# dune-community/pylrbms

Hardware: AMD Instinct MI355X
Metric: offline project+estimate throughput (higher is better)
Workload: dtype f64; 1 GPU; BASELINE.json config 3: 2D multiscale diffusion, 32x32 subdomains, k_c=4 (n=384 DG DoFs, n_rt=208 RT0 DoFs per subdomain), Q=2, local basis dim 40; subdomains=1024, N=40, Q=2, parallelism=subdomain tiles x1

## Files before the change

include/lrbms_hip.h:

```cpp
#ifndef LRBMS_HIP_H
#define LRBMS_HIP_H

#include <stdint.h>

#ifdef __cplusplus
extern "C" {
#endif

#define LRBMS_OK 0
#define LRBMS_E_INVALID (-1)
#define LRBMS_E_HIP (-2)
#define LRBMS_E_STATE (-3)
#define LRBMS_E_NOT_CONVERGED (-4)

#define LRBMS_NS 16

typedef struct lrbms_ctx lrbms_ctx;

typedef struct {
  int32_t kx, ky, n_T, n_rt, n_vertices, ncf;
  double hx, hy;
  double kappa[4];
  const int32_t* nb_elem;
  const int32_t* nb_face;
  const int32_t* nb_elem_out;
  const int32_t* nb_face_out;
  const int32_t* elem_side_pos;
  const int32_t* elem_rt;
  const int32_t* face_sign;
  const int32_t* dof_vertex;
  const int32_t* vdof_ptr;
  const int32_t* vdof_idx;
  const int32_t* rt_e0;
  const int32_t* rt_f0;
  const int32_t* rt_e1;
  const int32_t* rt_f1;
  const int32_t* rt_side;
  const int32_t* side_elem;
  const int32_t* side_elem_out;
  const int32_t* side_count;
  int32_t ntouch;
  const int32_t* touch_elem;
  const int32_t* touch_count;
  const double* grad;
  const double* area;
  const double* normal;
  const double* face_len;
  const double* points;
} lrbms_mesh_desc;

int lrbms_ctx_create(int device, lrbms_ctx** out);
int lrbms_ctx_destroy(lrbms_ctx* ctx);
const char* lrbms_last_error(lrbms_ctx* ctx);
const char* lrbms_version(void);

int lrbms_mesh_upload(lrbms_ctx* ctx, const lrbms_mesh_desc* desc, int32_t S, int32_t S_ext, const int32_t* nbr);

#define LRBMS_MAXQV 16
#define LRBMS_MAXQF 4
typedef struct {
  int32_t n, pad;
  double w[LRBMS_MAXQV];
  double b[LRBMS_MAXQV][3];
} lrbms_tri_rule;
typedef struct {
  int32_t n, pad;
  double w[LRBMS_MAXQF];
  double t[LRBMS_MAXQF];
} lrbms_edge_rule;
typedef struct {
  lrbms_tri_rule system_volume, energy_volume, elliptic_bar, rhs, f2, ceps, df_aa, df_ab, df_bb;
  lrbms_edge_rule system_inner_face, system_coupling_face, energy_face, flux_face;
  int32_t nfs, o_sysv, o_sysf, o_enf, o_flf, o_env, lam_stride;
  int32_t o_aa, o_ab, lamdf_stride;
  int32_t o_haa, o_hab, o_hbb, o_hceps, lhat_stride;
  int32_t o_frhs, o_ff2, f_stride, lbar_stride, pad_;
} lrbms_quadrature;
int lrbms_set_quadrature(lrbms_ctx* ctx, const lrbms_quadrature* quad);

int lrbms_assemble_swipdg(lrbms_ctx* ctx, int32_t Q, const double* lam, double* A_diag, double* A_cpl, void* stream);

int lrbms_assemble_rhs(lrbms_ctx* ctx, const double* f_smp, const double* lhat, double* b, double* f2, double* ceps,
                       void* stream);

int lrbms_assemble_products(lrbms_ctx* ctx, int32_t Q, const double* theta_bar, const double* lam, const double* lam_df,
                            const double* lbar, const double* lhat, double* P_diag, double* ebar, double* caa, double* Aab,
                            double* Bbb, void* stream);

int lrbms_assemble_flux(lrbms_ctx* ctx, int32_t Q, const double* lam, double* F, void* stream);

int lrbms_oswald_apply(lrbms_ctx* ctx, int32_t N, const double* V, double* Wt, void* stream);

int lrbms_flux_reconstruct(lrbms_ctx* ctx, int32_t Q, int32_t N, const double* F, const double* V, double* Rt,
                           void* stream);

int lrbms_project_system(lrbms_ctx* ctx, int32_t Q, int32_t N, const double* V, const double* A_diag,
                         const double* A_cpl, const double* P_diag, const double* b, double* work, double* B_sys,
                         double* rhs_red, double* E_red, double* M_red, void* stream);

int64_t lrbms_estimator_work_size(lrbms_ctx* ctx, int32_t Q, int32_t N);
int lrbms_estimator_grams(lrbms_ctx* ctx, int32_t Q, int32_t N, const double* V, const double* Wt, const double* Rt,
                          const double* ebar, const double* caa, const double* Aab, const double* Bbb,
                          const double* b, double* work, double* G_nc, double* r_fd, double* G_rdd, double* G_bb,
                          double* G_ab, double* G_aa, void* stream);

int lrbms_fused_supported(lrbms_ctx* ctx, int32_t Q, int32_t N);
int32_t lrbms_fused_fnc_ld(lrbms_ctx* ctx, int32_t N);
int64_t lrbms_fused_mfma_per_subdomain(lrbms_ctx* ctx, int32_t Q, int32_t N);
int lrbms_fused_factored_supported(lrbms_ctx* ctx, int32_t Q, int32_t N);
int64_t lrbms_fused_work_size(lrbms_ctx* ctx, int32_t Q, int32_t N);
int lrbms_project_estimate_fused(lrbms_ctx* ctx, int32_t Q, int32_t N, const double* V, const double* F,
                                 const double* A_diag, const double* A_cpl, const double* P_diag, const double* b,
                                 const double* ebar, const double* caa, const double* Aab, const double* Bbb,
                                 double* work, double* B_sys, double* rhs_red, double* E_red, double* M_red,
                                 double* G_nc, double* r_fd, double* G_rdd, double* G_bb, double* G_ab, double* G_aa,
                                 void* stream);

void* lrbms_ctx_aux_stream(lrbms_ctx* ctx, int32_t i);

#define LRBMS_OPT_OSWALD_VERTEX_PATCH 9
#define LRBMS_OPT_OSWALD_ZERO_ON_SUBDOMAIN_BOUNDARY 1
#define LRBMS_OPT_ACCUMULATE_COUPLING_ACROSS_Q 2
#define LRBMS_OPT_STREAMS 3
#define LRBMS_OPT_F1_KSPLIT 4
#define LRBMS_OPT_F1_FORM 5
#define LRBMS_OPT_COARSE 6
#define LRBMS_OPT_SOLVE_VALU 7
#define LRBMS_OPT_ESTIMATE_VALU 8
#define LRBMS_OPT_PREP_LDS 10
#define LRBMS_OPT_F2_FORM 11
int lrbms_ctx_set_option(lrbms_ctx* ctx, int32_t option, int32_t value);

int lrbms_set_diagonal_neighbours(lrbms_ctx* ctx, const int32_t* nbr_diag);

int lrbms_fused_set_subset(lrbms_ctx* ctx, const int32_t* subset, int32_t count);

int lrbms_kernel_timing(lrbms_ctx* ctx, int32_t enable);
int lrbms_kernel_timing_read(lrbms_ctx* ctx, char* names, int64_t names_cap, double* ms, int32_t cap, int32_t* count);

int lrbms_project_estimate_fused_phase(lrbms_ctx* ctx, int32_t phase, int32_t Q, int32_t N, const double* V, const double* F,
                                       const double* A_diag, const double* A_cpl, const double* P_diag, const double* b,
                                       const double* ebar, const double* caa, const double* Aab, const double* Bbb, double* work,
                                       double* B_sys, double* rhs_red, double* E_red, double* M_red, double* G_nc, double* r_fd,
                                       double* G_rdd, double* G_bb, double* G_ab, double* G_aa, void* stream);

int64_t lrbms_fside_size(lrbms_ctx* ctx, int32_t Q, int32_t N);
int64_t lrbms_fnc_size(lrbms_ctx* ctx, int32_t N);
int lrbms_project_estimate_fused_factored(lrbms_ctx* ctx, int32_t phase, int32_t Q, int32_t N, const double* V, const double* F,
                                          const double* A_diag, const double* A_cpl, const double* P_diag, const double* b,
                                          const double* ebar, const double* caa, const double* Aab, const double* Bbb, double* work,
                                          double* B_sys, double* rhs_red, double* E_red, double* M_red, double* G_nc_self,
                                          double* r_fd, double* G_rdd_self, double* G_bb_self, double* G_ab_self, double* G_aa,
                                          double* F_side, double* F_nc, void* stream);
int lrbms_reduced_estimate_factored(lrbms_ctx* ctx, int32_t Q, int32_t N, const double* theta, const double* u,
                                    const double* G_nc_self, const double* r_fd, const double* G_rdd_self, const double* G_bb_self,
                                    const double* G_ab_self, const double* G_aa, const double* F_side, const double* F_nc,
                                    const double* f2, const double* ceps, double hdiam, double* eta_loc, void* stream);
int lrbms_reduced_estimate_batch_factored(lrbms_ctx* ctx, int32_t Q, int32_t N, int32_t nmu, const double* theta, const double* u,
                                          const double* G_nc_self, const double* r_fd, const double* G_rdd_self,
                                          const double* G_bb_self, const double* G_ab_self, const double* G_aa, const double* F_side,
                                          const double* F_nc, const double* f2, const double* ceps, double hdiam, double* eta_loc,
                                          void* stream);

int lrbms_reduced_estimate(lrbms_ctx* ctx, int32_t Q, int32_t N, const double* theta, const double* u,
                           const double* G_nc, const double* r_fd, const double* G_rdd, const double* G_bb,
                           const double* G_ab, const double* G_aa, const double* f2, const double* ceps, double hdiam,
                           double* eta_loc, void* stream);

int lrbms_reduced_estimate_batch(lrbms_ctx* ctx, int32_t Q, int32_t N, int32_t nmu, const double* theta, const double* u,
                                 const double* G_nc, const double* r_fd, const double* G_rdd, const double* G_bb,
                                 const double* G_ab, const double* G_aa, const double* f2, const double* ceps, double hdiam,
                                 double* eta_loc, void* stream);

int64_t lrbms_reduced_solve_work_size(lrbms_ctx* ctx, int32_t N);
int lrbms_reduced_solve(lrbms_ctx* ctx, int32_t Q, int32_t N, const double* theta, const double* B_sys,
                        const double* rhs_red, double* work, double* u, double rtol, int32_t max_iter, double* info,
                        void* stream);

int64_t lrbms_reduced_solve_batch_work_size(lrbms_ctx* ctx, int32_t N, int32_t nmu);
int lrbms_reduced_solve_batch(lrbms_ctx* ctx, int32_t Q, int32_t N, int32_t nmu, const double* theta, const double* B_sys,
                              const double* rhs_red, double* work, double* u, double rtol, int32_t max_iter, double* info,
                              void* stream);

int64_t lrbms_reduced_precond_size(lrbms_ctx* ctx, int32_t N);
int lrbms_reduced_precond_build(lrbms_ctx* ctx, int32_t Q, int32_t N, const double* theta, const double* B_sys, double* work,
                                double* pc, void* stream);
int lrbms_reduced_precond_use(lrbms_ctx* ctx, int32_t N, const double* pc);

int64_t lrbms_fom_solve_work_size(lrbms_ctx* ctx);
int lrbms_fom_solve(lrbms_ctx* ctx, int32_t Q, const double* theta, const double* A_diag, const double* A_cpl, const double* b,
                    double* work, double* x, double rtol, int32_t max_iter, double* info, void* stream);

int lrbms_fom_implicit_euler(lrbms_ctx* ctx, int32_t Q, const double* theta, double dt, int32_t nt, const double* A_diag,
                             const double* A_cpl, const double* b, double* work, double* U, double rtol, int32_t max_iter,
                             double* info, void* stream);

int lrbms_mass_inverse_norm2(lrbms_ctx* ctx, int32_t L, const double* Y, double* out, void* stream);

int lrbms_div_apply(lrbms_ctx* ctx, int32_t C, int32_t mode, const double* Rt, double* out, void* stream);
int lrbms_div_pairing(lrbms_ctx* ctx, int32_t Q, int32_t L, const double* theta, const double* D, const double* G, double* out,
                      void* stream);
int lrbms_reduced_reconstruction_terms(lrbms_ctx* ctx, int32_t Q, int32_t N, int32_t L, const double* theta, const double* B_sys,
                                       const double* M_red, const double* rhs_red, const double* G_ud, const double* U,
                                       double* work, double* out, void* stream);

int lrbms_reduced_implicit_euler(lrbms_ctx* ctx, int32_t Q, int32_t N, const double* theta, double dt, int32_t nt,
                                 const double* B_sys, const double* M_red, const double* rhs_red, double* work, double* U,
                                 double rtol, int32_t max_iter, double* info, void* stream);

int64_t lrbms_reduced_time_residual_work_size(lrbms_ctx* ctx, int32_t N);
int lrbms_reduced_time_residual(lrbms_ctx* ctx, int32_t Q, int32_t N, int32_t L, const double* theta, const double* B_sys,
                                const double* M_red, const double* dU, double* work, double* out, void* stream);

// ... 46 lines not shown
```

pylrbms_amd/_native.py:

```python
import ctypes
import os

import numpy as np

_HERE = os.path.dirname(os.path.abspath(__file__))
LIB_PATH = os.path.join(_HERE, 'liblrbms_hip.so')

c_i32, c_i64, c_dbl, c_vp = ctypes.c_int32, ctypes.c_int64, ctypes.c_double, ctypes.c_void_p
_P_I32 = ctypes.POINTER(c_i32)
_P_DBL = ctypes.POINTER(c_dbl)


class MeshDesc(ctypes.Structure):
    _fields_ = ([(k, c_i32) for k in ('kx', 'ky', 'n_T', 'n_rt', 'n_vertices', 'ncf')] +
                [('hx', c_dbl), ('hy', c_dbl), ('kappa', c_dbl * 4)] +
                [(k, _P_I32) for k in ('nb_elem', 'nb_face', 'nb_elem_out', 'nb_face_out', 'elem_side_pos', 'elem_rt',
                                       'face_sign', 'dof_vertex', 'vdof_ptr', 'vdof_idx', 'rt_e0', 'rt_f0', 'rt_e1',
                                       'rt_f1', 'rt_side', 'side_elem', 'side_elem_out', 'side_count')] +
                [('ntouch', c_i32), ('touch_elem', _P_I32), ('touch_count', _P_I32)] +
                [(k, _P_DBL) for k in ('grad', 'area', 'normal', 'face_len', 'points')])


SIGNATURES = {
    'lrbms_version': (ctypes.c_char_p, []),
    'lrbms_ctx_create': (ctypes.c_int, [ctypes.c_int, ctypes.POINTER(c_vp)]),
    'lrbms_ctx_destroy': (ctypes.c_int, [c_vp]),
    'lrbms_last_error': (ctypes.c_char_p, [c_vp]),
    'lrbms_ctx_aux_stream': (c_vp, [c_vp, c_i32]),
    'lrbms_ctx_set_option': (ctypes.c_int, [c_vp, c_i32, c_i32]),
    'lrbms_set_quadrature': (ctypes.c_int, [c_vp, c_vp]),
    'lrbms_fused_set_subset': (ctypes.c_int, [c_vp, _P_I32, c_i32]),
    'lrbms_set_diagonal_neighbours': (ctypes.c_int, [c_vp, _P_I32]),
    'lrbms_kernel_timing': (ctypes.c_int, [c_vp, c_i32]),
    'lrbms_kernel_timing_read': (ctypes.c_int, [c_vp, ctypes.c_char_p, ctypes.c_int64, ctypes.POINTER(ctypes.c_double), c_i32,
                                                ctypes.POINTER(c_i32)]),
    'lrbms_mesh_upload': (ctypes.c_int, [c_vp, ctypes.POINTER(MeshDesc), c_i32, c_i32, _P_I32]),
    'lrbms_assemble_swipdg': (ctypes.c_int, [c_vp, c_i32, c_vp, c_vp, c_vp, c_vp]),
    'lrbms_assemble_rhs': (ctypes.c_int, [c_vp, c_vp, c_vp, c_vp, c_vp, c_vp, c_vp]),
    'lrbms_assemble_products': (ctypes.c_int, [c_vp, c_i32, _P_DBL, c_vp, c_vp, c_vp, c_vp, c_vp, c_vp, c_vp, c_vp, c_vp, c_vp]),
    'lrbms_assemble_flux': (ctypes.c_int, [c_vp, c_i32, c_vp, c_vp, c_vp]),
    'lrbms_oswald_apply': (ctypes.c_int, [c_vp, c_i32, c_vp, c_vp, c_vp]),
    'lrbms_flux_reconstruct': (ctypes.c_int, [c_vp, c_i32, c_i32, c_vp, c_vp, c_vp, c_vp]),
    'lrbms_project_system': (ctypes.c_int, [c_vp, c_i32, c_i32] + [c_vp] * 11),
    'lrbms_estimator_work_size': (c_i64, [c_vp, c_i32, c_i32]),
    'lrbms_estimator_grams': (ctypes.c_int, [c_vp, c_i32, c_i32] + [c_vp] * 16),
    'lrbms_fused_supported': (ctypes.c_int, [c_vp, c_i32, c_i32]),
    'lrbms_fused_mfma_per_subdomain': (c_i64, [c_vp, c_i32, c_i32]),
    'lrbms_fused_fnc_ld': (c_i32, [c_vp, c_i32]),
    'lrbms_fused_factored_supported': (ctypes.c_int, [c_vp, c_i32, c_i32]),
    'lrbms_fused_work_size': (c_i64, [c_vp, c_i32, c_i32]),
    'lrbms_project_estimate_fused': (ctypes.c_int, [c_vp, c_i32, c_i32] + [c_vp] * 22),
    'lrbms_project_estimate_fused_phase': (ctypes.c_int, [c_vp, c_i32, c_i32, c_i32] + [c_vp] * 22),
    'lrbms_fside_size': (c_i64, [c_vp, c_i32, c_i32]),
    'lrbms_fnc_size': (c_i64, [c_vp, c_i32]),
    'lrbms_project_estimate_fused_factored': (ctypes.c_int, [c_vp, c_i32, c_i32, c_i32] + [c_vp] * 24),
    'lrbms_reduced_estimate_factored': (ctypes.c_int, [c_vp, c_i32, c_i32, _P_DBL] + [c_vp] * 11 + [c_dbl, c_vp, c_vp]),
    'lrbms_reduced_estimate_batch_factored': (ctypes.c_int, [c_vp, c_i32, c_i32, c_i32, _P_DBL] + [c_vp] * 11 + [c_dbl, c_vp, c_vp]),
    'lrbms_reduced_estimate': (ctypes.c_int, [c_vp, c_i32, c_i32, _P_DBL] + [c_vp] * 9 + [c_dbl, c_vp, c_vp]),
    'lrbms_reduced_estimate_batch': (ctypes.c_int, [c_vp, c_i32, c_i32, c_i32, _P_DBL] + [c_vp] * 9 + [c_dbl, c_vp, c_vp]),
    'lrbms_reduced_solve_work_size': (c_i64, [c_vp, c_i32]),
    'lrbms_reduced_solve': (ctypes.c_int, [c_vp, c_i32, c_i32, _P_DBL, c_vp, c_vp, c_vp, c_vp, c_dbl, c_i32, _P_DBL, c_vp]),
    'lrbms_reduced_solve_batch_work_size': (c_i64, [c_vp, c_i32, c_i32]),
    'lrbms_reduced_solve_batch': (ctypes.c_int, [c_vp, c_i32, c_i32, c_i32, _P_DBL, c_vp, c_vp, c_vp, c_vp, c_dbl, c_i32, _P_DBL,
                                                 c_vp]),
    'lrbms_reduced_precond_size': (c_i64, [c_vp, c_i32]),
    'lrbms_reduced_precond_build': (ctypes.c_int, [c_vp, c_i32, c_i32, _P_DBL, c_vp, c_vp, c_vp, c_vp]),
    'lrbms_reduced_precond_use': (ctypes.c_int, [c_vp, c_i32, c_vp]),
    'lrbms_fom_solve_work_size': (c_i64, [c_vp]),
    'lrbms_fom_solve': (ctypes.c_int, [c_vp, c_i32, _P_DBL, c_vp, c_vp, c_vp, c_vp, c_vp, c_dbl, c_i32, _P_DBL, c_vp]),
    'lrbms_fom_implicit_euler': (ctypes.c_int, [c_vp, c_i32, _P_DBL, c_dbl, c_i32, c_vp, c_vp, c_vp, c_vp, c_vp, c_dbl, c_i32, _P_DBL,
                                                c_vp]),
    'lrbms_mass_inverse_norm2': (ctypes.c_int, [c_vp, c_i32, c_vp, c_vp, c_vp]),
    'lrbms_div_apply': (ctypes.c_int, [c_vp, c_i32, c_i32, c_vp, c_vp, c_vp]),
    'lrbms_div_pairing': (ctypes.c_int, [c_vp, c_i32, c_i32, _P_DBL, c_vp, c_vp, c_vp, c_vp]),
    'lrbms_reduced_reconstruction_terms': (ctypes.c_int, [c_vp, c_i32, c_i32, c_i32, _P_DBL] + [c_vp] * 8),
    'lrbms_reduced_implicit_euler': (ctypes.c_int, [c_vp, c_i32, c_i32, _P_DBL, c_dbl, c_i32, c_vp, c_vp, c_vp, c_vp, c_vp, c_dbl,
                                                    c_i32, _P_DBL, c_vp]),
    'lrbms_reduced_time_residual_work_size': (c_i64, [c_vp, c_i32]),
    'lrbms_reduced_time_residual': (ctypes.c_int, [c_vp, c_i32, c_i32, c_i32, _P_DBL, c_vp, c_vp, c_vp, c_vp, c_vp, c_vp]),
    'lrbms_assemble_source_gram': (ctypes.c_int, [c_vp, c_i32, c_vp, c_vp, c_vp]),
    'lrbms_fom_implicit_euler_src': (ctypes.c_int, [c_vp, c_i32, c_i32, _P_DBL, c_dbl, c_i32, c_vp, c_vp, c_vp, c_vp, c_vp, c_vp,
                                                    c_dbl, c_i32, _P_DBL, c_vp]),
    'lrbms_reduced_implicit_euler_src': (ctypes.c_int, [c_vp, c_i32, c_i32, c_i32, _P_DBL, c_dbl, c_i32, c_vp, c_vp, c_vp, c_vp, c_vp,
                                                        c_vp, c_dbl, c_i32, _P_DBL, c_vp]),
    'lrbms_project_sources': (ctypes.c_int, [c_vp, c_i32, c_i32, c_i32, c_vp, c_vp, c_vp, c_vp, c_vp, c_vp]),
    'lrbms_reduced_source_terms': (ctypes.c_int, [c_vp, c_i32, c_i32, c_i32, c_i32, _P_DBL, c_vp, c_vp, c_vp, c_vp, c_vp, c_dbl,
                                                  c_vp, c_vp]),
    'lrbms_reduced_solve_batch_src': (ctypes.c_int, [c_vp, c_i32, c_i32, c_i32, c_i32, _P_DBL, _P_DBL, c_vp, c_vp, c_vp, c_vp, c_dbl,
                                                     c_i32, _P_DBL, c_vp]),
    'lrbms_reduced_implicit_euler_batch_work_size': (c_i64, [c_vp, c_i32, c_i32]),
    'lrbms_reduced_implicit_euler_batch': (ctypes.c_int, [c_vp, c_i32, c_i32, c_i32, _P_DBL, c_dbl, c_i32, c_vp, c_vp, c_vp, c_vp, c_vp,
                                                          c_dbl, c_i32, _P_DBL, c_vp]),
    'lrbms_reduced_implicit_euler_batch_src': (ctypes.c_int, [c_vp, c_i32, c_i32, c_i32, c_i32, _P_DBL, c_dbl, c_i32, c_vp, c_vp, c_vp,
                                                              c_vp, c_vp, c_vp, c_dbl, c_i32, _P_DBL, c_vp]),
    'lrbms_combine_sources': (ctypes.c_int, [c_vp, c_i32, c_i64, _P_DBL, c_vp, c_vp, c_vp]),
    'lrbms_assemble_dirichlet_correction': (ctypes.c_int, [c_vp, c_i32, c_vp, c_vp, c_vp]),
    'lrbms_local_correction_work_size': (c_i64, [c_vp, c_i32]),
    'lrbms_local_correction_solve': (ctypes.c_int, [c_vp, c_i32, _P_DBL, c_i32, _P_I32, c_vp, c_vp, c_vp, c_vp, c_vp, c_vp, c_dbl,
                                                    c_i32, _P_DBL, c_vp]),
    'lrbms_blockell_apply': (ctypes.c_int, [c_vp, c_i32, c_vp, c_vp, c_vp, c_vp]),
    'lrbms_fom_apply': (ctypes.c_int, [c_vp, c_i32, c_i32, _P_DBL, c_vp, c_vp, c_vp, c_vp, c_vp]),
    'lrbms_gemm_tn': (ctypes.c_int, [c_vp, c_i32, c_i32, c_i32, c_i32, c_vp, c_i64, c_i32, c_vp, c_i64, c_i32, c_vp,
                                     c_i64, c_i32, c_vp, c_dbl, c_vp]),
}

_lib = None


class NativeError(RuntimeError):
    pass


def load_library(path=None):
    global _lib
    if _lib is not None and path is None:
        return _lib
    path = path or os.environ.get('LRBMS_HIP_LIB') or LIB_PATH
    import torch
    if not os.path.exists(path):
        raise NativeError('{} is missing: run `python __graft_entry__.py` (or pylrbms_amd/_build.py) to build the HIP '
                          'extension; there is no CPU fallback'.format(path))
    lib = ctypes.CDLL(path)
    for name, (restype, argtypes) in SIGNATURES.items():
        fn = getattr(lib, name)
        fn.restype, fn.argtypes = restype, argtypes
    _lib = lib
    return lib


def _i32p(a):
    return a.ctypes.data_as(_P_I32)


def _dblp(a):
    return a.ctypes.data_as(_P_DBL)


class ContextBase:

    PREFIX = None
    OPTIONS = {}
    TIMING_CAP = None
    _load = None

    def __init__(self, device_index=0):
        import torch
        self.torch = torch
        if not torch.cuda.is_available():
            raise NativeError('no HIP device visible: the LRBMS hot path has no CPU fallback')
        self.lib = self._load()
        self.device = torch.device('cuda', device_index)
        handle = c_vp()
        rc = self._fn('ctx_create')(device_index, ctypes.byref(handle))
        if rc != 0:
            raise NativeError('{}ctx_create failed with code {}'.format(self.PREFIX, rc))
        self.handle = handle
        self._pid = os.getpid()

    def _fn(self, name):
        return getattr(self.lib, self.PREFIX + name)

    def close(self):
        if getattr(self, 'handle', None):
            if getattr(self, '_pid', None) == os.getpid():
                self._fn('ctx_destroy')(self.handle)
            self.handle = None

    def __del__(self):
        try:
            self.close()
        except Exception:
            pass

    def _check(self, rc, what):
        if rc != 0:
            msg = self._fn('last_error')(self.handle)
            raise NativeError('{} failed ({}): {}'.format(what, rc, msg.decode() if msg else ''))

    def _stream(self):
        return c_vp(self.torch.cuda.current_stream(self.device).cuda_stream)

    def _ptr(self, t, shape, name):
        torch = self.torch
        if not isinstance(t, torch.Tensor) or t.dtype != torch.float64 or t.device != self.device:
            raise NativeError('{}: expected a float64 tensor on {}'.format(name, self.device))
        if tuple(t.shape) != tuple(shape):
            raise NativeError('{}: expected shape {}, got {}'.format(name, tuple(shape), tuple(t.shape)))
        if not t.is_contiguous():
            raise NativeError('{}: tensor must be contiguous'.format(name))
        return c_vp(t.data_ptr())

    def empty(self, *shape):
        return self.torch.empty(*shape, dtype=self.torch.float64, device=self.device)

    def zeros(self, *shape):
        return self.torch.zeros(*shape, dtype=self.torch.float64, device=self.device)

    def from_numpy(self, a):
        return self.torch.from_numpy(np.array(a, dtype=np.float64, order='C', copy=True)).to(self.device)

    def set_option(self, name, value):
        if name not in self.OPTIONS:
            raise NativeError('unknown option {!r}; known: {}'.format(name, sorted(self.OPTIONS)))
        self._check(self._fn('ctx_set_option')(self.handle, self.OPTIONS[name], int(value)), self.PREFIX + 'ctx_set_option')

    def kernel_timing(self, enable):
        self._check(self._fn('kernel_timing')(self.handle, 1 if enable else 0), self.PREFIX + 'kernel_timing')

    def kernel_timing_read(self, cap=None):
        cap = self.TIMING_CAP if cap is None else int(cap)
        names = ctypes.create_string_buffer(64 * cap)
        ms = (c_dbl * cap)()
        count = c_i32(0)
        self._check(self._fn('kernel_timing_read')(self.handle, names, 64 * cap, ms, cap, ctypes.byref(count)),
                    self.PREFIX + 'kernel_timing_read')
        nm = names.value.decode().split('\n') if count.value else []
        return [(nm[i], ms[i]) for i in range(count.value)]


class NativeContext(ContextBase):

    PREFIX = 'lrbms_'
    TIMING_CAP = 256
    _load = staticmethod(load_library)
    OPTIONS = {'oswald_zero_on_subdomain_boundary': 1, 'accumulate_coupling_across_q': 2, 'oswald_vertex_patch': 9, 'prep_lds': 10,
               'streams': 3, 'f1_ksplit': 4, 'f1_form': 5, 'coarse': 6, 'solve_valu': 7, 'estimate_valu': 8,
               'f2_form': 11}
    S = S_ext = None
    _keep = None

    def mesh_upload(self, template, kappa, nbr, S, S_ext):
        t = template
        self.t, self.S, self.S_ext = t, int(S), int(S_ext)
        self.n_T, self.n, self.n_rt, self.ncf = t.n_T, t.n, t.n_rt, t.ncf
        self.nvs = max(t.nvx, t.nvy)
        arrs = {}
        d = MeshDesc()
        d.kx, d.ky, d.n_T, d.n_rt, d.n_vertices, d.ncf = t.kx, t.ky, t.n_T, t.n_rt, t.n_vertices, t.ncf
        d.hx, d.hy = t.hx, t.hy
        d.ntouch = t.ntouch
        kap = np.asarray(kappa, dtype=np.float64).reshape(4)
        for i in range(4):
            d.kappa[i] = kap[i]
        for k in ('nb_elem', 'nb_face', 'nb_elem_out', 'nb_face_out', 'elem_side_pos', 'elem_rt', 'face_sign',
                  'dof_vertex', 'vdof_ptr', 'vdof_idx', 'rt_e0', 'rt_f0', 'rt_e1', 'rt_f1', 'rt_side', 'side_elem',
                  'side_elem_out', 'side_count', 'touch_elem', 'touch_count'):
            arrs[k] = np.ascontiguousarray(getattr(t, k), dtype=np.int32)
            setattr(d, k, _i32p(arrs[k]))
        for k in ('grad', 'area', 'normal', 'face_len', 'points'):
            arrs[k] = np.ascontiguousarray(getattr(t, k), dtype=np.float64)
            setattr(d, k, _dblp(arrs[k]))
        nb = np.ascontiguousarray(nbr, dtype=np.int32)
        assert nb.shape == (S, 5)
        rc = self.lib.lrbms_mesh_upload(self.handle, ctypes.byref(d), S, S_ext, _i32p(nb))
        self._keep = (arrs, nb)
        self._check(rc, 'lrbms_mesh_upload')

    def set_quadrature(self, spec):
        from pylrbms_amd.quadrature import native_quadrature
        self.quad = native_quadrature(spec)
        self.quad_spec = spec
        self._check(self.lib.lrbms_set_quadrature(self.handle, ctypes.byref(self.quad)), 'lrbms_set_quadrature')

    def _quad(self):
        if getattr(self, 'quad', None) is None:
            raise NativeError('set_quadrature() must run before the assembly calls')
        return self.quad

    def assemble_swipdg(self, lam):
        Q, qd = lam.shape[0], self._quad()
        A_diag = self.empty(Q, self.S, self.n_T, 4, 9)
        A_cpl = self.empty(Q, self.S, 4, self.ncf, 9)
        rc = self.lib.lrbms_assemble_swipdg(self.handle, Q, self._ptr(lam, (Q, self.S_ext, self.n_T, qd.lam_stride), 'lam'),
                                            c_vp(A_diag.data_ptr()), c_vp(A_cpl.data_ptr()), self._stream())
        self._check(rc, 'lrbms_assemble_swipdg')
        return A_diag, A_cpl

    def assemble_rhs(self, f_smp, lhat):
        qd = self._quad()
        b, f2, ceps = self.empty(self.S, self.n), self.empty(self.S), self.empty(self.S)
        rc = self.lib.lrbms_assemble_rhs(self.handle, self._ptr(f_smp, (self.S, self.n_T, qd.f_stride), 'f_smp'),
                                         self._ptr(lhat, (self.S, self.n_T, qd.lhat_stride), 'lhat'), c_vp(b.data_ptr()),
                                         c_vp(f2.data_ptr()), c_vp(ceps.data_ptr()), self._stream())
        self._check(rc, 'lrbms_assemble_rhs')
        return b, f2, ceps

    def assemble_products(self, theta_bar, lam, lam_df, lbar, lhat):
        Q, qd = lam.shape[0], self._quad()
        th = np.ascontiguousarray(theta_bar, dtype=np.float64)
        assert th.shape == (Q,)
        P_diag = self.empty(self.S, self.n_T, 4, 9)
        ebar = self.empty(self.S, self.n_T)
        caa = self.empty(Q, Q, self.S, self.n_T)
        Aab = self.empty(Q, self.S, self.n_T, 3, 3)
        Bbb = self.empty(self.S, self.n_T, 3, 3)
        rc = self.lib.lrbms_assemble_products(
            self.handle, Q, _dblp(th), self._ptr(lam, (Q, self.S_ext, self.n_T, qd.lam_stride), 'lam'),
            self._ptr(lam_df, (Q, self.S, self.n_T, qd.lamdf_stride), 'lam_df'),
            self._ptr(lbar, (self.S, self.n_T, qd.lbar_stride), 'lbar'), self._ptr(lhat, (self.S, self.n_T, qd.lhat_stride), 'lhat'),
            c_vp(P_diag.data_ptr()), c_vp(ebar.data_ptr()), c_vp(caa.data_ptr()), c_vp(Aab.data_ptr()),
            c_vp(Bbb.data_ptr()), self._stream())
        self._check(rc, 'lrbms_assemble_products')
        return P_diag, ebar, caa, Aab, Bbb

    def assemble_flux(self, lam):
        Q, qd = lam.shape[0], self._quad()
        F = self.empty(Q, self.S, self.n_rt, 6)
        rc = self.lib.lrbms_assemble_flux(self.handle, Q, self._ptr(lam, (Q, self.S_ext, self.n_T, qd.lam_stride), 'lam'),
                                          c_vp(F.data_ptr()), self._stream())
        self._check(rc, 'lrbms_assemble_flux')
        return F

    def oswald_apply(self, V, out=None):
        N = V.shape[2]
        Wt = out if out is not None else self.empty(self.S, self.n, 5 * N)
        rc = self.lib.lrbms_oswald_apply(self.handle, N, self._ptr(V, (self.S_ext, self.n, N), 'V'),
                                         self._ptr(Wt, (self.S, self.n, 5 * N), 'Wt'), self._stream())
        self._check(rc, 'lrbms_oswald_apply')
        return Wt

    def flux_reconstruct(self, F, V, out=None):
        Q, N = F.shape[0], V.shape[2]
        Rt = out if out is not None else self.empty(self.S, self.n_rt, 5 * Q * N)
        rc = self.lib.lrbms_flux_reconstruct(self.handle, Q, N, self._ptr(F, (Q, self.S, self.n_rt, 6), 'F'),
                                             self._ptr(V, (self.S_ext, self.n, N), 'V'),
                                             self._ptr(Rt, (self.S, self.n_rt, 5 * Q * N), 'Rt'), self._stream())
        self._check(rc, 'lrbms_flux_reconstruct')
        return Rt

    def project_system(self, V, A_diag, A_cpl, P_diag, b, work=None, out=None):
        Q, N, S = A_diag.shape[0], V.shape[2], self.S
        if work is None:
            work = self.empty(Q * S * self.n * N)
        if work.numel() < Q * S * self.n * N:
            raise NativeError('project_system: work too small')
        if out is None:
            out = (self.empty(Q, S, 5, N, N), self.empty(S, N), self.empty(S, N, N), self.empty(S, N, N))
        B_sys, rhs_red, E_red, M_red = out
        rc = self.lib.lrbms_project_system(
            self.handle, Q, N, self._ptr(V, (self.S_ext, self.n, N), 'V'),
            self._ptr(A_diag, (Q, S, self.n_T, 4, 9), 'A_diag'), self._ptr(A_cpl, (Q, S, 4, self.ncf, 9), 'A_cpl'),
            self._ptr(P_diag, (S, self.n_T, 4, 9), 'P_diag'), self._ptr(b, (S, self.n), 'b'), c_vp(work.data_ptr()),
            self._ptr(B_sys, (Q, S, 5, N, N), 'B_sys'), self._ptr(rhs_red, (S, N), 'rhs_red'),
            self._ptr(E_red, (S, N, N), 'E_red'), self._ptr(M_red, (S, N, N), 'M_red'), self._stream())
        self._check(rc, 'lrbms_project_system')
        return B_sys, rhs_red, E_red, M_red

    def estimator_work_size(self, Q, N):
        sz = self.lib.lrbms_estimator_work_size(self.handle, Q, N)
        if sz < 0:
            raise NativeError('lrbms_estimator_work_size failed')
        return int(sz)

    def estimator_grams(self, V, Wt, Rt, ebar, caa, Aab, Bbb, b, work=None, out=None):
        Q, N, S = caa.shape[0], V.shape[2], self.S
        W, C = 5 * N, 5 * Q * N
        need = self.estimator_work_size(Q, N)
        if work is None:
            work = self.empty(need)
        if work.numel() < need:
            raise NativeError('estimator_grams: work too small')
        if out is None:
            out = (self.empty(S, W, W), self.empty(S, C), self.empty(S, 9, Q * N, Q * N), self.empty(S, 9, Q * N, Q * N),
                   self.empty(Q, S, N, C), self.empty(Q, Q, S, N, N))
        G_nc, r_fd, G_rdd, G_bb, G_ab, G_aa = out
        rc = self.lib.lrbms_estimator_grams(
            self.handle, Q, N, self._ptr(V, (self.S_ext, self.n, N), 'V'), self._ptr(Wt, (S, self.n, W), 'Wt'),
            self._ptr(Rt, (S, self.n_rt, C), 'Rt'), self._ptr(ebar, (S, self.n_T), 'ebar'),
            self._ptr(caa, (Q, Q, S, self.n_T), 'caa'), self._ptr(Aab, (Q, S, self.n_T, 3, 3), 'Aab'),
            self._ptr(Bbb, (S, self.n_T, 3, 3), 'Bbb'), self._ptr(b, (S, self.n), 'b'), c_vp(work.data_ptr()),
            self._ptr(G_nc, (S, W, W), 'G_nc'), self._ptr(r_fd, (S, C), 'r_fd'), self._ptr(G_rdd, (S, 9, Q * N, Q * N), 'G_rdd'),
            self._ptr(G_bb, (S, 9, Q * N, Q * N), 'G_bb'), self._ptr(G_ab, (Q, S, N, C), 'G_ab'),
            self._ptr(G_aa, (Q, Q, S, N, N), 'G_aa'), self._stream())
        self._check(rc, 'lrbms_estimator_grams')
        return G_nc, r_fd, G_rdd, G_bb, G_ab, G_aa

    def fused_supported(self, Q, N, factored=False):
        fn = self.lib.lrbms_fused_factored_supported if factored else self.lib.lrbms_fused_supported
        return bool(fn(self.handle, Q, N))

    def fused_work_size(self, Q, N):
        sz = self.lib.lrbms_fused_work_size(self.handle, Q, N)
        if sz < 0:
            raise NativeError('lrbms_fused_work_size failed')
        return int(sz)
# ... 500 lines not shown
```

pylrbms_amd/csrc/assemble.hip:

```cpp
#include "lrbms_dev.h"

struct QVec { double v[8]; };

namespace {

typedef lrbms_quadrature Quad;

struct FaceSide {
  double lam[LRBMS_MAXQF];
  double kgn[3];
  double phi[3][LRBMS_MAXQF];
};

__device__ inline void kgrad_dot_n(const Tmpl& t, int e, double nx, double ny, double out[3]) {
  for (int i = 0; i < 3; ++i) {
    double gx = t.grad[(e * 3 + i) * 2 + 0], gy = t.grad[(e * 3 + i) * 2 + 1];
    double kx = t.kappa[0] * gx + t.kappa[1] * gy, ky = t.kappa[2] * gx + t.kappa[3] * gy;
    out[i] = kx * nx + ky * ny;
  }
}

__device__ inline void load_self_side(const Tmpl& t, const lrbms_edge_rule& r, const double* smp, int e, int f, double nx,
                                      double ny, FaceSide& s) {
  for (int k = 0; k < r.n; ++k) s.lam[k] = smp[k];
// ... 354 lines not shown
      double sigma = 0.5 * (m.lam[k] + p.lam[k]) * SIGMA_INNER * (0.5 * delta) / len;
      for (int j = 0; j < 3; ++j) {
        c0[j] += rf.w[k] * (-0.5 * m.lam[k] * m.kgn[j] + rho * sigma * m.phi[j][k]);
        c1[j] += rf.w[k] * (-0.5 * p.lam[k] * p.kgn[j] - rho * sigma * p.phi[j][k]);
      }
    }
  }
  double* out = F + (((long)q * S + s) * t.nrt + r) * 6;
  for (int j = 0; j < 3; ++j) {
    out[j] = c0[j];
    out[3 + j] = c1[j];
  }
}

__global__ __launch_bounds__(256) void k_assemble_dcorr(Tmpl t, const Quad* __restrict__ qd, int S, int S_ext,
                                                        const int* __restrict__ nbr, const double* __restrict__ lam,
                                                        double* __restrict__ D_corr) {
  long idx = (long)blockIdx.x * blockDim.x + threadIdx.x;
  if (idx >= (long)S * t.nT) return;
  const Quad& Q_ = *qd;
  const lrbms_edge_rule& r = Q_.system_coupling_face;
  const int LS = Q_.lam_stride, oF = Q_.o_sysf, nfs = Q_.nfs;
  const int q = blockIdx.y;
  const int s = (int)(idx / t.nT), e = (int)(idx % t.nT);
  const double* lam_q = lam + (long)q * S_ext * t.nT * LS;
  const double* lam_e = lam_q + ((long)s * t.nT + e) * LS;
  for (int f = 0; f < 3; ++f) {
    const int nb = t.nb_elem[e * 3 + f];
    if (nb >= 0) continue;
    const int side = -1 - nb;
    const int s2 = nbr[s * 5 + side_to_slot(side)];
    if (s2 < 0) continue;
    const double nx = t.normal[(e * 3 + f) * 2], ny = t.normal[(e * 3 + f) * 2 + 1];
    const double len = t.face_len[e * 3 + f];
    const double delta = n_kappa_n(t, nx, ny);
    FaceSide m, p;
    load_self_side(t, r, lam_e + oF + f * nfs, e, f, nx, ny, m);
    const int e2 = t.nb_elem_out[e * 3 + f], f2 = t.nb_face_out[e * 3 + f];
    load_other_side(t, r, lam_q + ((long)s2 * t.nT + e2) * LS + oF + f2 * nfs, e2, f2, nx, ny, p);
    double ss[9] = {0, 0, 0, 0, 0, 0, 0, 0, 0}, so[9] = {0, 0, 0, 0, 0, 0, 0, 0, 0}, bd[9] = {0, 0, 0, 0, 0, 0, 0, 0, 0};
    swipdg_inner(r, m, p, len, delta, ss, so);
    swipdg_boundary(r, m, len, delta, bd);
    double* out = D_corr + ((((long)q * S + s) * 4 + side) * t.ncf + t.elem_side_pos[e * 3 + f]) * 9;
    for (int i = 0; i < 9; ++i) out[i] = bd[i] - ss[i];
  }
}

}

int launch_assemble_dcorr(lrbms_ctx* ctx, int Q, const double* lam, double* D_corr, hipStream_t st) {
  const Tmpl& t = ctx->t;
  LRBMS_HIP_CHECK(ctx, hipMemsetAsync(D_corr, 0, sizeof(double) * (size_t)Q * ctx->S * 4 * t.ncf * 9, st));
  long total = (long)ctx->S * t.nT;
  dim3 grid((unsigned)((total + 255) / 256), Q);
  if (!ctx->qdev) return lrbms_fail(ctx, LRBMS_E_STATE, "quadrature not set (lrbms_set_quadrature)");
  hipLaunchKernelGGL(k_assemble_dcorr, grid, dim3(256), 0, st, t, ctx->qdev, ctx->S, ctx->S_ext, ctx->nbr, lam, D_corr);
  LRBMS_LAUNCH_CHECK(ctx);
  return LRBMS_OK;
}

int launch_assemble_swipdg(lrbms_ctx* ctx, int Q, const double* lam, double* A_diag, double* A_cpl, hipStream_t st) {
  const Tmpl& t = ctx->t;
  LRBMS_HIP_CHECK(ctx, hipMemsetAsync(A_cpl, 0, sizeof(double) * (size_t)Q * ctx->S * 4 * t.ncf * 9, st));
  long total = (long)ctx->S * t.nT;
  dim3 grid((unsigned)((total + 255) / 256), Q);
  if (!ctx->qdev) return lrbms_fail(ctx, LRBMS_E_STATE, "quadrature not set (lrbms_set_quadrature)");
  hipLaunchKernelGGL(k_assemble_swipdg, grid, dim3(256), 0, st, t, ctx->qdev, ctx->S, ctx->S_ext, ctx->nbr, lam, A_diag, A_cpl);
  LRBMS_LAUNCH_CHECK(ctx);
  return LRBMS_OK;
}

int launch_assemble_source_gram(lrbms_ctx* ctx, int K, const double* f_smp_K, double* F2, hipStream_t st) {
  if (K < 1 || K > 64) return lrbms_fail(ctx, LRBMS_E_INVALID, "assemble_source_gram: K must be in [1, 64]");
  hipLaunchKernelGGL(k_assemble_source_gram, dim3(ctx->S, K * (K + 1) / 2), dim3(256), 0, st, ctx->t, ctx->qdev, ctx->S, K, f_smp_K, F2);
  LRBMS_LAUNCH_CHECK(ctx);
  return LRBMS_OK;
}

int launch_assemble_rhs(lrbms_ctx* ctx, const double* f_smp, const double* lhat, double* b, double* f2, double* ceps,
                        hipStream_t st) {
  if (!ctx->qdev) return lrbms_fail(ctx, LRBMS_E_STATE, "quadrature not set (lrbms_set_quadrature)");
  hipLaunchKernelGGL(k_assemble_rhs, dim3(ctx->S), dim3(256), 0, st, ctx->t, ctx->qdev, f_smp, lhat, b, f2, ceps);
  LRBMS_LAUNCH_CHECK(ctx);
  return LRBMS_OK;
}

int launch_assemble_products(lrbms_ctx* ctx, int Q, const double* theta_bar, const double* lam, const double* lam_df,
                             const double* lbar, const double* lhat, double* P_diag, double* ebar, double* caa, double* Aab,
                             double* Bbb, hipStream_t st) {
  if (!ctx->qdev) return lrbms_fail(ctx, LRBMS_E_STATE, "quadrature not set (lrbms_set_quadrature)");
  QVec tb;
  for (int q = 0; q < 8; ++q) tb.v[q] = q < Q ? theta_bar[q] : 0.0;
  long total = (long)ctx->S * ctx->t.nT;
  hipLaunchKernelGGL(k_assemble_products, dim3((unsigned)((total + 255) / 256)), dim3(256), 0, st, ctx->t, ctx->qdev, ctx->S,
                     ctx->S_ext, ctx->nbr, Q, tb, lam, lam_df, lbar, lhat, P_diag, ebar, caa, Aab, Bbb);
  LRBMS_LAUNCH_CHECK(ctx);
  const long need = (long)Q * ctx->S * ctx->t.nT * 6;
  if (ctx->wab_cap < need) {
    if (ctx->wab) LRBMS_HIP_CHECK(ctx, hipFree(ctx->wab));
    ctx->wab = nullptr;
    ctx->wab_cap = 0;
    LRBMS_HIP_CHECK(ctx, hipMalloc(&ctx->wab, sizeof(double) * (size_t)need));
    ctx->wab_cap = need;
  }
  ctx->wab_src = nullptr;
  if (int rc = launch_wab(ctx, Q, Aab, ctx->wab, st)) return rc;
  ctx->wab_src = Aab;
  ctx->wab_Q = Q;
  return LRBMS_OK;
}

int launch_assemble_flux(lrbms_ctx* ctx, int Q, const double* lam, double* F, hipStream_t st) {
  long total = (long)ctx->S * ctx->t.nrt;
  dim3 grid((unsigned)((total + 255) / 256), Q);
  if (!ctx->qdev) return lrbms_fail(ctx, LRBMS_E_STATE, "quadrature not set (lrbms_set_quadrature)");
  hipLaunchKernelGGL(k_assemble_flux, grid, dim3(256), 0, st, ctx->t, ctx->qdev, ctx->S, ctx->S_ext, ctx->nbr, lam, F);
  LRBMS_LAUNCH_CHECK(ctx);
  return LRBMS_OK;
}
```

pylrbms_amd/csrc/capi.hip:

```cpp
#include <cmath>
#include <cstring>
#include <map>
#include <mutex>

#include "lrbms_dev.h"

int64_t estimator_work_size(lrbms_ctx* ctx, int Q, int N);
int64_t reduced_solve_work_size(lrbms_ctx* ctx, int N);
int launch_reduced_estimate_batch(lrbms_ctx* ctx, int Q, int N, int nmu, const double* theta, const double* u, const double* G_nc,
                                  const double* r_fd, const double* G_rdd, const double* G_bb, const double* G_ab,
                                  const double* G_aa, const double* Fside, const double* Fnc, const double* f2, const double* ceps,
                                  double hdiam, double* eta_loc, hipStream_t st);
int64_t reduced_solve_batch_work_size(lrbms_ctx* ctx, int N, int nmu);
int launch_reduced_solve_batch(lrbms_ctx* ctx, int Q, int N, int nmu, const double* theta, const double* B_sys,
                               const double* rhs_red, double* work, double* u, double rtol, int max_iter, double* info,
                               hipStream_t st);
int launch_assemble_dcorr(lrbms_ctx* ctx, int Q, const double* lam, double* D_corr, hipStream_t st);
int64_t local_correction_work_size(lrbms_ctx* ctx, int nmark);
int launch_local_correction(lrbms_ctx* ctx, int Q, const double* theta, int nmark, const int32_t* marked, const double* A_diag,
                            const double* A_cpl, const double* D_corr, const double* b, double* work, double* corr, double rtol,
                            int max_iter, double* info, hipStream_t st);
int64_t fom_solve_work_size(lrbms_ctx* ctx);
int launch_fom_solve(lrbms_ctx* ctx, int Q, const double* theta, const double* A_diag, const double* A_cpl, const double* b,
                     double* work, double* x, double rtol, int max_iter, double* info, hipStream_t st);
// ... 91 lines not shown
    (void)hipStreamDestroy(it->second.s);
    side_streams.erase(it);
  }
}

int lrbms_ctx_base_init(lrbms_ctx_base* ctx, int device) {
  ctx->device = device;
  bool ok = hipEventCreateWithFlags(&ctx->ev_fork, hipEventDisableTiming) == hipSuccess;
  for (int i = 0; i < 3 && ok; ++i)
    ok = (ctx->aux[i] = lrbms_side_stream_acquire(device, i)) != nullptr &&
         hipEventCreateWithFlags(&ctx->ev_join[i], hipEventDisableTiming) == hipSuccess;
  return ok ? LRBMS_OK : LRBMS_E_HIP;
}

void lrbms_ctx_base_release(lrbms_ctx_base* ctx) {
  for (int i = 0; i < 3; ++i) {
    if (ctx->aux[i]) lrbms_side_stream_release(ctx->device, i);
    if (ctx->ev_join[i]) (void)hipEventDestroy(ctx->ev_join[i]);
  }
  if (ctx->ev_fork) (void)hipEventDestroy(ctx->ev_fork);
  for (auto& k : ctx->ktimers) {
    if (k.e0) (void)hipEventDestroy(k.e0);
    if (k.e1) (void)hipEventDestroy(k.e1);
  }
}

int lrbms_ctx_kernel_timing(lrbms_ctx_base* ctx, int32_t enable) {
  if (!ctx) return LRBMS_E_INVALID;
  ctx->ktime = enable != 0;
  ctx->ktime_n = 0;
  for (auto& k : ctx->ktimers) k.used = false;
  return LRBMS_OK;
}

int lrbms_ctx_kernel_timing_read(lrbms_ctx_base* ctx, char* names, int64_t names_cap, double* ms, int32_t cap, int32_t* count) {
  if (!ctx || !names || !ms || !count || names_cap <= 0) return LRBMS_E_INVALID;
  LRBMS_HIP_CHECK(ctx, hipDeviceSynchronize());
  int n = 0;
  std::string joined;
  for (int i = 0; i < ctx->ktime_n && n < cap; ++i) {
    const auto& k = ctx->ktimers[i];
    if (!k.used) continue;
    float t = 0.f;
    LRBMS_HIP_CHECK(ctx, hipEventElapsedTime(&t, k.e0, k.e1));
    ms[n++] = (double)t;
    if (!joined.empty()) joined += '\n';
    joined += k.name;
  }
  if ((int64_t)joined.size() + 1 > names_cap) return lrbms_fail(ctx, LRBMS_E_INVALID, "kernel_timing_read: names buffer too small");
  memcpy(names, joined.c_str(), joined.size() + 1);
  *count = n;
  ctx->ktime_n = 0;
  for (auto& k : ctx->ktimers) k.used = false;
  return LRBMS_OK;
}

extern "C" {

const char* lrbms_version(void) { return "lrbms_hip 0.1.0 (gfx950)"; }

int lrbms_ctx_create(int device, lrbms_ctx** out) {
  if (!out) return LRBMS_E_INVALID;
  *out = nullptr;
  int count = 0;
  if (hipGetDeviceCount(&count) != hipSuccess || device < 0 || device >= count) return LRBMS_E_HIP;
  if (hipSetDevice(device) != hipSuccess) return LRBMS_E_HIP;
  lrbms_ctx* ctx = new (std::nothrow) lrbms_ctx();
  if (!ctx) return LRBMS_E_INVALID;
  if (lrbms_ctx_base_init(ctx, device) != LRBMS_OK || hipEventCreateWithFlags(&ctx->ev_prep, hipEventDisableTiming) != hipSuccess)
    return lrbms_ctx_destroy(ctx), LRBMS_E_HIP;
  *out = ctx;
  return LRBMS_OK;
}

int lrbms_ctx_destroy(lrbms_ctx* ctx) {
  if (!ctx) return LRBMS_E_INVALID;
  (void)hipSetDevice(ctx->device);
  coarse_release(ctx);
  free_owned(ctx);
  if (ctx->ksp_part) (void)hipFree(ctx->ksp_part);
  if (ctx->ksp_ticket) (void)hipFree(ctx->ksp_ticket);
  if (ctx->subset) (void)hipFree(ctx->subset);
  if (ctx->wab) (void)hipFree(ctx->wab);
  if (ctx->src_phi) (void)hipFree(ctx->src_phi);
  lrbms_ctx_base_release(ctx);
  if (ctx->ev_prep) (void)hipEventDestroy(ctx->ev_prep);
  delete ctx;
  return LRBMS_OK;
}

void* lrbms_ctx_aux_stream(lrbms_ctx* ctx, int32_t i) { return (ctx && i >= 0 && i < 3) ? (void*)ctx->aux[i] : nullptr; }

const char* lrbms_last_error(lrbms_ctx* ctx) { return ctx ? ctx->err.c_str() : "null context"; }

int lrbms_ctx_set_option(lrbms_ctx* ctx, int32_t option, int32_t value) {
  if (!ctx) return LRBMS_E_INVALID;
  int lo = 0, hi = 1;
  if (option == LRBMS_OPT_STREAMS) lo = -1;
  if (option == LRBMS_OPT_F1_KSPLIT) hi = 4;
  if (option == LRBMS_OPT_COARSE) hi = 2;
  if (option == LRBMS_OPT_PREP_LDS) hi = 3;
  if (option == LRBMS_OPT_F1_FORM) hi = 3;
  if (option == LRBMS_OPT_F2_FORM) hi = 2;
  if (value < lo || value > hi || (option == LRBMS_OPT_F1_KSPLIT && value == 3))
    return lrbms_fail(ctx, LRBMS_E_INVALID, "set_option: value out of range for this option");
  switch (option) {
    case LRBMS_OPT_OSWALD_ZERO_ON_SUBDOMAIN_BOUNDARY: ctx->t.opt_oswald_subdomain = value; break;
    case LRBMS_OPT_ACCUMULATE_COUPLING_ACROSS_Q: ctx->t.opt_accumulate_coupling = value; break;
    case LRBMS_OPT_OSWALD_VERTEX_PATCH:
      if (ctx->pass_ran && ctx->t.opt_oswald_vertex != value)
        return lrbms_fail(ctx, LRBMS_E_STATE, "set_option: LRBMS_OPT_OSWALD_VERTEX_PATCH cannot change after a fused pass has run on this context");
      ctx->t.opt_oswald_vertex = value;
      break;
    case LRBMS_OPT_STREAMS: ctx->opt_streams = value; break;
    case LRBMS_OPT_F1_KSPLIT: ctx->opt_f1_ksplit = value; break;
    case LRBMS_OPT_F1_FORM: ctx->opt_f1_legacy = value; break;
    case LRBMS_OPT_F2_FORM: ctx->opt_f2_form = value; break;
    case LRBMS_OPT_COARSE: ctx->opt_coarse = value; break;
    case LRBMS_OPT_SOLVE_VALU: ctx->opt_solve_valu = value; break;
    case LRBMS_OPT_ESTIMATE_VALU: ctx->opt_estimate_valu = value; break;
    case LRBMS_OPT_PREP_LDS: ctx->opt_prep_lds = value; break;
    default: return lrbms_fail(ctx, LRBMS_E_INVALID, "set_option: unknown option");
  }
  return LRBMS_OK;
}

int lrbms_set_diagonal_neighbours(lrbms_ctx* ctx, const int32_t* nbr_diag) {
  LRBMS_REQUIRE_MESH(ctx);
  if (!nbr_diag) return lrbms_fail(ctx, LRBMS_E_INVALID, "set_diagonal_neighbours: null table");
  for (long i = 0; i < (long)ctx->S * 4; ++i)
    if (nbr_diag[i] < -1 || nbr_diag[i] >= ctx->S_ext)
      return lrbms_fail(ctx, LRBMS_E_INVALID, "set_diagonal_neighbours: index out of range [-1, S_ext)");
  LRBMS_HIP_CHECK(ctx, hipDeviceSynchronize());
  LRBMS_HIP_CHECK(ctx, hipMemcpy(const_cast<int*>(ctx->t.nbr_diag), nbr_diag, sizeof(int) * (size_t)ctx->S * 4, hipMemcpyHostToDevice));
  ctx->diag_explicit = true;
  return LRBMS_OK;
}

int lrbms_fused_set_subset(lrbms_ctx* ctx, const int32_t* subset, int32_t count) {
  LRBMS_REQUIRE_MESH(ctx);
  if (count < 0 || count > ctx->S || (count > 0 && subset == nullptr))
    return lrbms_fail(ctx, LRBMS_E_INVALID, "fused_set_subset: count must be in [0, S] and the list non-null");
  for (int i = 0; i < count; ++i)
    if (subset[i] < 0 || subset[i] >= ctx->S || (i > 0 && subset[i] <= subset[i - 1]))
      return lrbms_fail(ctx, LRBMS_E_INVALID, "fused_set_subset: the list must be strictly ascending local subdomain indices in [0, S)");
  if (count > ctx->subset_cap) {
    if (ctx->subset) LRBMS_HIP_CHECK(ctx, hipFree(ctx->subset));
    ctx->subset = nullptr;
    ctx->subset_cap = 0;
    LRBMS_HIP_CHECK(ctx, hipMalloc(&ctx->subset, sizeof(int) * (size_t)ctx->S));
    ctx->subset_cap = ctx->S;
  }
  if (count > 0) {
    LRBMS_HIP_CHECK(ctx, hipDeviceSynchronize());
    LRBMS_HIP_CHECK(ctx, hipMemcpy(ctx->subset, subset, sizeof(int) * (size_t)count, hipMemcpyHostToDevice));
  }
  ctx->subset_n = count;
  return LRBMS_OK;
}

int lrbms_kernel_timing(lrbms_ctx* ctx, int32_t enable) { return lrbms_ctx_kernel_timing(ctx, enable); }

int lrbms_kernel_timing_read(lrbms_ctx* ctx, char* names, int64_t names_cap, double* ms, int32_t cap, int32_t* count) {
  return lrbms_ctx_kernel_timing_read(ctx, names, names_cap, ms, cap, count);
}

int lrbms_mesh_upload(lrbms_ctx* ctx, const lrbms_mesh_desc* d, int32_t S, int32_t S_ext, const int32_t* nbr) {
  if (!ctx || !d || !nbr) return LRBMS_E_INVALID;
  if (S <= 0 || S_ext < S) return lrbms_fail(ctx, LRBMS_E_INVALID, "mesh_upload: need 0 < S <= S_ext");
  if (d->kx <= 0 || d->ky <= 0 || d->n_T != 8 * d->kx * d->ky || d->n_rt <= 0 ||
      d->n_vertices != (2 * d->kx + 1) * (2 * d->ky + 1) || d->ncf != 2 * (d->kx > d->ky ? d->kx : d->ky))
    return lrbms_fail(ctx, LRBMS_E_INVALID, "mesh_upload: inconsistent template sizes");
  for (int i = 0; i < S; ++i) {
    for (int k = 0; k < 5; ++k) {
      const int v = nbr[i * 5 + k];
      if (v < -1 || v >= S_ext) return lrbms_fail(ctx, LRBMS_E_INVALID, "mesh_upload: neighbour index out of range");
    }
    if (nbr[i * 5 + 2] != i) return lrbms_fail(ctx, LRBMS_E_INVALID, "mesh_upload: nbr[s][2] must be s");
  }
  const int nT = d->n_T, n = 3 * nT;
  for (int i = 0; i < 3 * nT; ++i) {
    if (d->nb_elem[i] >= nT || d->nb_elem[i] < -4) return lrbms_fail(ctx, LRBMS_E_INVALID, "mesh_upload: nb_elem out of range");
    if (d->nb_elem[i] < 0 && (d->nb_elem_out[i] < 0 || d->nb_elem_out[i] >= nT || d->elem_side_pos[i] < 0 ||
                              d->elem_side_pos[i] >= d->ncf || d->nb_face_out[i] < 0 || d->nb_face_out[i] > 2))
      return lrbms_fail(ctx, LRBMS_E_INVALID, "mesh_upload: side face pairing out of range");
    if (d->nb_face[i] < 0 || d->nb_face[i] > 2) return lrbms_fail(ctx, LRBMS_E_INVALID, "mesh_upload: nb_face out of range");
    if (d->elem_rt[i] < 0 || d->elem_rt[i] >= d->n_rt) return lrbms_fail(ctx, LRBMS_E_INVALID, "mesh_upload: elem_rt out of range");
    if (d->dof_vertex[i] < 0 || d->dof_vertex[i] >= d->n_vertices || d->vdof_idx[i] < 0 || d->vdof_idx[i] >= n)
      return lrbms_fail(ctx, LRBMS_E_INVALID, "mesh_upload: vertex star out of range");
  }
  if (d->vdof_ptr[0] != 0 || d->vdof_ptr[d->n_vertices] != n) return lrbms_fail(ctx, LRBMS_E_INVALID, "mesh_upload: bad vdof_ptr");
  for (int v = 0; v < d->n_vertices; ++v)
    if (d->vdof_ptr[v + 1] < d->vdof_ptr[v]) return lrbms_fail(ctx, LRBMS_E_INVALID, "mesh_upload: vdof_ptr not monotone");
  for (int r = 0; r < d->n_rt; ++r) {
    if (d->rt_e0[r] < 0 || d->rt_e0[r] >= nT || d->rt_f0[r] < 0 || d->rt_f0[r] > 2 || d->rt_side[r] < -1 || d->rt_side[r] > 3 ||
        d->rt_e1[r] < 0 || d->rt_e1[r] >= nT || d->rt_f1[r] < 0 || d->rt_f1[r] > 2)
      return lrbms_fail(ctx, LRBMS_E_INVALID, "mesh_upload: rt face table out of range");
  }
  for (int sd = 0; sd < 4; ++sd) {
    if (d->side_count[sd] < 0 || d->side_count[sd] > d->ncf) return lrbms_fail(ctx, LRBMS_E_INVALID, "mesh_upload: side_count");
    for (int p = 0; p < d->side_count[sd]; ++p)
      if (d->side_elem[sd * d->ncf + p] < 0 || d->side_elem[sd * d->ncf + p] >= nT || d->side_elem_out[sd * d->ncf + p] < 0 ||
          d->side_elem_out[sd * d->ncf + p] >= nT)
        return lrbms_fail(ctx, LRBMS_E_INVALID, "mesh_upload: side element out of range");
  }

  LRBMS_HIP_CHECK(ctx, hipSetDevice(ctx->device));
  free_owned(ctx);
  Tmpl& t = ctx->t;
  t.kx = d->kx; t.ky = d->ky; t.nT = nT; t.n = n; t.nrt = d->n_rt; t.nv = d->n_vertices;
  t.nvx = 2 * d->kx + 1; t.nvy = 2 * d->ky + 1; t.ncf = d->ncf; t.hx = d->hx; t.hy = d->hy;
  std::memcpy(t.kappa, d->kappa, sizeof(double) * 4);
  const double det = t.kappa[0] * t.kappa[3] - t.kappa[1] * t.kappa[2];
  if (!(det > 0.0)) return lrbms_fail(ctx, LRBMS_E_INVALID, "mesh_upload: kappa must be positive definite");
  t.kinv[0] = t.kappa[3] / det; t.kinv[1] = -t.kappa[1] / det; t.kinv[2] = -t.kappa[2] / det; t.kinv[3] = t.kappa[0] / det;
  const double a = t.kappa[0], b = 0.5 * (t.kappa[1] + t.kappa[2]), c = t.kappa[3];
  t.kmin = 0.5 * (a + c) - std::sqrt(0.25 * (a - c) * (a - c) + b * b);
  int rc;
#define UP(field, count)                                                                            \
  do {                                                                                              \
    if (!d->field) return lrbms_fail(ctx, LRBMS_E_INVALID, "mesh_upload: null template array");     \
    if ((rc = upload(ctx, d->field, (long)(count), &t.field))) return rc;                           \
  } while (0)
  UP(nb_elem, 3 * nT); UP(nb_face, 3 * nT); UP(nb_elem_out, 3 * nT); UP(nb_face_out, 3 * nT); UP(elem_side_pos, 3 * nT);
  UP(elem_rt, 3 * nT); UP(face_sign, 3 * nT); UP(dof_vertex, n); UP(vdof_ptr, d->n_vertices + 1); UP(vdof_idx, n);
  UP(rt_e0, d->n_rt); UP(rt_f0, d->n_rt); UP(rt_e1, d->n_rt); UP(rt_f1, d->n_rt); UP(rt_side, d->n_rt);
  UP(side_elem, 4 * d->ncf); UP(side_elem_out, 4 * d->ncf); UP(side_count, 4);
  if (d->ntouch <= 0 || !d->touch_elem || !d->touch_count) return lrbms_fail(ctx, LRBMS_E_INVALID, "mesh_upload: touch table missing");
  for (int sd = 0; sd < 4; ++sd) {
    if (d->touch_count[sd] < 0 || d->touch_count[sd] > d->ntouch) return lrbms_fail(ctx, LRBMS_E_INVALID, "mesh_upload: touch_count");
    for (int p = 0; p < d->touch_count[sd]; ++p)
      if (d->touch_elem[sd * d->ntouch + p] < 0 || d->touch_elem[sd * d->ntouch + p] >= nT)
        return lrbms_fail(ctx, LRBMS_E_INVALID, "mesh_upload: touch_elem out of range");
  }
  t.ntouch = d->ntouch;
  UP(touch_elem, 4 * d->ntouch); UP(touch_count, 4);
  UP(grad, 6 * nT); UP(area, nT); UP(normal, 6 * nT); UP(face_len, 3 * nT); UP(points, 6 * nT);
#undef UP
  const int* nbr_dev = nullptr;
  if ((rc = upload(ctx, nbr, (long)S * 5, &nbr_dev))) return rc;
  ctx->nbr = const_cast<int*>(nbr_dev);
  ctx->nbr_host.assign(nbr, nbr + (size_t)S * 5);
  {
    std::vector<int32_t> dg((size_t)S * 4, -1);
    for (int i = 0; i < S; ++i)
      for (int c = 0; c < 4; ++c) {
        const int sa = nbr[i * 5 + (c < 2 ? 0 : 4)];
        if (sa >= 0 && sa < S) dg[(size_t)i * 4 + c] = nbr[sa * 5 + ((c & 1) ? 3 : 1)];
      }
    const int* dg_dev = nullptr;
    if ((rc = upload(ctx, dg.data(), (long)dg.size(), &dg_dev))) return rc;
    t.nbr_diag = dg_dev;
    ctx->diag_explicit = false;
  }
  ctx->subset_n = 0;
  ctx->wab_src = nullptr;
  ctx->pass_ran = false;
  ctx->S = S;
  ctx->S_ext = S_ext;
  if ((rc = build_template_tables(ctx))) return rc;
  ctx->has_mesh = true;
  return LRBMS_OK;
}

#define CHECK_Q_N(ctx, Q, N)                                                                        \
  do {                                                                                              \
    if ((Q) < 1 || (Q) > 8) return lrbms_fail(ctx, LRBMS_E_INVALID, "Q must be in 1..8");            \
    if ((N) < 1) return lrbms_fail(ctx, LRBMS_E_INVALID, "N must be >= 1");                          \
  } while (0)
#define CHECK_PTR(ctx, p) \
  do { if (!(p)) return lrbms_fail(ctx, LRBMS_E_INVALID, "null pointer: " #p); } while (0)

int lrbms_set_quadrature(lrbms_ctx* ctx, const lrbms_quadrature* quad) {
  if (!ctx || !quad) return LRBMS_E_INVALID;
  const lrbms_tri_rule* tri[9] = {&quad->system_volume, &quad->energy_volume, &quad->elliptic_bar, &quad->rhs, &quad->f2,
                                  &quad->ceps, &quad->df_aa, &quad->df_ab, &quad->df_bb};
  const lrbms_edge_rule* edge[4] = {&quad->system_inner_face, &quad->system_coupling_face, &quad->energy_face, &quad->flux_face};
  for (auto r : tri)
    if (r->n < 1 || r->n > LRBMS_MAXQV) return lrbms_fail(ctx, LRBMS_E_INVALID, "set_quadrature: triangle rule size out of range");
  for (auto r : edge) {
    if (r->n < 1 || r->n > LRBMS_MAXQF) return lrbms_fail(ctx, LRBMS_E_INVALID, "set_quadrature: edge rule size out of range");
    for (int k = 0; k < r->n; ++k)
      if (fabs(r->t[k] + r->t[r->n - 1 - k] - 1.0) > 1e-14 || fabs(r->w[k] - r->w[r->n - 1 - k]) > 1e-14)
        return lrbms_fail(ctx, LRBMS_E_INVALID, "set_quadrature: edge rules must be symmetric about 1/2");
  }
  const int nfs = quad->system_inner_face.n > quad->system_coupling_face.n ? quad->system_inner_face.n : quad->system_coupling_face.n;
  if (quad->nfs != nfs || quad->o_sysf < quad->o_sysv + quad->system_volume.n || quad->o_enf < quad->o_sysf + 3 * nfs ||
      quad->o_flf < quad->o_enf + 3 * quad->energy_face.n || quad->o_env < quad->o_flf + 3 * quad->flux_face.n ||
      quad->lam_stride < quad->o_env + quad->energy_volume.n || quad->lamdf_stride < quad->o_ab + quad->df_ab.n ||
      quad->o_ab < quad->o_aa + quad->df_aa.n || quad->o_hab < quad->o_haa + quad->df_aa.n ||
      quad->o_hbb < quad->o_hab + quad->df_ab.n || quad->o_hceps < quad->o_hbb + quad->df_bb.n ||
      quad->lhat_stride < quad->o_hceps + quad->ceps.n || quad->o_ff2 < quad->o_frhs + quad->rhs.n ||
      quad->f_stride < quad->o_ff2 + quad->f2.n || quad->lbar_stride < quad->elliptic_bar.n)
    return lrbms_fail(ctx, LRBMS_E_INVALID, "set_quadrature: inconsistent sample record layout");
  LRBMS_HIP_CHECK(ctx, hipSetDevice(ctx->device));
  if (!ctx->qdev) {
    LRBMS_HIP_CHECK(ctx, hipMalloc(&ctx->qdev, sizeof(lrbms_quadrature)));
    ctx->owned.push_back(ctx->qdev);
  }
  LRBMS_HIP_CHECK(ctx, hipMemcpy(ctx->qdev, quad, sizeof(lrbms_quadrature), hipMemcpyHostToDevice));
  return LRBMS_OK;
}

int lrbms_assemble_swipdg(lrbms_ctx* ctx, int32_t Q, const double* lam, double* A_diag, double* A_cpl, void* stream) {
  LRBMS_REQUIRE_MESH(ctx); CHECK_Q_N(ctx, Q, 1); CHECK_PTR(ctx, lam); CHECK_PTR(ctx, A_diag); CHECK_PTR(ctx, A_cpl);
  return launch_assemble_swipdg(ctx, Q, lam, A_diag, A_cpl, (hipStream_t)stream);
}

int lrbms_assemble_rhs(lrbms_ctx* ctx, const double* f_smp, const double* lhat, double* b, double* f2, double* ceps,
                       void* stream) {
  LRBMS_REQUIRE_MESH(ctx); CHECK_PTR(ctx, f_smp); CHECK_PTR(ctx, lhat); CHECK_PTR(ctx, b); CHECK_PTR(ctx, f2); CHECK_PTR(ctx, ceps);
  return launch_assemble_rhs(ctx, f_smp, lhat, b, f2, ceps, (hipStream_t)stream);
}

int lrbms_assemble_products(lrbms_ctx* ctx, int32_t Q, const double* theta_bar, const double* lam, const double* lam_df,
                            const double* lbar, const double* lhat, double* P_diag, double* ebar, double* caa, double* Aab,
                            double* Bbb, void* stream) {
  LRBMS_REQUIRE_MESH(ctx); CHECK_Q_N(ctx, Q, 1); CHECK_PTR(ctx, theta_bar); CHECK_PTR(ctx, lam); CHECK_PTR(ctx, lam_df); CHECK_PTR(ctx, lbar);
  CHECK_PTR(ctx, lhat); CHECK_PTR(ctx, P_diag); CHECK_PTR(ctx, ebar); CHECK_PTR(ctx, caa); CHECK_PTR(ctx, Aab); CHECK_PTR(ctx, Bbb);
  return launch_assemble_products(ctx, Q, theta_bar, lam, lam_df, lbar, lhat, P_diag, ebar, caa, Aab, Bbb, (hipStream_t)stream);
}

int lrbms_assemble_flux(lrbms_ctx* ctx, int32_t Q, const double* lam, double* F, void* stream) {
  LRBMS_REQUIRE_MESH(ctx); CHECK_Q_N(ctx, Q, 1); CHECK_PTR(ctx, lam); CHECK_PTR(ctx, F);
  return launch_assemble_flux(ctx, Q, lam, F, (hipStream_t)stream);
}

int lrbms_oswald_apply(lrbms_ctx* ctx, int32_t N, const double* V, double* Wt, void* stream) {
  LRBMS_REQUIRE_MESH(ctx); CHECK_Q_N(ctx, 1, N); CHECK_PTR(ctx, V); CHECK_PTR(ctx, Wt);
  return launch_oswald(ctx, N, V, Wt, (hipStream_t)stream);
}

int lrbms_flux_reconstruct(lrbms_ctx* ctx, int32_t Q, int32_t N, const double* F, const double* V, double* Rt, void* stream) {
  LRBMS_REQUIRE_MESH(ctx); CHECK_Q_N(ctx, Q, N); CHECK_PTR(ctx, F); CHECK_PTR(ctx, V); CHECK_PTR(ctx, Rt);
  return launch_flux(ctx, Q, N, F, V, Rt, (hipStream_t)stream);
}

int lrbms_project_system(lrbms_ctx* ctx, int32_t Q, int32_t N, const double* V, const double* A_diag, const double* A_cpl,
                         const double* P_diag, const double* b, double* work, double* B_sys, double* rhs_red, double* E_red,
                         double* M_red, void* stream) {
  LRBMS_REQUIRE_MESH(ctx); CHECK_Q_N(ctx, Q, N); CHECK_PTR(ctx, V); CHECK_PTR(ctx, A_diag); CHECK_PTR(ctx, A_cpl);
  CHECK_PTR(ctx, P_diag); CHECK_PTR(ctx, b); CHECK_PTR(ctx, work); CHECK_PTR(ctx, B_sys); CHECK_PTR(ctx, rhs_red);
  CHECK_PTR(ctx, E_red); CHECK_PTR(ctx, M_red);
  if ((size_t)2 * 3 * ctx->t.ncf * N * sizeof(double) > 64 * 1024)
    return lrbms_fail(ctx, LRBMS_E_INVALID, "project_system: coupling tile exceeds 64 KB of LDS");
  return launch_project_system(ctx, Q, N, V, A_diag, A_cpl, P_diag, b, work, B_sys, rhs_red, E_red, M_red, (hipStream_t)stream);
}

int64_t lrbms_estimator_work_size(lrbms_ctx* ctx, int32_t Q, int32_t N) {
  if (!ctx || !ctx->has_mesh || Q < 1 || N < 1) return -1;
  return estimator_work_size(ctx, Q, N);
}

int lrbms_estimator_grams(lrbms_ctx* ctx, int32_t Q, int32_t N, const double* V, const double* Wt, const double* Rt,
                          const double* ebar, const double* caa, const double* Aab, const double* Bbb, const double* b,
                          double* work, double* G_nc, double* r_fd, double* G_rdd, double* G_bb, double* G_ab, double* G_aa,
                          void* stream) {
  LRBMS_REQUIRE_MESH(ctx); CHECK_Q_N(ctx, Q, N); CHECK_PTR(ctx, V); CHECK_PTR(ctx, Wt); CHECK_PTR(ctx, Rt); CHECK_PTR(ctx, ebar);
  CHECK_PTR(ctx, caa); CHECK_PTR(ctx, Aab); CHECK_PTR(ctx, Bbb); CHECK_PTR(ctx, b); CHECK_PTR(ctx, work); CHECK_PTR(ctx, G_nc);
  CHECK_PTR(ctx, r_fd); CHECK_PTR(ctx, G_rdd); CHECK_PTR(ctx, G_bb); CHECK_PTR(ctx, G_ab); CHECK_PTR(ctx, G_aa);
  return launch_estimator_grams(ctx, Q, N, V, Wt, Rt, ebar, caa, Aab, Bbb, b, work, G_nc, r_fd, G_rdd, G_bb, G_ab, G_aa,
                                (hipStream_t)stream);
}

int32_t lrbms_fused_fnc_ld(lrbms_ctx* ctx, int32_t N) {
  if (!ctx || !ctx->has_mesh || N < 1) return -1;
  const int nvs = ctx->t.nvx > ctx->t.nvy ? ctx->t.nvx : ctx->t.nvy;
  return 2 * N + 4 * nvs + (ctx->t.opt_oswald_vertex ? N : 0);
}

int64_t lrbms_fused_mfma_per_subdomain(lrbms_ctx* ctx, int32_t Q, int32_t N) {
  if (!ctx || !ctx->has_mesh) return -1;
  return f1_mfma_per_subdomain(ctx, Q, N);
}

int lrbms_fused_supported(lrbms_ctx* ctx, int32_t Q, int32_t N) {
  if (!ctx || !ctx->has_mesh || Q < 1 || Q > 8 || N < 1) return 0;
  return fused_supported(ctx, Q, N, false) ? 1 : 0;
}

int lrbms_fused_factored_supported(lrbms_ctx* ctx, int32_t Q, int32_t N) {
  if (!ctx || !ctx->has_mesh || Q < 1 || N < 1) return 0;
  return fused_supported(ctx, Q, N, true) ? 1 : 0;
}

int64_t lrbms_fused_work_size(lrbms_ctx* ctx, int32_t Q, int32_t N) {
  if (!ctx || !ctx->has_mesh || Q < 1 || N < 1) return -1;
  return fused_work_size(ctx, Q, N);
}

int lrbms_project_estimate_fused(lrbms_ctx* ctx, int32_t Q, int32_t N, const double* V, const double* F, const double* A_diag,
                                 const double* A_cpl, const double* P_diag, const double* b, const double* ebar,
                                 const double* caa, const double* Aab, const double* Bbb, double* work, double* B_sys,
                                 double* rhs_red, double* E_red, double* M_red, double* G_nc, double* r_fd, double* G_rdd,
                                 double* G_bb, double* G_ab, double* G_aa, void* stream) {
  LRBMS_REQUIRE_MESH(ctx); CHECK_Q_N(ctx, Q, N); CHECK_PTR(ctx, V); CHECK_PTR(ctx, F); CHECK_PTR(ctx, A_diag); CHECK_PTR(ctx, A_cpl);
  CHECK_PTR(ctx, P_diag); CHECK_PTR(ctx, b); CHECK_PTR(ctx, ebar); CHECK_PTR(ctx, caa); CHECK_PTR(ctx, Aab); CHECK_PTR(ctx, Bbb);
  CHECK_PTR(ctx, work); CHECK_PTR(ctx, B_sys); CHECK_PTR(ctx, rhs_red); CHECK_PTR(ctx, E_red); CHECK_PTR(ctx, M_red);
  CHECK_PTR(ctx, G_nc); CHECK_PTR(ctx, r_fd); CHECK_PTR(ctx, G_rdd); CHECK_PTR(ctx, G_bb); CHECK_PTR(ctx, G_ab); CHECK_PTR(ctx, G_aa);
  return launch_project_estimate_fused(ctx, Q, N, V, F, A_diag, A_cpl, P_diag, b, ebar, caa, Aab, Bbb, work, B_sys, rhs_red, E_red,
                                       M_red, G_nc, r_fd, G_rdd, G_bb, G_ab, G_aa, nullptr, nullptr, 0, (hipStream_t)stream);
}

// ... 316 lines not shown
```

pylrbms_amd/csrc/fused.hip:

```cpp
#include <cstdlib>
#include <map>
#include <mutex>
#include <type_traits>
#include <utility>

#include "lrbms_dev.h"

namespace {

typedef double d4 __attribute__((ext_vector_type(4)));
typedef double d2 __attribute__((ext_vector_type(2)));
template <int W> struct VecT { using T = double; };
template <> struct VecT<2> { using T = d2; };
template <int W> __device__ inline typename VecT<W>::T ldv(const double* p) { return *reinterpret_cast<const typename VecT<W>::T*>(p); }
template <int W> __device__ inline void stv(double* p, typename VecT<W>::T v) { *reinterpret_cast<typename VecT<W>::T*>(p) = v; }
template <int W> __device__ inline typename VecT<W>::T zerov() { return typename VecT<W>::T(0.0); }
using W1 = std::integral_constant<int, 1>;
using W2 = std::integral_constant<int, 2>;

#if !defined(LRBMS_EXPERIMENT_BUILD) &&                                                                               \
    (defined(F1_NO_STAGE) || defined(F1_NO_APPLY) || defined(F1_NO_VALU_STAGE) || defined(F1_NO_MFMA) ||             \
     defined(F1_LDS_FILL) || defined(F1_PRODUCER_PRIO) || defined(F1_SPLIT_SIMD) || defined(F1_PF) ||                \
     defined(F2_NO_STAGE) || defined(F2_NO_MFMA) || defined(F2G_WG) || defined(F1_TRACE) || defined(F1V_NO_STORE) || defined(F1V_NO_MIRROR) || defined(F3_EW_X) || defined(PREP_TRACE) || defined(THIN_TRACE))
#error "experiment switch defined in a product build of fused.hip (use tools/build_variant.sh, which sets LRBMS_EXPERIMENT_BUILD)"
// ... 3276 lines not shown
    d4 acc[NACC];
#pragma unroll
    for (int k = 0; k < NACC; ++k) acc[k] = (d4){0.0, 0.0, 0.0, 0.0};
    for (int kk = 0; kk < KP; kk += 4) {
#pragma unroll
      for (int k = 0; k < NACC; ++k) {
        const int tile = wave + NW * k;
        if (tile < NTX * NTX) {
          const int ti = tile / NTX, tj = tile - ti * NTX;
          acc[k] = __builtin_amdgcn_mfma_f64_16x16x4f64(Wa[(kk + lk) * LDA + ti * 16 + li], Yc[(kk + lk) * LDB + tj * 16 + li], acc[k], 0, 0, 0);
        }
      }
    }
    const int cslot = pass == 0 ? 2 : slot;
#pragma unroll
    for (int k = 0; k < NACC; ++k) {
      const int tile = wave + NW * k;
      const int ti = tile / NTX, tj = tile - ti * NTX;
      const int jj = tj * 16 + li;
#pragma unroll
      for (int r = 0; r < 4; ++r) {
        const int row = ti * 16 + lk + 4 * r;
        const double val = acc[k][r];
        if (tile < NTX * NTX && jj < N && row < N) {
          G[(long)(slot * N + row) * W + cslot * N + jj] = val;
          if (pass == 0) G[(long)(2 * N + jj) * W + slot * N + row] = val;
        }
      }
    }
  }
  constexpr int RPC = NMAX / 4;
  for (int it = tid; it < 3 * N * 4; it += 512) {
    const int which = it / (4 * N), rem = it - which * 4 * N, rc = rem / N, j = rem - rc * N;
    int slot2 = -1, seen = 0;
#pragma unroll
    for (int sl = 0; sl < 5; ++sl) {
      if (sl == 2 || sl == slot) continue;
      if (seen == which) slot2 = sl;
      ++seen;
    }
    double accv[RPC];
#pragma unroll
    for (int i = 0; i < RPC; ++i) accv[i] = 0.0;
    const int sx = nbr[s * 5 + slot2];
    if (sx >= 0) {
      const int sd2 = slot_to_side(slot2), bit2 = 1 << sd2;
      const double* Ab = AvgSide + ((long)s * 4 + sd2) * nvs * N;
      for (int p = 0; p < ne; ++p) {
        if (!(side_mask[p] & bit2)) continue;
        double w[3];
#pragma unroll
        for (int i = 0; i < 3; ++i) {
          const int pos = ptab[(3 * p + i) * 4 + sd2];
          w[i] = pos >= 0 ? -Ab[(long)pos * N + j] : 0.0;
        }
        const double* K = Ksc + 9 * p;
#pragma unroll
        for (int k = 0; k < 3; ++k) {
          const double y = K[k * 3] * w[0] + K[k * 3 + 1] * w[1] + K[k * 3 + 2] * w[2];
          const double* wa = Wa + (3 * p + k) * LDA + rc * RPC;
#pragma unroll
          for (int i = 0; i < RPC; ++i) accv[i] += wa[i] * y;
        }
      }
    }
#pragma unroll
    for (int i = 0; i < RPC; ++i)
      if (rc * RPC + i < N) G[(long)(slot * N + rc * RPC + i) * W + slot2 * N + j] = accv[i];
  }
}

template <int NTX>
__global__ __launch_bounds__(512) __attribute__((amdgpu_waves_per_eu(NTX <= 3 ? 8 : 6, 8))) void k_thin_nc(Tmpl t, int S, const int* __restrict__ nbr, int N,
                                                 const double* __restrict__ V, const double* __restrict__ ebar,
                                                 const double* __restrict__ AvgSelf, const double* __restrict__ AvgSide,
                                                 double* __restrict__ G_nc) {
  thin_nc_body<NTX>(t, S, nbr, N, V, ebar, AvgSelf, AvgSide, G_nc, blockIdx.x, subdomain_of(t, blockIdx.y));
}

__host__ __device__ inline int fnc_ld(int nvs, int N, int vertex_patch = 0) { return 2 * N + 4 * nvs + (vertex_patch ? N : 0); }
constexpr int NCF_ROWS = 8;

struct ThinNcfArgs {
  const double *V, *ebar, *AvgSelf, *AvgSide;
  const int* nbr;
  double* Fnc;
  int N, S;
};

__device__ __forceinline__ void thin_ncf_body(const Tmpl& t, const ThinNcfArgs& a, int side, int s) {
  extern __shared__ double lds[];
  const int slot = side_to_slot(side), tid = threadIdx.x, N = a.N;
  const int nvs = nvs_of(t), LD = fnc_ld(nvs, N, t.opt_oswald_vertex);
  double* Fs = a.Fnc + ((long)s * 4 + side) * nvs * LD;
  const int s2 = a.nbr[s * 5 + slot];
  if (s2 < 0) {
    for (int i = tid; i < nvs * LD; i += 256) Fs[i] = 0.0;
    return;
  }
  THIN_STAMP(2, 0);
  const int ne = t.touch_count[side];
  double* Y = lds;
  double* Ksc = Y + 3 * t.ntouch * N;
  int* ttab = reinterpret_cast<int*>(Ksc + 9 * t.ntouch);
  int* vtab = ttab + t.ntouch;
  int* ptab = vtab + 3 * t.ntouch;
  int* side_mask = ptab + 12 * t.ntouch;
  int* rlist = side_mask + t.ntouch;
  const double* ebs = a.ebar + (long)s * t.nT;
  for (int i = tid; i < ne; i += 256) {
    ttab[i] = t.touch_elem[side * t.ntouch + i];
    side_mask[i] = t.touch_mask[side * t.ntouch + i];
  }
  static_assert(NCF_ROWS == 8, "layout of t.touch_rlist");
  for (int i = tid; i < nvs * (NCF_ROWS + 1); i += 256) rlist[i] = t.touch_rlist[side * nvs * (NCF_ROWS + 1) + i];
  for (int i = tid; i < 3 * ne; i += 256) vtab[i] = t.touch_vtx[side * t.ntouch * 3 + i];
  for (int i = tid; i < 12 * ne; i += 256) ptab[i] = t.touch_pos[side * t.ntouch * 12 + i];
  for (int i = tid; i < 9 * ne; i += 256) {
    const int T = t.touch_elem[side * t.ntouch + i / 9];
    Ksc[i] = ebs[T] * t.stiff[9 * T + i % 9];
  }
  THIN_STAMP(2, 1);
  __syncthreads();
  THIN_STAMP(2, 2);
  const double* Vs = a.V + (long)s * t.n * N;
  const double* As = a.AvgSelf + (long)s * t.nv * N;
  const int nside = (side == 0 || side == 3) ? t.nvx : t.nvy;
  const double* Aa = a.AvgSide + ((long)s * 4 + side) * nvs * N;
  constexpr int OT = 2;
  double aav[OT];
#pragma unroll
  for (int u = 0; u < OT; ++u) {
    const int it = u * 256 + tid, pos = it / N, j = it - pos * N;
    aav[u] = it < nvs * N && pos < nside ? Aa[(long)pos * N + j] : 0.0;
  }
  auto stage_y = [&](auto wtag) {
    constexpr int W = decltype(wtag)::value;
    using VT = typename VecT<W>::T;
    constexpr int IT = W == 2 ? 3 : 5;
    const int NW = N / W;
    for (int base = 0; base < ne * NW; base += IT * 256) {
      VT vv[IT][3], av[IT][3];
#pragma unroll
      for (int u = 0; u < IT; ++u) {
        const int it = base + u * 256 + tid, itc = it < ne * NW ? it : ne * NW - 1;
        const int p = itc / NW, j = (itc - p * NW) * W, T = ttab[p];
#pragma unroll
        for (int i = 0; i < 3; ++i) {
          vv[u][i] = ldv<W>(Vs + (long)(3 * T + i) * N + j);
          av[u][i] = ldv<W>(As + (long)vtab[3 * p + i] * N + j);
        }
      }
#pragma unroll
      for (int u = 0; u < IT; ++u) {
        const int it = base + u * 256 + tid;
        if (it >= ne * NW) continue;
        const int p = it / NW, j = (it - p * NW) * W;
        VT ws[3];
#pragma unroll
        for (int i = 0; i < 3; ++i) ws[i] = vv[u][i] - av[u][i];
        const double* K = Ksc + 9 * p;
#pragma unroll
        for (int k = 0; k < 3; ++k) stv<W>(Y + (3 * p + k) * N + j, K[k * 3] * ws[0] + K[k * 3 + 1] * ws[1] + K[k * 3 + 2] * ws[2]);
      }
    }
  };
  if (N & 1) stage_y(W1{});
  else stage_y(W2{});
  THIN_STAMP(2, 3);
  __syncthreads();
  THIN_STAMP(2, 4);
  for (int it = tid, u = 0; it < nvs * N; it += 256, ++u) {
    const int pos = it / N, j = it - pos * N;
    double c = 0.0;
    if (pos < nside) {
      const int* rl = rlist + pos * (NCF_ROWS + 1);
      if (rl[0] >= 0) {
        for (int k = 0; k < rl[0]; ++k) c -= Y[rl[1 + k] * N + j];
      } else {
        for (int r = 0; r < 3 * ne; ++r)
          if (ptab[r * 4 + side] == pos) c -= Y[r * N + j];
      }
    }
    Fs[(long)pos * LD + j] = u < OT ? (u == 0 ? aav[0] : aav[1]) : (pos < nside ? Aa[(long)pos * N + j] : 0.0);
    Fs[(long)pos * LD + N + j] = c;
    if (t.opt_oswald_vertex) {
      const bool carries = (side == 0 || side == 3) && (pos == 0 || pos == t.nvx - 1);
      const int corner = (side == 0 ? 0 : 2) + (pos == 0 ? 0 : 1);
      const double* Ac = a.AvgSide + (long)a.S * 4 * nvs * N;
      Fs[(long)pos * LD + 2 * N + 4 * nvs + j] = carries ? Ac[((long)s * 4 + corner) * N + j] : 0.0;
    }
  }
  for (int it = tid; it < nvs * 4 * nvs; it += 256) {
    const int pos = it / (4 * nvs), rem = it - pos * 4 * nvs, sb = rem / nvs, pos2 = rem - sb * nvs;
    double m = 0.0;
    const int ax = side == 0 || side == 3 ? pos : (side == 1 ? 0 : t.nvx - 1), ay = side == 1 || side == 2 ? pos : (side == 0 ? 0 : t.nvy - 1);
    const int bx = sb == 0 || sb == 3 ? pos2 : (sb == 1 ? 0 : t.nvx - 1), by = sb == 1 || sb == 2 ? pos2 : (sb == 0 ? 0 : t.nvy - 1);
    const bool near = ax - bx <= 1 && bx - ax <= 1 && ay - by <= 1 && by - ay <= 1;
    if (pos < nside && near) {
      const int bit = 1 << sb;
      const int* rl = rlist + pos * (NCF_ROWS + 1);
      const int nr = rl[0] >= 0 ? rl[0] : 3 * ne;
      for (int i = 0; i < nr; ++i) {
        const int r = rl[0] >= 0 ? rl[1 + i] : i, p = r / 3, k = r - 3 * p;
        if (!(side_mask[p] & bit) || ptab[r * 4 + side] != pos) continue;
#pragma unroll
        for (int k2 = 0; k2 < 3; ++k2)
          if (ptab[(3 * p + k2) * 4 + sb] == pos2) m += Ksc[9 * p + 3 * k + k2];
      }
    }
    Fs[(long)pos * LD + 2 * N + rem] = m;
  }
  THIN_STAMP(2, 5);
}

__global__ __launch_bounds__(256) void k_thin_ncf(Tmpl t, ThinNcfArgs a) { thin_ncf_body(t, a, blockIdx.x, subdomain_of(t, blockIdx.y)); }

static size_t thin_ncf_lds_bytes(const Tmpl& t, int N) {
  const size_t nvs = (size_t)(t.nvx > t.nvy ? t.nvx : t.nvy);
  return sizeof(double) * (3 * (size_t)t.ntouch * N + 9 * (size_t)t.ntouch) +
         sizeof(int) * (17 * (size_t)t.ntouch + nvs * (NCF_ROWS + 1));
}

struct ThinRtArgs {
  const double *V, *Rself, *Rside, *Bbb, *Aab, *b;
  const int* nbr;
  double *Fside, *r_fd;
  int Q, N, S;
};

__host__ __device__ inline int fside_ld(int Q, int N) { return 4 * Q * N + 4; }

static size_t thin_rt_lds_bytes(const Tmpl& t, int Q, int N) {
  return sizeof(double) * ((size_t)(8 + 3 * Q) * t.ncf + 1 + (size_t)t.ncf * Q * N + 3 * (size_t)t.ncf);
}

__device__ __forceinline__ void thin_rt_body(const Tmpl& t, const ThinRtArgs& a, int side, int s) {
  extern __shared__ double lds[];
  const int slot = side_to_slot(side), tid = threadIdx.x;
  const int Q = a.Q, N = a.N, QN = Q * N, C = 5 * QN, S = a.S, LD = fside_ld(Q, N);
  double* Fs = a.Fside + ((long)s * 4 + side) * t.ncf * LD;
  const int s2 = a.nbr[s * 5 + slot];
  const int np = s2 < 0 ? 0 : t.side_count[side];
  for (int i = tid; i < (t.ncf - np) * LD; i += 256) Fs[(long)np * LD + i] = 0.0;
  if (np == 0) {
    for (int i = tid; i < QN; i += 256) a.r_fd[(long)s * C + slot * QN + i] = 0.0;
    return;
  }
  THIN_STAMP(1, 0);
  double* fco = lds;
  double* sc2 = fco + 4 * np;
  double* Bl = sc2 + np;
  double* Aq = Bl + 3 * np;
  double* Rl = Aq + 3 * Q * np + ((np * (8 + 3 * Q)) & 1);
  int* fidx = reinterpret_cast<int*>(Rl + np * QN);
  const int* nbr_s = a.nbr + s * 5;
  const double* Rs = a.Rself + (long)s * t.nrt * QN;
  const double* Rsd = a.Rside + ((long)s * 4 + side) * t.ncf * QN;
  constexpr int RT_IT = 3;
  double rr[RT_IT];
#pragma unroll
  for (int u = 0; u < RT_IT; ++u) rr[u] = Rsd[u * 256 + tid < np * QN ? u * 256 + tid : 0];
  if (tid < np) {
    const int p = tid;
    const int4* ti4 = reinterpret_cast<const int4*>(t.sface_i + (side * t.ncf + p) * 12);
    const int4 i0 = ti4[0], i1 = ti4[1], i2 = ti4[2];
    const double* td = t.sface_d + (side * t.ncf + p) * 4;
    const double len[3] = {td[0], td[1], td[2]}, area = td[3];
    const int T = i0.x, fp = i0.y;
    const int rt[3] = {i0.z, i0.w, i1.x}, sg[3] = {i1.y, i1.z, i1.w}, bs[3] = {i2.x, i2.y, i2.z};
    const double* be = a.b + (long)s * t.n + 3 * T;
    const double* B = a.Bbb + ((long)s * t.nT + T) * 9 + fp * 3;
    const double b0 = be[0], b1 = be[1], b2 = be[2], B0 = B[0], B1 = B[1], B2 = B[2];
    double Aqv[4][3];
#pragma unroll
    for (int q = 0; q < 4; ++q)
      if (q < Q) {
        const double* A = a.Aab + (((long)q * S + s) * t.nT + T) * 9;
#pragma unroll
        for (int k = 0; k < 3; ++k) Aqv[q][k] = A[k * 3 + fp];
      }
    fidx[p * 5] = T;
    fidx[p * 5 + 1] = fp;
#pragma unroll
    for (int g = 0; g < 3; ++g) {
      fidx[p * 5 + 2 + g] = rt[g];
      const int sign = (bs[g] >= 0 && nbr_s[side_to_slot(bs[g] >= 0 ? bs[g] : 0)] < 0) ? 1 : sg[g];
      fco[p * 4 + g] = sign * len[g] / area;
    }
    fco[p * 4 + 3] = area;
    const double cp = fco[p * 4 + fp];
    sc2[p] = (b0 + b1 + b2) * cp;
    double* row = Fs + (long)p * LD + 4 * QN;
    row[0] = fp == 0 ? B0 : fp == 1 ? B1 : B2;
    row[1] = area * cp * cp;
    row[2] = sc2[p];
    row[3] = 0.0;
    Bl[p * 3] = B0;
    Bl[p * 3 + 1] = B1;
    Bl[p * 3 + 2] = B2;
#pragma unroll
    for (int q = 0; q < 4; ++q)
      if (q < Q)
#pragma unroll
        for (int k = 0; k < 3; ++k) Aq[(p * Q + q) * 3 + k] = Aqv[q][k];
  }
#pragma unroll
  for (int u = 0; u < RT_IT; ++u)
    if (u * 256 + tid < np * QN) Rl[u * 256 + tid] = rr[u];
  for (int i = RT_IT * 256 + tid; i < np * QN; i += 256) Rl[i] = Rsd[i];
  THIN_STAMP(1, 1);
  __syncthreads();
  THIN_STAMP(1, 2);
  auto factor_rows = [&](auto wtag) {
    constexpr int W = decltype(wtag)::value;
    using VT = typename VecT<W>::T;
    constexpr int IT = W == 2 ? 2 : 3;
    const int QW = QN / W;
    for (int base = 0; base < np * QW; base += IT * 256) {
      VT ra[IT], rv[IT][3], xv[IT][3];
#pragma unroll
      for (int u = 0; u < IT; ++u) {
        const int it = base + u * 256 + tid, itc = it < np * QW ? it : np * QW - 1;
        const int p = itc / QW, c = (itc - p * QW) * W, q = c / N, i = c - q * N;
        const int T = fidx[p * 5];
        ra[u] = ldv<W>(Rl + p * QN + c);
#pragma unroll
        for (int g = 0; g < 3; ++g) {
          rv[u][g] = ldv<W>(Rs + (long)fidx[p * 5 + 2 + g] * QN + c);
          xv[u][g] = ldv<W>(a.V + ((long)s * t.n + 3 * T + g) * N + i);
        }
      }
#pragma unroll
      for (int u = 0; u < IT; ++u) {
        const int it = base + u * 256 + tid;
        if (it >= np * QW) continue;
        const int p = it / QW, c = (it - p * QW) * W, q = c / N;
        const int fp = fidx[p * 5 + 1];
        const double area = fco[p * 4 + 3];
        VT yb = zerov<W>(), d = zerov<W>();
#pragma unroll
        for (int g = 0; g < 3; ++g) {
          yb += Bl[p * 3 + g] * rv[u][g];
          d += fco[p * 4 + g] * rv[u][g];
        }
        VT x = zerov<W>();
#pragma unroll
        for (int k = 0; k < 3; ++k) x += xv[u][k] * Aq[(p * Q + q) * 3 + k];
        double* row = Fs + (long)p * LD;
        stv<W>(row + c, ra[u]);
        stv<W>(row + QN + c, yb);
        stv<W>(row + 2 * QN + c, area * fco[p * 4 + fp] * d);
        stv<W>(row + 3 * QN + c, x);
      }
    }
  };
  if (N & 1) factor_rows(W1{});
  else factor_rows(W2{});
  THIN_STAMP(1, 3);
  for (int c = tid; c < QN; c += 256) {
    double v = 0.0;
    for (int p = 0; p < np; ++p) v += sc2[p] * Rl[p * QN + c];
    a.r_fd[(long)s * C + slot * QN + c] = v;
  }
  THIN_STAMP(1, 4);
}

__global__ __launch_bounds__(256) void k_thin_rt(Tmpl t, ThinRtArgs a) { thin_rt_body(t, a, blockIdx.x, subdomain_of(t, blockIdx.y)); }

struct ThinExpandArgs {
  const double* Fside;
  const int* nbr;
  double *G_bb, *G_rdd, *G_ab;
  int Q, N, S;
};

__global__ __launch_bounds__(256) __attribute__((amdgpu_waves_per_eu(6, 8))) void k_thin_expand(Tmpl t, ThinExpandArgs a) {
  extern __shared__ double lds[];
  const int side = blockIdx.x, s = subdomain_of(t, blockIdx.y), slot = side_to_slot(side), tid = threadIdx.x;
  const int Q = a.Q, N = a.N, QN = Q * N, C = 5 * QN, S = a.S, LD = fside_ld(Q, N);
  double* Gb_as = a.G_bb + ((long)s * 9 + 1 + side) * QN * QN;
  double* Gb_aa = a.G_bb + ((long)s * 9 + 5 + side) * QN * QN;
  double* Gd_as = a.G_rdd + ((long)s * 9 + 1 + side) * QN * QN;
  double* Gd_aa = a.G_rdd + ((long)s * 9 + 5 + side) * QN * QN;
  const int s2 = a.nbr[s * 5 + slot];
  const int np = t.side_count[side];
  if (s2 < 0 || np == 0) {
    for (int i = tid; i < QN * QN; i += 256) Gb_as[i] = Gb_aa[i] = Gd_as[i] = Gd_aa[i] = 0.0;
// ... 174 lines not shown
        const int i = base + u * 256 + tid;
        if (i >= KP * NW) continue;
        const int row = i / NW, col = (i - row * NW) * W;
        stv<W>(Xin + row * LD + col, i < K * NW ? xv[u] : zerov<W>());
        stv<W>(Tm + row * LD + col, i < K * NW ? vv[u] : zerov<W>());
        for (int q = 1; q < Q; ++q)
          if (i >= K * NW) stv<W>(Tm + (q * KP + row) * LD + col, zerov<W>());
      }
    }
    THIN_STAMP(0, 1);
    __syncthreads();
    for (int i = tid; i < cnt * NW; i += 256) {
      const int pos = i / NW, col = (i - pos * NW) * W;
      VT v2[3];
#pragma unroll
      for (int k = 0; k < 3; ++k) v2[k] = ldv<W>(Tm + (3 * pos + k) * LD + col);
      for (int q = 0; q < Q; ++q) {
        const double* C = Cl + (q * cnt + pos) * 9;
#pragma unroll
        for (int ii = 0; ii < 3; ++ii)
          stv<W>(Tm + (q * KP + 3 * pos + ii) * LD + col, C[ii * 3] * v2[0] + C[ii * 3 + 1] * v2[1] + C[ii * 3 + 2] * v2[2]);
      }
    }
  };
  if (N & 1) stage(W1{});
  else stage(W2{});
  __syncthreads();
  THIN_STAMP(0, 2);
  for (int q = 0; q < Q; ++q) {
    double* out = B_sys + ((((long)q * S + s) * 5 + slot) * N) * N;
    const double* Tq = Tm + q * KP * LD;
#pragma unroll
    for (int k = 0; k < NT; ++k) {
      const int tile = wave + 4 * k;
      if (tile >= NTX * NTX) continue;
      const int ti = tile / NTX, tj = tile - ti * NTX;
      d4 acc = (d4){0.0, 0.0, 0.0, 0.0};
      for (int k0 = 0; k0 < KP; k0 += 32) {
        double xa[8], yb[8];
#pragma unroll
        for (int u = 0; u < 8; ++u) {
          const int kr = k0 + 4 * u + lk < KP ? k0 + 4 * u + lk : KP - 1;
          xa[u] = Xin[kr * LD + ti * 16 + li];
          yb[u] = Tq[kr * LD + tj * 16 + li];
        }
#pragma unroll
        for (int u = 0; u < 8; ++u)
          if (k0 + 4 * u < KP) acc = __builtin_amdgcn_mfma_f64_16x16x4f64(xa[u], yb[u], acc, 0, 0, 0);
      }
      const int col = tj * 16 + li;
#pragma unroll
      for (int r = 0; r < 4; ++r) {
        const int row = ti * 16 + lk + 4 * r;
        if (row < N && col < N) out[(long)row * N + col] = acc[r];
      }
    }
  }
  THIN_STAMP(0, 3);
}

template <int NTX>
__global__ __launch_bounds__(256) void k_coupling(Tmpl t, int S, const int* __restrict__ nbr, int Q, int N,
                                                  const double* __restrict__ V, const double* __restrict__ A_cpl,
                                                  double* __restrict__ B_sys) {
  coupling_body<NTX>(t, S, nbr, Q, N, V, A_cpl, B_sys, blockIdx.x, subdomain_of(t, blockIdx.y));
}

template <int NTX>
__global__ __launch_bounds__(256) void k_thin3(Tmpl t, ThinRtArgs a, ThinNcfArgs f, const double* __restrict__ A_cpl,
                                               double* __restrict__ B_sys) {
  const int side = blockIdx.x, s = subdomain_of(t, blockIdx.y), z = blockIdx.z;
  if (z == 0)
    coupling_body<NTX>(t, a.S, a.nbr, a.Q, a.N, a.V, A_cpl, B_sys, side, s);
  else if (z == 1)
    thin_rt_body(t, a, side, s);
  else
    thin_ncf_body(t, f, side, s);
}

struct ThinNcArgs {
  const double *ebar, *AvgSelf, *AvgSide, *A_cpl;
  double *G_nc, *B_sys;
  double* Fnc;
};
template <int NTX>
__global__ __launch_bounds__(512) __attribute__((amdgpu_waves_per_eu(NTX <= 3 ? 5 : 4, 8))) void k_thin(Tmpl t, ThinRtArgs a, ThinNcArgs c) {
  const int side = blockIdx.x, s = subdomain_of(t, blockIdx.y);
  if (blockIdx.z == 0 && c.Fnc == nullptr) {
    thin_nc_body<NTX>(t, a.S, a.nbr, a.N, a.V, c.ebar, c.AvgSelf, c.AvgSide, c.G_nc, side, s);
    return;
  }
  if (threadIdx.x >= 256) return;
  if (blockIdx.z == 0) {
    const ThinNcfArgs f{a.V, c.ebar, c.AvgSelf, c.AvgSide, a.nbr, c.Fnc, a.N, a.S};
    thin_ncf_body(t, f, side, s);
    return;
  }
  if (blockIdx.z == 1)
    coupling_body<NTX>(t, a.S, a.nbr, a.Q, a.N, a.V, c.A_cpl, c.B_sys, side, s);
  else
    thin_rt_body(t, a, side, s);
}

inline unsigned grid_for(long total) {
  long g = (total + 255) / 256;
  return (unsigned)(g < 1 ? 1 : (g > 16384 ? 16384 : g));
}

}


int64_t fused_work_size(lrbms_ctx* ctx, int Q, int N) {
  const Tmpl& t = ctx->t;
  const long nvs = t.nvx > t.nvy ? t.nvx : t.nvy;
  return (long)ctx->S * t.nrt * Q * N + (long)ctx->S * 4 * t.ncf * Q * N + (long)ctx->S * t.nv * N + (long)ctx->S * 4 * nvs * N +
         (long)ctx->S * 4 * t.ncf * fside_ld(Q, N) +
         (long)Q * ctx->S * t.nT * 6;
}

int64_t fused_fside_size(lrbms_ctx* ctx, int Q, int N) { return (long)ctx->S * 4 * ctx->t.ncf * fside_ld(Q, N); }

int64_t fused_fnc_size(lrbms_ctx* ctx, int N) {
  const int nvs = ctx->t.nvx > ctx->t.nvy ? ctx->t.nvx : ctx->t.nvy;
  return (long)ctx->S * 4 * nvs * fnc_ld(nvs, N, ctx->t.opt_oswald_vertex);
}

namespace {
__global__ __launch_bounds__(256) void k_build_tables(Tmpl t, double* __restrict__ stiff, int* __restrict__ tvtx,
                                                      int* __restrict__ tpos, int* __restrict__ tmask, int* __restrict__ sfi,
                                                      double* __restrict__ sfd, int* __restrict__ trl) {
  const int i = blockIdx.x * blockDim.x + threadIdx.x;
  const int nvs_b = t.nvx > t.nvy ? t.nvx : t.nvy;
  if (i < 4 * nvs_b) {
    const int sd = i / nvs_b, pos = i - sd * nvs_b;
    int cnt = 0;
    for (int r = 0; r < 3 * t.touch_count[sd]; ++r) {
      const int T = t.touch_elem[sd * t.ntouch + r / 3];
      const int v = t.dof_vertex[3 * T + r % 3], lx = v % t.nvx, ly = v / t.nvx;
      const int ps = sd == 0 ? (ly == 0 ? lx : -1) : sd == 1 ? (lx == 0 ? ly : -1) : sd == 2 ? (lx == t.nvx - 1 ? ly : -1) : (ly == t.nvy - 1 ? lx : -1);
      if (ps == pos) {
        if (cnt < 8) trl[i * 9 + 1 + cnt] = r;
        ++cnt;
      }
    }
    for (int k = cnt; k < 8; ++k) trl[i * 9 + 1 + k] = 0;
    trl[i * 9] = cnt <= 8 ? cnt : -1;
  }
  if (i < 4 * t.ncf) {
    const int sd = i / t.ncf, p = i - sd * t.ncf;
    int* o = sfi + i * 12;
    double* d = sfd + i * 4;
    for (int k = 0; k < 12; ++k) o[k] = 0;
    for (int k = 0; k < 4; ++k) d[k] = 0.0;
    if (p < t.side_count[sd]) {
      const int T = t.side_elem[i];
      int fp = 0;
      for (int f = 0; f < 3; ++f)
        if (t.nb_elem[T * 3 + f] == -(1 + sd)) fp = f;
      o[0] = T;
      o[1] = fp;
      for (int g = 0; g < 3; ++g) {
        const int nb = t.nb_elem[T * 3 + g];
        o[2 + g] = t.elem_rt[T * 3 + g];
        o[5 + g] = t.face_sign[T * 3 + g];
        o[8 + g] = nb < 0 ? -1 - nb : -1;
        d[g] = t.face_len[T * 3 + g];
      }
      d[3] = t.area[T];
    }
  }
  if (i < t.nT) {
    double K[9];
    stiffness3(t, i, K);
    for (int k = 0; k < 9; ++k) stiff[i * 9 + k] = K[k];
    double* mass9 = stiff + 9 * t.nT;
    const double m = t.area[i] * (1.0 / 12.0);
    for (int k = 0; k < 9; ++k) mass9[i * 9 + k] = (k % 4 == 0) ? m + m : m;
// ... 57 lines not shown
  LRBMS_HIP_CHECK(ctx, hipMalloc(&tmask, sizeof(int) * 4 * (size_t)t.ntouch));
  ctx->owned.push_back(tmask);
  int* sfi = nullptr;
  double* sfd = nullptr;
  LRBMS_HIP_CHECK(ctx, hipMalloc(&sfi, sizeof(int) * 48 * (size_t)t.ncf));
  ctx->owned.push_back(sfi);
  LRBMS_HIP_CHECK(ctx, hipMalloc(&sfd, sizeof(double) * 16 * (size_t)t.ncf));
  ctx->owned.push_back(sfd);
  const int nvs_b = t.nvx > t.nvy ? t.nvx : t.nvy;
  int* trl = nullptr;
  LRBMS_HIP_CHECK(ctx, hipMalloc(&trl, sizeof(int) * 36 * (size_t)nvs_b));
  ctx->owned.push_back(trl);
  const int total = std::max(std::max(64, std::max(4 * t.ncf, 4 * nvs_b)), t.nT > 4 * t.ntouch ? t.nT : 4 * t.ntouch);
  hipLaunchKernelGGL(k_build_tables, dim3((total + 255) / 256), dim3(256), 0, nullptr, t, stiff, tvtx, tpos, tmask, sfi, sfd, trl);
  LRBMS_LAUNCH_CHECK(ctx);
  LRBMS_HIP_CHECK(ctx, hipDeviceSynchronize());
  t.stiff = stiff;
  t.mass9 = stiff + 9 * (size_t)t.nT;
  t.zero64 = stiff + 18 * (size_t)t.nT;
  t.lgz = stiff + 27 * (size_t)t.nT + 64;
  t.hab = t.lgz + 6 * (size_t)t.nT;
  t.touch_vtx = tvtx;
  t.touch_pos = tpos;
  t.touch_mask = tmask;
  t.sface_i = sfi;
  t.sface_d = sfd;
  t.touch_rlist = trl;
  return LRBMS_OK;
}

#define LRBMS_F1V_LIST(X) X(2, 2, 1, 3, 0)
static bool f1v_instantiated(int ntx, int Q, const int lv[3]) {
#define LRBMS_F1V_HAS(A, B, C, D, E) if (ntx == A && Q == B && lv[0] == C && lv[1] == D && lv[2] == E) return true;
  LRBMS_F1V_LIST(LRBMS_F1V_HAS)
#undef LRBMS_F1V_HAS
  return false;
}

static bool f1v_layout(std::vector<Grp>& groups, int N, int ntx, int lv[3]) {
  int ns = 0, nu = 0;
  for (Grp& g : groups) {
    g.sym = (g.kind == G_SYS || g.kind == G_ENERGY || g.kind == G_MASS || (g.kind == G_AA && g.q == g.q2)) ? 1 : 0;
    (g.sym ? ns : nu) += 1;
  }
  const int tail = N - 16 * (ntx - 1);
  const int ntail = (ns * tail + 15) / 16, nuns = (nu * N + 15) / 16;
  const int nblock = ns * (ntx - 1), T = nblock + ntail + nuns;
  if (T > 4 * F1_NTY || ntx > 3) return false;
  int si = 0, ui = 0;
  for (Grp& g : groups) {
    if (g.sym) {
      for (int j = 0; j < 4; ++j) g.cb[j] = j < ntx - 1 ? 16 * (j * ns + si) : 16 * nblock + si * tail;
      ++si;
    } else {
      for (int j = 0; j < 4; ++j) g.cb[j] = 16 * (nblock + ntail) + ui * N + 16 * j;
      ++ui;
    }
  }
  lv[0] = lv[1] = lv[2] = 0;
  for (int l = 0; 4 * l < T; ++l) {
    const int k = std::min(4 * l + 3, T - 1);
    lv[(k < nblock ? k / ns + 1 : ntx) - 1] += 1;
  }
  return true;
}

namespace {
__global__ __launch_bounds__(256) void k_wab(Tmpl t, long total, const double* __restrict__ Aab, double* __restrict__ Wab) {
  for (long it = (long)blockIdx.x * 256 + threadIdx.x; it < total; it += (long)gridDim.x * 256) {
    const long blk = it / 6;
    const int k = (int)(it - blk * 6), d = k / 3, f = k - d * 3, T = (int)(blk % t.nT);
    const double* ab = Aab + blk * 9;
    const double* h = t.hab + T * 6 + d * 3;
    Wab[it] = (h[0] * ab[f] + h[1] * ab[3 + f]) + h[2] * ab[6 + f];
  }
}
}
int launch_wab(lrbms_ctx* ctx, int Q, const double* Aab, double* Wab, hipStream_t st) {
  const long total = (long)Q * ctx->S * ctx->t.nT * 6;
  KScope ks(ctx, "k_wab", st);
  hipLaunchKernelGGL(k_wab, dim3(grid_for(total)), dim3(256), 0, st, ctx->t, total, Aab, Wab);
  LRBMS_LAUNCH_CHECK(ctx);
  return LRBMS_OK;
}

static bool f1w_usable(lrbms_ctx* ctx, int Q, int N) { return Q == 2 && N % 2 == 0; }

static bool f1w_layout(std::vector<Grp>& groups, int N, int Q) {
  const int ntx = (N + 15) / 16, tail = N - 32;
  if (Q != 2 || ntx != 3 || N % 2 != 0 || tail < 2 || tail > 8 || groups.size() != 11) return false;
  int s3 = 0, s2 = 0, ui = 0;
  for (Grp& g : groups) {
    g.sym = (g.kind == G_SYS || g.kind == G_ENERGY || g.kind == G_MASS || (g.kind == G_AA && g.q == g.q2)) ? 1 : 0;
    for (int j = 0; j < 4; ++j) g.cb[j] = 0;
    if (g.sym && g.kind != G_AA) {
      g.cb[0] = 16 * s3;
      g.cb[1] = 16 * (4 + s3);
      g.cb[2] = 16 * 8 + s3 * tail;
      ++s3;
    } else if (g.sym) {
      g.cb[0] = 16 * (12 + s2);
      g.cb[1] = 16 * (10 + s2);
      g.cb[2] = 16 * 14 + s2 * tail;
      ++s2;
    } else {
      for (int j = 0; j < 4; ++j) g.cb[j] = g.kind == G_AA ? 16 * (15 + j) : 16 * 18 + (ui - 1) * N + 16 * j;
      if (g.kind == G_AA && ui != 0) return false;
      ++ui;
    }
  }
  return s3 == 4 && s2 == 2 && ui == 5 && 16 * 18 + 4 * N <= 16 * 28;
}

long f1_mfma_per_subdomain(lrbms_ctx* ctx, int Q, int N) {
  const Tmpl& t = ctx->t;
  if (N < 1 || N > 64 || Q < 1 || Q > 4) return 0;
  const int ntx = (N + 15) / 16, ng = Q + 2 + Q * (Q + 1) / 2 + Q * Q, nch = t.nT / EC;
  std::vector<Grp> groups;
  for (int q = 0; q < Q; ++q) groups.push_back({G_SYS, q, 0});
  groups.push_back({G_ENERGY, 0, 0});
  groups.push_back({G_MASS, 0, 0});
  for (int q = 0; q < Q; ++q)
    for (int q2 = q; q2 < Q; ++q2) groups.push_back({G_AA, q, q2});
  for (int q = 0; q < Q; ++q)
    for (int q2 = 0; q2 < Q; ++q2) groups.push_back({G_AB, q, q2});
  const bool one_slice = ng <= std::min(F1_MAXG, (4 * F1_NTY * 16) / N);
  const bool unified = (Q == 1 || Q == 2) && one_slice && ntx <= 3 && ctx->opt_f1_legacy != 1;
  int lv[3] = {0, 0, 0};
  if (unified && ctx->opt_f1_legacy == 0 && f1w_usable(ctx, Q, N) && f1w_layout(groups, N, Q))
    return (long)nch * (150 - 34 + 34 * 2 / 4) + (long)t.nT * 3 * ntx + (long)t.nT * 5 / 4;
  if (unified && ctx->opt_f1_legacy != 2 && N % 2 == 0 && N >= 2 && f1v_layout(groups, N, ntx, lv) && f1v_instantiated(ntx, Q, lv))
    return (long)nch * 3 * 4 * (lv[0] + 2 * lv[1] + 3 * lv[2]) + (long)t.nT * (3 * ntx + Q * ntx);
  const int tiles = (ng * N + 15) / 16;
  return (long)nch * 3 * ntx * tiles + (long)t.nT * 3 * ntx;
}

static size_t thin_nc_lds_bytes(const Tmpl& t, int ntx) {
  const size_t kp = (size_t)((3 * t.ntouch + 3) & ~3);
  return sizeof(double) * (kp * 2 * padded_ld(ntx) + 9 * (size_t)t.ntouch) + sizeof(int) * 17 * (size_t)t.ntouch;
}

bool fused_supported(lrbms_ctx* ctx, int Q, int N, bool factored) {
  const Tmpl& t = ctx->t;
  constexpr size_t LDS_MAX = 160 * 1024;
  if (N > 64 || Q > 4 || Q * N > 128 || t.nT % 8 != 0 || t.ntouch > 256) return false;
  const int ntx = (N + 15) / 16, nr = (Q * N + 15) / 16, nch = t.nT / EC;
  const int ngroups = Q + 2 + Q * (Q + 1) / 2 + Q * Q;
  const bool unified = (Q == 1 || Q == 2) && ntx <= 3 && ngroups <= std::min(F1_MAXG, (4 * F1_NTY * 16) / N);
  if (unified) {
    int ks = 1;
    while (72 * (size_t)(t.nT / ks) > 56 * 1024 && nch % (4 * ks) == 0) ks *= 2;
    if (72 * (size_t)(t.nT / ks) > 56 * 1024) return false;
  } else if (96 * (size_t)t.nT > 48 * 1024) {
    return false;
  }
  static const size_t f2_static[8] = {12288, 28672, 28672, 45056, 45056, 61440, 61440, 77824};
  if (44 * (size_t)t.nT + f2_static[nr - 1] > LDS_MAX) return false;
  if (coupling_lds_bytes(t, ntx, Q) > LDS_MAX) return false;
  if (factored) return thin_ncf_lds_bytes(t, N) <= LDS_MAX;
  if (thin_nc_lds_bytes(t, ntx) > LDS_MAX || t.ntouch * N > 3 * 512) return false;
  if ((size_t)t.ncf * fside_ld(Q, N) * sizeof(double) > LDS_MAX) return false;
  return true;
}

static hipError_t raise_max_lds(int device, const void* fn, int bytes) {
  static std::mutex mu;
  static std::map<std::pair<int, const void*>, int> raised;
  std::lock_guard<std::mutex> lock(mu);
  int& cur = raised[{device, fn}];
  if (cur >= bytes) return hipSuccess;
  const hipError_t e = hipFuncSetAttribute(fn, hipFuncAttributeMaxDynamicSharedMemorySize, bytes);
  if (e == hipSuccess) cur = bytes;
  return e;
}

int launch_project_estimate_fused(lrbms_ctx* ctx, int Q, int N, const double* V, const double* F, const double* A_diag,
                                  const double* A_cpl, const double* P_diag, const double* b, const double* ebar,
                                  const double* caa, const double* Aab, const double* Bbb, double* work, double* B_sys,
                                  double* rhs_red, double* E_red, double* M_red, double* G_nc, double* r_fd, double* G_rdd,
                                  double* G_bb, double* G_ab, double* G_aa, double* Fside, double* Fnc, int phase,
                                  hipStream_t st) {
  if (!fused_supported(ctx, Q, N, Fside != nullptr))
    return lrbms_fail(ctx, LRBMS_E_INVALID, "fused pass: unsupported N / Q / template size for this output layout");
  if (phase < 0 || phase > 5) return lrbms_fail(ctx, LRBMS_E_INVALID, "fused pass: phase must be 0 .. 5");
  if (phase == 5 && st == ctx->aux[0])
    return lrbms_fail(ctx, LRBMS_E_INVALID, "fused pass: phase 5 runs its halo-dependent half on library stream 0; the caller's stream must be another one");
  ctx->pass_ran = true;
  const bool both = phase == 5;
  const bool do_prep = phase == 0 || phase == 1 || phase == 3 || both;
  const bool do_a = phase == 0 || phase == 1 || phase == 4 || both;
  const bool do_b = phase == 0 || phase == 2 || both;
  Tmpl t = ctx->t;
  t.sub_list = ctx->subset_n > 0 ? ctx->subset : nullptr;
  t.sub_count = ctx->subset_n;
  const int S = ctx->S, QN = Q * N, C = 5 * QN;
  const int Sg = t.sub_list ? t.sub_count : S;
  const long nvs = t.nvx > t.nvy ? t.nvx : t.nvy;
  double* Rself = work;
  double* Rside = Rself + (long)S * t.nrt * QN;
  double* AvgSelf = Rside + (long)S * 4 * t.ncf * QN;
  double* AvgSide = AvgSelf + (long)S * t.nv * N;
  const bool factored = Fside != nullptr;
  if (factored != (Fnc != nullptr)) return lrbms_fail(ctx, LRBMS_E_INVALID, "fused pass: F_side and F_nc go together");
  if (t.opt_oswald_vertex && !factored)
    return lrbms_fail(ctx, LRBMS_E_INVALID, "LRBMS_OPT_OSWALD_VERTEX_PATCH: the diagonal subdomains enter through the factored layout "
                                            "only (F_nc)");
  if (t.opt_oswald_vertex && ctx->S_ext != ctx->S && !ctx->diag_explicit)
    return lrbms_fail(ctx, LRBMS_E_INVALID, "LRBMS_OPT_OSWALD_VERTEX_PATCH on a sharded grid: the diagonal subdomains must be halo "
                                            "slabs named by lrbms_set_diagonal_neighbours");
  if (!factored) Fside = AvgSide + (long)S * 4 * nvs * N;
  const long gstride = factored ? (long)QN * QN : (long)9 * QN * QN;
  const int abld = factored ? QN : C;
  const int aboff = factored ? 0 : 2 * QN;
  const bool forked = ctx->opt_streams >= 0 ? ctx->opt_streams != 0 : Sg < 192;
  const int gy_flux = (t.nrt * N + 255) / 256, gy_vtx = (t.nv * N + 255) / 256;
  const bool merge_thin = forked || factored;
  const int ntx_p = (N + 15) / 16;
  const bool prep_ok = ctx->opt_prep_lds != 0 && N % 2 == 0;
  const bool gnc_fold = prep_ok && ctx->opt_prep_lds != 2 && ntx_p <= 3 && prep_lds_bytes(t, Q, N, true) <= 160 * 1024;
  const size_t prep_lds = prep_lds_bytes(t, Q, N, gnc_fold);
  const bool prep_from_lds = prep_ok && prep_lds <= 160 * 1024;
  bool side_from_lds = false;
  const double* Wab = nullptr;
  bool f1w_ok = false;
  if (ctx->opt_f1_legacy == 0 && do_a) {
    std::vector<Grp> probe;
    for (int i = 0; i < 11; ++i) probe.push_back({i < 2 ? G_SYS : i == 2 ? G_ENERGY : i == 3 ? G_MASS : i < 7 ? G_AA : G_AB, i == 6 ? 1 : 0, i == 5 || i == 6 ? 1 : 0});
    f1w_ok = Q == 2 && f1w_layout(probe, N, Q);
    if (f1w_ok) {
      if (ctx->wab != nullptr && ctx->wab_src == Aab && ctx->wab_Q == Q) {
        Wab = ctx->wab;
      } else {
        double* wloc = AvgSide + (long)S * 4 * nvs * N + (long)S * 4 * t.ncf * fside_ld(Q, N);
        if (int rc = launch_wab(ctx, Q, Aab, wloc, st)) return rc;
        Wab = wloc;
      }
    }
  }
  if (do_prep) {
    if (prep_from_lds) {
      KScope ks(ctx, "k_prep_lds", st);
      if (ctx->num_cus == 0) {
        int ncu = 0;
        LRBMS_HIP_CHECK(ctx, hipDeviceGetAttribute(&ncu, hipDeviceAttributeMultiprocessorCount, ctx->device));
        ctx->num_cus = ncu > 0 ? ncu : 256;
      }
      const int prep_parts = 2 * Sg <= ctx->num_cus ? 2 : 1;
      const GncArgs ga{ebar, gnc_fold ? G_nc : nullptr, factored ? (long)N * N : (long)25 * N * N, factored ? N : 5 * N,
                       factored ? 0 : 10 * N * N + 2 * N};
      const size_t prep_lds_p = prep_lds_bytes_persistent(t, Q, N, gnc_fold);
      const bool persist = prep_parts == 1 && Sg > ctx->num_cus && ctx->opt_prep_lds != 3 && prep_lds_p <= 160 * 1024 && gnc_fold &&
                           7 * ((t.nT / 2 + 7) / 8) < t.nT / 2 &&
                           (size_t)t.n * (N / 2) <= 8 * (size_t)PREP_LDS_THREADS && (size_t)Q * t.nrt * 3 <= 2 * (size_t)PREP_LDS_THREADS &&
                           (size_t)Q * S * t.nrt * 48 < ((size_t)1 << 31);
      const size_t lds_used = persist ? prep_lds_p : prep_lds;
      const int gx = persist ? ctx->num_cus : Sg;
#define LRBMS_PREP(NTXV)                                                                                                              \
  do {                                                                                                                                \
    LRBMS_HIP_CHECK(ctx, raise_max_lds(ctx->device, (const void*)k_prep_lds<NTXV>, (int)lds_used));                                   \
    hipLaunchKernelGGL(k_prep_lds<NTXV>, dim3(gx, prep_parts), dim3(PREP_LDS_THREADS), lds_used, st, t, S, ctx->nbr, Q, N, F, V, Rself, Rside, AvgSelf, \
                       AvgSide, phase == 0 ? 1 : 0, ga, persist ? 1 : 0);                                                             \
  } while (0)
      if (ntx_p == 1) LRBMS_PREP(1);
      else if (ntx_p == 2) LRBMS_PREP(2);
      else LRBMS_PREP(3);
#undef LRBMS_PREP
    } else {
      {
        KScope ks(ctx, "k_flux_compact", st);
        hipLaunchKernelGGL(k_flux_compact, dim3(Sg, gy_flux), dim3(256), 0, st, t, S, ctx->nbr, Q, N, F, V, Rself, Rside,
                           phase == 0 ? 1 : 0);
      }
      KScope ks(ctx, "k_vertex_avg", st);
      hipLaunchKernelGGL(k_vertex_avg, dim3(Sg, gy_vtx), dim3(256), 0, st, t, S, ctx->nbr, N, V, AvgSelf, AvgSide,
                         phase == 0 ? 1 : 0);
    }
  }
  auto side_prep = [&](hipStream_t ss) -> int {
    if (prep_from_lds && prep_lds_bytes(t, Q, N, false) - prep_lds_slab_bytes(t, N, false) <= 64 * 1024) {
      side_from_lds = true;
      KScope ks(ctx, "k_prep_lds<side>", ss);
      const GncArgs ga{ebar, nullptr, 0, 0, 0};
      const size_t side_lds = prep_lds_bytes(t, Q, N, false) - prep_lds_slab_bytes(t, N, false);
      hipLaunchKernelGGL((k_prep_lds<1, 256>), dim3(Sg, 1), dim3(256), side_lds, ss, t, S, ctx->nbr, Q, N, F, V, Rself, Rside, AvgSelf,
                         AvgSide, 2, ga, 0);
    } else {
      {
        KScope ks(ctx, "k_flux_side", ss);
        hipLaunchKernelGGL(k_flux_side, dim3(grid_for((long)Sg * 4 * t.ncf * N)), dim3(256), 0, ss, t, S, ctx->nbr, Q, N, F, V, Rside);
      }
      if (merge_thin) {
        KScope ks(ctx, "k_vertex_side", ss);
        hipLaunchKernelGGL(k_vertex_side, dim3(grid_for((long)Sg * 4 * nvs * N)), dim3(256), 0, ss, t, S, ctx->nbr, N, V, AvgSide);
      }
    }
    return LRBMS_OK;
  };
  if (phase == 2) {
    LRBMS_HIP_CHECK(ctx, hipStreamWaitEvent(st, ctx->prep_done ? ctx->prep_done : ctx->ev_prep, 0));
    if (int rc = side_prep(st)) return rc;
  }
  LRBMS_LAUNCH_CHECK(ctx);
  const bool multi = (do_a || do_b) && forked;
  hipStream_t s_rt = multi || both ? ctx->aux[0] : st, s_f23 = multi ? ctx->aux[1] : st, s_nc = multi || both ? ctx->aux[0] : st;
  hipStream_t s_f3 = multi ? ctx->aux[0] : st;
  const bool f3_runs = do_a && !(prep_from_lds && gnc_fold);
  const bool use_aux[3] = {(both || (multi && (do_b || f3_runs))) && ctx->aux[0] != st, multi && do_a && ctx->aux[1] != st, false};
  const bool forks = use_aux[0] || use_aux[1] || use_aux[2];
  if (forks) {
    LRBMS_HIP_CHECK(ctx, hipEventRecord(ctx->ev_fork, st));
    for (int i = 0; i < 3; ++i)
      if (use_aux[i]) LRBMS_HIP_CHECK(ctx, hipStreamWaitEvent(ctx->aux[i], ctx->ev_fork, 0));
  }
  if (phase == 1 || phase == 3) {
    if (!forks) LRBMS_HIP_CHECK(ctx, hipEventRecord(ctx->ev_prep, st));
    ctx->prep_done = forks ? ctx->ev_fork : ctx->ev_prep;
  }

  std::vector<Grp> groups;
  if (do_a) {
  for (int q = 0; q < Q; ++q) groups.push_back({G_SYS, q, 0, N, B_sys + ((long)q * S * 5 + 2) * N * N, nullptr, (long)5 * N * N});
// ... 35 lines not shown
      const int nch = t.nT / EC;
      int ksplit = 1;
      if (lean) {
        const int want = ctx->opt_f1_ksplit > 0 ? ctx->opt_f1_ksplit : (S <= 64 ? 2 : 1);
        while (ksplit < want && nch % (4 * ksplit) == 0) ksplit *= 2;
      } else if (unified) {
        const int want = ctx->opt_f1_ksplit > 0 ? ctx->opt_f1_ksplit : (S <= 64 ? 2 : 1);
        while (ksplit < want && nch % (4 * ksplit) == 0) ksplit *= 2;
        while (72 * (size_t)(t.nT / ksplit) > 56 * 1024 && nch % (4 * ksplit) == 0) ksplit *= 2;
        if (72 * (size_t)(t.nT / ksplit) > 56 * 1024)
          return lrbms_fail(ctx, LRBMS_E_INVALID, "fused pass: template too large for k_f1u");
      } else {
        const bool split_ok = nch % 4 == 0;
        ksplit = split_ok && (ctx->opt_f1_ksplit > 0 ? ctx->opt_f1_ksplit == 2 : 4 * S * nsl <= 256) ? 2 : 1;
      }
      if (ksplit > 1 && unified) {
        const long need = (long)S * ksplit * (lean ? f1v_part_size(ntx) : f1u_part_size(ntx));
        if (ctx->ksp_part_cap < need) {
          if (ctx->ksp_part) LRBMS_HIP_CHECK(ctx, hipFree(ctx->ksp_part));
          ctx->ksp_part = nullptr;
          ctx->ksp_part_cap = 0;
          LRBMS_HIP_CHECK(ctx, hipMalloc(&ctx->ksp_part, sizeof(double) * (size_t)need));
          ctx->ksp_part_cap = need;
        }
        if (ctx->ksp_ticket_cap < S) {
          if (ctx->ksp_ticket) LRBMS_HIP_CHECK(ctx, hipFree(ctx->ksp_ticket));
          ctx->ksp_ticket = nullptr;
          ctx->ksp_ticket_cap = 0;
          LRBMS_HIP_CHECK(ctx, hipMalloc(&ctx->ksp_ticket, sizeof(int) * (size_t)S));
          LRBMS_HIP_CHECK(ctx, hipMemset(ctx->ksp_ticket, 0, sizeof(int) * (size_t)S));
          ctx->ksp_ticket_cap = S;
        }
        a.part = ctx->ksp_part;
        a.ticket = ctx->ksp_ticket;
      }
      if (ksplit > 1 && !unified) {
        for (int sl = 0; sl < nsl; ++sl)
          hipLaunchKernelGGL(k_f1_zero, dim3(Sg), dim3(256), 0, st, gt[sl], S, N, sl == 0 ? a.rhs_red : nullptr, t.sub_list);
      }
      const dim3 grid(Sg, nsl, ksplit);
      KScope ks(ctx, lean2 ? "k_f1w" : lean ? "k_f1v" : unified ? "k_f1u" : "k_f1", st);
      if (lean2) {
        hipLaunchKernelGGL(k_f1w, grid, dim3(512), 0, st, t, a, gt[0], Wab);
        LRBMS_LAUNCH_CHECK(ctx);
        continue;
      }
      if (lean) {
#define LRBMS_F1V(A, B, C, D, E)                                               \
  if (ntx == A && Q == B && lv[0] == C && lv[1] == D && lv[2] == E)            \
    hipLaunchKernelGGL((k_f1v<A, B, C, D, E>), grid, dim3(512), 0, st, t, a, gt[0]);
        LRBMS_F1V_LIST(LRBMS_F1V)
#undef LRBMS_F1V
        LRBMS_LAUNCH_CHECK(ctx);
        continue;
      }
      const size_t ldsf1u = sizeof(double) * 9 * (t.nT / ksplit);
#define LRBMS_F1(NTXV)                                                                                              \
  do {                                                                                                              \
    if (Q == 1 && unified) hipLaunchKernelGGL((k_f1u<NTXV, 1>), grid, dim3(512), ldsf1u, st, t, a, gt[0]);            \
    else if (Q == 2 && unified) hipLaunchKernelGGL((k_f1u<NTXV, 2>), grid, dim3(512), ldsf1u, st, t, a, gt[0]);       \
    else if (Q == 1 && one_slice) hipLaunchKernelGGL((k_f1<NTXV, NTY, 1>), grid, dim3(512), ldsf1, st, t, a, gt[0], gt[1], gt[2]); \
    else if (Q == 2 && one_slice) hipLaunchKernelGGL((k_f1<NTXV, NTY, 2>), grid, dim3(512), ldsf1, st, t, a, gt[0], gt[1], gt[2]); \
    else hipLaunchKernelGGL((k_f1<NTXV, NTY, 0>), grid, dim3(512), ldsf1, st, t, a, gt[0], gt[1], gt[2]);             \
  } while (0)
      switch (ntx) {
        case 1: LRBMS_F1(1); break;
        case 2: LRBMS_F1(2); break;
        case 3: LRBMS_F1(3); break;
        default:
          if (Q == 1 && one_slice) hipLaunchKernelGGL((k_f1<4, NTY, 1>), grid, dim3(512), ldsf1, st, t, a, gt[0], gt[1], gt[2]);
          else if (Q == 2 && one_slice) hipLaunchKernelGGL((k_f1<4, NTY, 2>), grid, dim3(512), ldsf1, st, t, a, gt[0], gt[1], gt[2]);
          else hipLaunchKernelGGL((k_f1<4, NTY, 0>), grid, dim3(512), ldsf1, st, t, a, gt[0], gt[1], gt[2]);
          break;
      }
#undef LRBMS_F1
      LRBMS_LAUNCH_CHECK(ctx);
    }
  }
  }
  if (both)
    if (int rc = side_prep(ctx->aux[0])) return rc;
  if (do_b && merge_thin) {
    const int ntx = (N + 15) / 16;
    ThinRtArgs a{V, Rself, Rside, Bbb, Aab, b, ctx->nbr, Fside, r_fd, Q, N, S};
    ThinNcArgs c{ebar, AvgSelf, AvgSide, A_cpl, G_nc, B_sys, Fnc};
    size_t lds = factored ? thin_ncf_lds_bytes(t, N) : thin_nc_lds_bytes(t, ntx);
    lds = std::max(lds, thin_rt_lds_bytes(t, Q, N));
    lds = std::max(lds, coupling_lds_bytes(t, ntx, Q));
#define LRBMS_THIN(NTX)                                                                                                      \
  do {                                                                                                                       \
    if (lds > 64 * 1024)                                                                                                     \
      LRBMS_HIP_CHECK(ctx, hipFuncSetAttribute((const void*)k_thin<NTX>, hipFuncAttributeMaxDynamicSharedMemorySize, (int)lds)); \
    hipLaunchKernelGGL(k_thin<NTX>, dim3(4, Sg, 3), dim3(512), lds, s_rt, t, a, c);                                           \
  } while (0)
#define LRBMS_THIN3(NTX)                                                                                                     \
  do {                                                                                                                       \
    if (lds > 64 * 1024)                                                                                                     \
      LRBMS_HIP_CHECK(ctx, hipFuncSetAttribute((const void*)k_thin3<NTX>, hipFuncAttributeMaxDynamicSharedMemorySize, (int)lds)); \
    hipLaunchKernelGGL(k_thin3<NTX>, dim3(4, Sg, 3), dim3(256), lds, s_rt, t, a, f, A_cpl, B_sys);                            \
  } while (0)
    if (factored) {
      const ThinNcfArgs f{V, ebar, AvgSelf, AvgSide, ctx->nbr, Fnc, N, S};
      KScope ks(ctx, "k_thin3", s_rt);
      switch (ntx) {
        case 1: LRBMS_THIN3(1); break;
        case 2: LRBMS_THIN3(2); break;
        case 3: LRBMS_THIN3(3); break;
        default: LRBMS_THIN3(4); break;
      }
    } else {
      KScope ks(ctx, "k_thin", s_rt);
      switch (ntx) {
        case 1: LRBMS_THIN(1); break;
        case 2: LRBMS_THIN(2); break;
        case 3: LRBMS_THIN(3); break;
        default: LRBMS_THIN(4); break;
      }
    }
#undef LRBMS_THIN3
#undef LRBMS_THIN
    LRBMS_LAUNCH_CHECK(ctx);
    if (!factored) {
      ThinExpandArgs e{Fside, ctx->nbr, G_bb, G_rdd, G_ab, Q, N, S};
      const size_t lds3 = sizeof(double) * (size_t)t.ncf * fside_ld(Q, N);
      KScope ks(ctx, "k_thin_expand", s_rt);
      hipLaunchKernelGGL(k_thin_expand, dim3(4, Sg), dim3(256), lds3, s_rt, t, e);
      LRBMS_LAUNCH_CHECK(ctx);
    }
  }
  if (do_b && !merge_thin) {
    hipStream_t side = s_nc;
    if (phase != 0 && !side_from_lds) {
      KScope ks(ctx, "k_vertex_side", side);
      hipLaunchKernelGGL(k_vertex_side, dim3(grid_for((long)Sg * 4 * nvs * N)), dim3(256), 0, side, t, S, ctx->nbr, N, V, AvgSide);
    }
    const int ntx = (N + 15) / 16;
    if (factored) {
      const ThinNcfArgs f{V, ebar, AvgSelf, AvgSide, ctx->nbr, Fnc, N, S};
      const size_t ldsf = thin_ncf_lds_bytes(t, N);
      if (ldsf > 64 * 1024)
        LRBMS_HIP_CHECK(ctx, hipFuncSetAttribute((const void*)k_thin_ncf, hipFuncAttributeMaxDynamicSharedMemorySize, (int)ldsf));
      KScope ks(ctx, "k_thin_ncf", side);
      hipLaunchKernelGGL(k_thin_ncf, dim3(4, Sg), dim3(256), ldsf, side, t, f);
    } else {
    const size_t lds = thin_nc_lds_bytes(t, ntx);
#define LRBMS_THIN_NC(NTX)                                                                                                       \
  do {                                                                                                                           \
    if (lds > 64 * 1024)                                                                                                         \
      LRBMS_HIP_CHECK(ctx, hipFuncSetAttribute((const void*)k_thin_nc<NTX>, hipFuncAttributeMaxDynamicSharedMemorySize, (int)lds)); \
    hipLaunchKernelGGL(k_thin_nc<NTX>, dim3(4, Sg), dim3(512), lds, side, t, S, ctx->nbr, N, V, ebar, AvgSelf, AvgSide, G_nc);    \
  } while (0)
    {
    KScope ks(ctx, "k_thin_nc", side);
    switch (ntx) {
      case 1: LRBMS_THIN_NC(1); break;
      case 2: LRBMS_THIN_NC(2); break;
      case 3: LRBMS_THIN_NC(3); break;
      default: LRBMS_THIN_NC(4); break;
    }
    }
#undef LRBMS_THIN_NC
    }
    LRBMS_LAUNCH_CHECK(ctx);
    ThinRtArgs a{V, Rself, Rside, Bbb, Aab, b, ctx->nbr, Fside, r_fd, Q, N, S};
    const size_t lds2 = thin_rt_lds_bytes(t, Q, N);
    {
      KScope ks(ctx, "k_thin_rt", s_rt);
      hipLaunchKernelGGL(k_thin_rt, dim3(4, Sg), dim3(256), lds2, s_rt, t, a);
    }
    LRBMS_LAUNCH_CHECK(ctx);
    if (!factored) {
      ThinExpandArgs e{Fside, ctx->nbr, G_bb, G_rdd, G_ab, Q, N, S};
      const size_t lds3 = sizeof(double) * (size_t)t.ncf * fside_ld(Q, N);
      KScope ks(ctx, "k_thin_expand", s_rt);
      hipLaunchKernelGGL(k_thin_expand, dim3(4, Sg), dim3(256), lds3, s_rt, t, e);
      LRBMS_LAUNCH_CHECK(ctx);
    }
  }
  const int nr2 = (QN + 15) / 16;
  static const size_t f2g_static[8] = {f2g_static_lds_bytes<1>(), f2g_static_lds_bytes<2>(), f2g_static_lds_bytes<3>(), f2g_static_lds_bytes<4>(),
                                       f2g_static_lds_bytes<5>(), f2g_static_lds_bytes<6>(), f2g_static_lds_bytes<7>(), f2g_static_lds_bytes<8>()};
  const bool f2_gram = (ctx->opt_f2_form == 0 || ctx->opt_f2_form == 2) && f2g_dyn_lds_bytes(t) + f2g_static[nr2 - 1] <= 160 * 1024;
  const bool f2_pair = ctx->opt_f2_form == 0 && QN % 2 == 0 && (reinterpret_cast<uintptr_t>(Rself) & 15) == 0 && 8L * t.nrt * QN < (1L << 31);
  if (do_a && f2_gram) {
    F2Args a{Rself, Bbb, b, ctx->nbr, G_bb, G_rdd, r_fd, Q, N, S, gstride};
    const size_t ldsf2 = f2g_dyn_lds_bytes(t);
#define LRBMS_F2G_P(NRV, PV)                                                                                                \
  do {                                                                                                                       \
    LRBMS_HIP_CHECK(ctx, raise_max_lds(ctx->device, (const void*)k_f2g<NRV, PV>, (int)ldsf2));                              \
    hipLaunchKernelGGL((k_f2g<NRV, PV>), dim3(Sg), dim3(64 * (F2_NCW + EC)), ldsf2, s_f23, t, a);                             \
  } while (0)
#define LRBMS_F2G(NRV)                                                                                                      \
  do {                                                                                                                       \
    if (f2_pair) LRBMS_F2G_P(NRV, 1);                                                                                        \
    else LRBMS_F2G_P(NRV, 0);                                                                                                \
  } while (0)
    KScope ks(ctx, "k_f2", s_f23);
    switch (nr2) {
      case 1: LRBMS_F2G(1); break;
      case 2: LRBMS_F2G(2); break;
      case 3: LRBMS_F2G(3); break;
      case 4: LRBMS_F2G(4); break;
      case 5: LRBMS_F2G(5); break;
      case 6: LRBMS_F2G(6); break;
      case 7: LRBMS_F2G(7); break;
      default: LRBMS_F2G(8); break;
    }
#undef LRBMS_F2G
#undef LRBMS_F2G_P
    LRBMS_LAUNCH_CHECK(ctx);
  }
  if (do_a && !f2_gram) {
    F2Args a{Rself, Bbb, b, ctx->nbr, G_bb, G_rdd, r_fd, Q, N, S, gstride};
    const int nr = nr2;
    const size_t ldsf2 = sizeof(double) * 4 * t.nT + sizeof(int) * 3 * t.nT;
#define LRBMS_F2(NRV)                                                                                                       \
  do {                                                                                                                       \
    if (ldsf2 > 64 * 1024)                                                                                                   \
      LRBMS_HIP_CHECK(ctx, hipFuncSetAttribute((const void*)k_f2<NRV>, hipFuncAttributeMaxDynamicSharedMemorySize, (int)ldsf2)); \
    hipLaunchKernelGGL(k_f2<NRV>, dim3(Sg), dim3(64 * (F2_NCW + EC)), ldsf2, s_f23, t, a);                                    \
  } while (0)
    KScope ks(ctx, "k_f2", s_f23);
    switch (nr) {
      case 1: LRBMS_F2(1); break;
      case 2: LRBMS_F2(2); break;
      case 3: LRBMS_F2(3); break;
      case 4: LRBMS_F2(4); break;
      case 5: LRBMS_F2(5); break;
      case 6: LRBMS_F2(6); break;
      case 7: LRBMS_F2(7); break;
      default: LRBMS_F2(8); break;
    }
#undef LRBMS_F2
    LRBMS_LAUNCH_CHECK(ctx);
  }
  if (do_a && !(prep_from_lds && gnc_fold)) {
    F3Args a{V, ebar, AvgSelf, AvgSide, G_nc, N, S, factored ? (long)N * N : 25L * N * N, factored ? N : 5 * N,
             factored ? 0 : 10 * N * N + 2 * N};
    const int ntx = (N + 15) / 16;
    KScope ks(ctx, "k_f3", s_f3);
    switch (ntx) {
      case 1: hipLaunchKernelGGL(k_f3<1>, dim3(Sg), dim3(256), 0, s_f3, t, a); break;
      case 2: hipLaunchKernelGGL(k_f3<2>, dim3(Sg), dim3(256), 0, s_f3, t, a); break;
      case 3: hipLaunchKernelGGL(k_f3<3>, dim3(Sg), dim3(256), 0, s_f3, t, a); break;
      default: hipLaunchKernelGGL(k_f3<4>, dim3(Sg), dim3(256), 0, s_f3, t, a); break;
    }
    LRBMS_LAUNCH_CHECK(ctx);
// ... 28 lines not shown
```

pylrbms_amd/csrc/lrbms_dev.h:

```cpp
#pragma once
#include <hip/hip_runtime.h>
#include <stdint.h>
#include <string>
#include <vector>

#include "lrbms_ctx_base.h"

struct Tmpl {
  int kx, ky, nT, n, nrt, nv, nvx, nvy, ncf;
  double hx, hy;
  double kappa[4], kinv[4], kmin;
  const int *nb_elem, *nb_face, *nb_elem_out, *nb_face_out, *elem_side_pos, *elem_rt, *face_sign;
  const int *dof_vertex, *vdof_ptr, *vdof_idx;
  const int *rt_e0, *rt_f0, *rt_e1, *rt_f1, *rt_side;
  const int *side_elem, *side_elem_out, *side_count;
  int ntouch;
  const int *touch_elem, *touch_count;
  const double *grad, *area, *normal, *face_len, *points;
  const double* stiff;
  const double* mass9;
  const double* zero64;
  const double* lgz;
  const double* hab;
  const int* touch_vtx;
  const int* touch_pos;
  const int* touch_mask;
  const int* touch_rlist;
  const int* sface_i;
  const double* sface_d;
  int opt_oswald_subdomain;
  int opt_oswald_vertex;
  int opt_accumulate_coupling;
  const int* sub_list;
  int sub_count;
  const int* nbr_diag;
};

__device__ inline int subdomain_of(const Tmpl& t, int b) { return t.sub_list ? t.sub_list[b] : b; }

struct lrbms_ctx : lrbms_ctx_base {
  int num_cus = 0;
  Tmpl t{};
  int S = 0, S_ext = 0;
  int* nbr = nullptr;
  std::vector<int32_t> nbr_host;
  hipEvent_t ev_prep = nullptr;
  hipEvent_t prep_done = nullptr;
  void* blas = nullptr;
  double* coarse = nullptr;
  long coarse_cap = 0;
  double* ksp_part = nullptr;
  long ksp_part_cap = 0;
  int* ksp_ticket = nullptr;
  long ksp_ticket_cap = 0;
  double* wab = nullptr;
  long wab_cap = 0;
  const double* wab_src = nullptr;
  int wab_Q = 0;
  bool pass_ran = false;
  bool diag_explicit = false;
  int* subset = nullptr;
  int subset_n = 0, subset_cap = 0;
  lrbms_quadrature* qdev = nullptr;
  int opt_streams = -1, opt_f1_ksplit = 0, opt_f1_legacy = 0, opt_coarse = 1, opt_solve_valu = 0, opt_estimate_valu = 0, opt_prep_lds = 1, opt_f2_form = 0;
  double* src_phi = nullptr;
  const double* user_pc = nullptr;
  int user_pc_N = 0;
};

#define SIGMA_INNER 8.0
#define SIGMA_BOUNDARY 14.0

__host__ __device__ inline int side_to_slot(int side) { return side < 2 ? side : side + 1; }
__host__ __device__ inline int slot_to_side(int slot) { return slot < 2 ? slot : slot - 1; }

int build_template_tables(lrbms_ctx* ctx);
int launch_wab(lrbms_ctx* ctx, int Q, const double* Aab, double* Wab, hipStream_t st);
long f1_mfma_per_subdomain(lrbms_ctx* ctx, int Q, int N);
int coarse_begin(lrbms_ctx* ctx, double** A0_out, hipStream_t st);
int coarse_finish(lrbms_ctx* ctx, const double** A0inv_out, hipStream_t st);
int launch_coarse_apply(lrbms_ctx* ctx, int N, int nmu, const double* A0inv, const double* r, double* z, double* prz, hipStream_t st);

int launch_assemble_swipdg(lrbms_ctx*, int Q, const double* lam, double* A_diag, double* A_cpl, hipStream_t);
int launch_assemble_rhs(lrbms_ctx*, const double* f_smp, const double* lhat, double* b, double* f2, double* ceps, hipStream_t);
int launch_assemble_products(lrbms_ctx*, int Q, const double* theta_bar_dev, const double* lam, const double* lam_df,
                             const double* lbar, const double* lhat, double* P_diag, double* ebar, double* caa, double* Aab,
                             double* Bbb, hipStream_t);
int launch_assemble_flux(lrbms_ctx*, int Q, const double* lam, double* F, hipStream_t);
int launch_oswald(lrbms_ctx*, int N, const double* V, double* Wt, hipStream_t);
int launch_flux(lrbms_ctx*, int Q, int N, const double* F, const double* V, double* Rt, hipStream_t);
int launch_blockell_apply(lrbms_ctx*, int S, int M, const double* A, long sA, const double* x, double* y, hipStream_t);
int launch_fom_apply(lrbms_ctx*, int Q, int M, const double* theta, const double* A_diag, const double* A_cpl,
                     const double* x, double* y, hipStream_t);
int launch_gemm_tn(lrbms_ctx*, int batch, int K, int Mx, int My, const double* X, long sx, int ldx, const double* Y,
                   long sy, int ldy, double* G, long sg, int ldg, const double* rowscale, double alpha, hipStream_t);
int launch_project_system(lrbms_ctx*, int Q, int N, const double* V, const double* A_diag, const double* A_cpl,
                          const double* P_diag, const double* b, double* work, double* B_sys, double* rhs_red,
                          double* E_red, double* M_red, hipStream_t);
int launch_estimator_grams(lrbms_ctx*, int Q, int N, const double* V, const double* Wt, const double* Rt,
                           const double* ebar, const double* caa, const double* Aab, const double* Bbb, const double* b,
                           double* work, double* G_nc, double* r_fd, double* G_rdd, double* G_bb, double* G_ab,
                           double* G_aa, hipStream_t);
int launch_reduced_estimate(lrbms_ctx*, int Q, int N, const double* theta_dev, const double* u, const double* G_nc,
                            const double* r_fd, const double* G_rdd, const double* G_bb, const double* G_ab,
                            const double* G_aa, const double* Fside, const double* Fnc, const double* f2, const double* ceps,
                            double hdiam, double* eta_loc, hipStream_t);
int launch_reduced_solve(lrbms_ctx*, int Q, int N, const double* theta, const double* B_sys, const double* rhs_red,
                         double* work, double* u, double rtol, int max_iter, double* info, hipStream_t);
```

pylrbms_amd/sources.py:

```python
import numpy as np


def source_components(p):
    f = p['f']
    if not isinstance(f, dict):
        return None
    funcs, coeffs = list(f['functions']), list(f['coefficients'])
    if len(funcs) != len(coeffs) or not funcs:
        raise ValueError("p['f'] needs as many coefficients as functions (and at least one)")
    if len(funcs) == 1 and not hasattr(coeffs[0], 'evaluate') and coeffs[0] == 1:
        return None
    return funcs, coeffs


def coefficient_parameter_type(c):
    if not hasattr(c, 'evaluate'):
        return {}
    if hasattr(c, 'factors'):
        out = {}
        for fac in c.factors:
            out.update(coefficient_parameter_type(fac))
        return out
    return dict(getattr(c, 'parameter_type', None) or {})


def check_coefficients(coeffs, parameter_type):
    for j, c in enumerate(coeffs):
        for k, shape in coefficient_parameter_type(c).items():
            if k == '_t' and k not in parameter_type:
                raise NotImplementedError('source coefficient {} depends on the time (_t): a time-dependent source needs the '
                                          'parabolic discretize'.format(j))
            if k not in parameter_type or tuple(parameter_type[k]) != tuple(shape):
                raise ValueError("source coefficient {} reads the parameter {!r} of shape {}, which p['parameter_type'] = {} does "
                                 'not contain'.format(j, k, tuple(shape), dict(parameter_type)))


def evaluate_coefficients(coeffs, mu):
    return np.array([c.evaluate(mu) if hasattr(c, 'evaluate') else float(c) for c in coeffs], dtype=np.float64)


def local_estimates(engine, U, theta, src, rows):
    import torch
    eng, c = engine, engine.ctx
    zero_f2 = c.zeros(eng.S)
    out = []
    for c0 in range(0, U.shape[2], 16):
        V = U[:, :, c0:c0 + 16].contiguous()
        L = V.shape[2]
        buf = eng.project_and_estimate(V, project_system=False)
        grams = list(buf['grams'])
        grams[1] = torch.zeros_like(grams[1])
        u = torch.eye(L, dtype=V.dtype, device=V.device).expand(eng.S, L, L).contiguous()
        eta = c.reduced_estimate_batch(np.tile(theta, (L, 1)), u, tuple(grams), zero_f2, eng.ceps, eng.hdiam)
        if rows is not None:
            D = c.div_apply(c.flux_reconstruct(eng.F, V), mode=0)
            _, r_fd_K = c.project_sources(eng.Q, src['b_K'], V, D)
            r = rows[c0:c0 + L]
            eta[1] += c.reduced_source_terms(theta, r.contiguous() if hasattr(r, 'contiguous') else np.ascontiguousarray(r), src['F2'],
                                             r_fd_K, u, eng.ceps, eng.hdiam)
        out.append(eta)
    eta = torch.cat(out, dim=2)
    return eta[0], eta[1], eta[2]


def setup_sources(engine, funcs, coeffs):
    import torch
    from pylrbms_amd.engine import sample_function, volume_record_points
    eng = engine
    sp = eng.quadrature
    xf, cl, kl = volume_record_points(eng.grid, eng.local, (sp.rhs, sp.f2))
    f_smp_K = eng.ctx.from_numpy(np.ascontiguousarray(np.stack([sample_function(fn, xf, cl, kl) for fn in funcs])))
    b_K = torch.stack([eng.ctx.assemble_rhs(f_smp_K[j].contiguous(), eng.lhat)[0] for j in range(len(funcs))]).contiguous()
    F2 = eng.ctx.assemble_source_gram(f_smp_K)
    return {'functions': funcs, 'coefficients': coeffs, 'K': len(funcs), 'f_smp_K': f_smp_K, 'b_K': b_K, 'F2': F2}
```

Before: 1.721 million subdomains/s.

## Precompute per-subdomain side tables at assembly and reuse them across estimator passes

Adds a k_side_tables kernel that builds, once at assembly time, the per-side stiffness-scaled tables (ktab, mtab) and the RT face records, which the thin NCF and RT kernels used to rebuild on every project+estimate call. Assembled arrays are tracked by pointer and generation counter so the cached tables are rebuilt only when the inputs change. The thin kernels now load the precomputed tables instead of gathering ebar, Bbb, Aab and b and running the mask-matching loop. The cost is extra device memory, bookkeeping, and a risk of stale tables if an array is changed in place without being reassembled.

```diff
diff --git a/include/lrbms_hip.h b/include/lrbms_hip.h
--- a/include/lrbms_hip.h
+++ b/include/lrbms_hip.h
@@ -87,6 +87,8 @@
                             const double* lbar, const double* lhat, double* P_diag, double* ebar, double* caa, double* Aab,
                             double* Bbb, void* stream);
 
+int32_t lrbms_assembled_arrays(lrbms_ctx* ctx, int32_t kind, const double** out, int32_t cap);
+
 int lrbms_assemble_flux(lrbms_ctx* ctx, int32_t Q, const double* lam, double* F, void* stream);
 
 int lrbms_oswald_apply(lrbms_ctx* ctx, int32_t N, const double* V, double* Wt, void* stream);
@@ -129,6 +131,7 @@
 #define LRBMS_OPT_ESTIMATE_VALU 8
 #define LRBMS_OPT_PREP_LDS 10
 #define LRBMS_OPT_F2_FORM 11
+#define LRBMS_OPT_SIDE_TABLES 12
 int lrbms_ctx_set_option(lrbms_ctx* ctx, int32_t option, int32_t value);
 
 int lrbms_set_diagonal_neighbours(lrbms_ctx* ctx, const int32_t* nbr_diag);
diff --git a/pylrbms_amd/_native.py b/pylrbms_amd/_native.py
--- a/pylrbms_amd/_native.py
+++ b/pylrbms_amd/_native.py
@@ -79,6 +79,7 @@
     'lrbms_reduced_time_residual_work_size': (c_i64, [c_vp, c_i32]),
     'lrbms_reduced_time_residual': (ctypes.c_int, [c_vp, c_i32, c_i32, c_i32, _P_DBL, c_vp, c_vp, c_vp, c_vp, c_vp, c_vp]),
     'lrbms_assemble_source_gram': (ctypes.c_int, [c_vp, c_i32, c_vp, c_vp, c_vp]),
+    'lrbms_assembled_arrays': (c_i32, [c_vp, c_i32, ctypes.POINTER(c_vp), c_i32]),
     'lrbms_fom_implicit_euler_src': (ctypes.c_int, [c_vp, c_i32, c_i32, _P_DBL, c_dbl, c_i32, c_vp, c_vp, c_vp, c_vp, c_vp, c_vp,
                                                     c_dbl, c_i32, _P_DBL, c_vp]),
     'lrbms_reduced_implicit_euler_src': (ctypes.c_int, [c_vp, c_i32, c_i32, c_i32, _P_DBL, c_dbl, c_i32, c_vp, c_vp, c_vp, c_vp, c_vp,
@@ -225,7 +226,8 @@
     _load = staticmethod(load_library)
     OPTIONS = {'oswald_zero_on_subdomain_boundary': 1, 'accumulate_coupling_across_q': 2, 'oswald_vertex_patch': 9, 'prep_lds': 10,
                'streams': 3, 'f1_ksplit': 4, 'f1_form': 5, 'coarse': 6, 'solve_valu': 7, 'estimate_valu': 8,
-               'f2_form': 11}
+               'f2_form': 11,
+               'side_tables': 12}
     S = S_ext = None
     _keep = None
 
@@ -255,6 +257,7 @@
         rc = self.lib.lrbms_mesh_upload(self.handle, ctypes.byref(d), S, S_ext, _i32p(nb))
         self._keep = (arrs, nb)
         self._check(rc, 'lrbms_mesh_upload')
+        self._pins = {}
 
     def set_quadrature(self, spec):
         from pylrbms_amd.quadrature import native_quadrature
@@ -276,24 +279,45 @@
         self._check(rc, 'lrbms_assemble_swipdg')
         return A_diag, A_cpl
 
-    def assemble_rhs(self, f_smp, lhat):
+    def _out(self, out, shapes):
+        if out is None:
+            return tuple(self.empty(*shape) for shape in shapes)
+        assert len(out) == len(shapes)
+        for x, shape in zip(out, shapes):
+            self._ptr(x, shape, 'out')
+        return tuple(out)
+
+    def _pin_assembled(self, written):
+        pins = self.__dict__.setdefault('_pins', {})
+        for kind, x in written.items():
+            pins[(kind, x.data_ptr())] = x
+        cap = 64
+        buf = (c_vp * cap)()
+        live = set()
+        for kind in range(4):
+            n = self.lib.lrbms_assembled_arrays(self.handle, kind, buf, cap)
+            if n < 0 or n > cap:
+                raise NativeError('lrbms_assembled_arrays: {}'.format(n))
+            live.update((kind, int(buf[i] or 0)) for i in range(n))
+        for key in [k for k in pins if k not in live]:
+            del pins[key]
+
+    def assemble_rhs(self, f_smp, lhat, out=None):
         qd = self._quad()
-        b, f2, ceps = self.empty(self.S, self.n), self.empty(self.S), self.empty(self.S)
+        b, f2, ceps = self._out(out, [(self.S, self.n), (self.S,), (self.S,)])
         rc = self.lib.lrbms_assemble_rhs(self.handle, self._ptr(f_smp, (self.S, self.n_T, qd.f_stride), 'f_smp'),
                                          self._ptr(lhat, (self.S, self.n_T, qd.lhat_stride), 'lhat'), c_vp(b.data_ptr()),
                                          c_vp(f2.data_ptr()), c_vp(ceps.data_ptr()), self._stream())
         self._check(rc, 'lrbms_assemble_rhs')
+        self._pin_assembled({2: b})
         return b, f2, ceps
 
-    def assemble_products(self, theta_bar, lam, lam_df, lbar, lhat):
+    def assemble_products(self, theta_bar, lam, lam_df, lbar, lhat, out=None):
         Q, qd = lam.shape[0], self._quad()
         th = np.ascontiguousarray(theta_bar, dtype=np.float64)
         assert th.shape == (Q,)
-        P_diag = self.empty(self.S, self.n_T, 4, 9)
-        ebar = self.empty(self.S, self.n_T)
-        caa = self.empty(Q, Q, self.S, self.n_T)
-        Aab = self.empty(Q, self.S, self.n_T, 3, 3)
-        Bbb = self.empty(self.S, self.n_T, 3, 3)
+        P_diag, ebar, caa, Aab, Bbb = self._out(out, [(self.S, self.n_T, 4, 9), (self.S, self.n_T), (Q, Q, self.S, self.n_T),
+                                                      (Q, self.S, self.n_T, 3, 3), (self.S, self.n_T, 3, 3)])
         rc = self.lib.lrbms_assemble_products(
             self.handle, Q, _dblp(th), self._ptr(lam, (Q, self.S_ext, self.n_T, qd.lam_stride), 'lam'),
             self._ptr(lam_df, (Q, self.S, self.n_T, qd.lamdf_stride), 'lam_df'),
@@ -301,6 +325,7 @@
             c_vp(P_diag.data_ptr()), c_vp(ebar.data_ptr()), c_vp(caa.data_ptr()), c_vp(Aab.data_ptr()),
             c_vp(Bbb.data_ptr()), self._stream())
         self._check(rc, 'lrbms_assemble_products')
+        self._pin_assembled({0: Bbb, 1: Aab, 3: ebar})
         return P_diag, ebar, caa, Aab, Bbb
 
     def assemble_flux(self, lam):
diff --git a/pylrbms_amd/csrc/assemble.hip b/pylrbms_amd/csrc/assemble.hip
--- a/pylrbms_amd/csrc/assemble.hip
+++ b/pylrbms_amd/csrc/assemble.hip
@@ -460,7 +460,8 @@
   if (!ctx->qdev) return lrbms_fail(ctx, LRBMS_E_STATE, "quadrature not set (lrbms_set_quadrature)");
   hipLaunchKernelGGL(k_assemble_rhs, dim3(ctx->S), dim3(256), 0, st, ctx->t, ctx->qdev, f_smp, lhat, b, f2, ceps);
   LRBMS_LAUNCH_CHECK(ctx);
-  return LRBMS_OK;
+  note_assembled(ctx, lrbms_ctx::SRC_B, b);
+  return side_tables_after_assembly(ctx, true, st);
 }
 
 int launch_assemble_products(lrbms_ctx* ctx, int Q, const double* theta_bar, const double* lam, const double* lam_df,
@@ -473,6 +474,10 @@
   hipLaunchKernelGGL(k_assemble_products, dim3((unsigned)((total + 255) / 256)), dim3(256), 0, st, ctx->t, ctx->qdev, ctx->S,
                      ctx->S_ext, ctx->nbr, Q, tb, lam, lam_df, lbar, lhat, P_diag, ebar, caa, Aab, Bbb);
   LRBMS_LAUNCH_CHECK(ctx);
+  note_assembled(ctx, lrbms_ctx::SRC_BBB, Bbb);
+  note_assembled(ctx, lrbms_ctx::SRC_AAB, Aab);
+  note_assembled(ctx, lrbms_ctx::SRC_EBAR, ebar);
+  ctx->asm_Q = Q;
   const long need = (long)Q * ctx->S * ctx->t.nT * 6;
   if (ctx->wab_cap < need) {
     if (ctx->wab) LRBMS_HIP_CHECK(ctx, hipFree(ctx->wab));
@@ -485,7 +490,8 @@
   if (int rc = launch_wab(ctx, Q, Aab, ctx->wab, st)) return rc;
   ctx->wab_src = Aab;
   ctx->wab_Q = Q;
-  return LRBMS_OK;
+  ctx->wab_gen = asm_gen_of(ctx, lrbms_ctx::SRC_AAB, Aab);
+  return side_tables_after_assembly(ctx, false, st);
 }
 
 int launch_assemble_flux(lrbms_ctx* ctx, int Q, const double* lam, double* F, hipStream_t st) {
diff --git a/pylrbms_amd/csrc/capi.hip b/pylrbms_amd/csrc/capi.hip
--- a/pylrbms_amd/csrc/capi.hip
+++ b/pylrbms_amd/csrc/capi.hip
@@ -197,6 +197,7 @@
   if (ctx->ksp_ticket) (void)hipFree(ctx->ksp_ticket);
   if (ctx->subset) (void)hipFree(ctx->subset);
   if (ctx->wab) (void)hipFree(ctx->wab);
+  if (ctx->stab) (void)hipFree(ctx->stab);
   if (ctx->src_phi) (void)hipFree(ctx->src_phi);
   lrbms_ctx_base_release(ctx);
   if (ctx->ev_prep) (void)hipEventDestroy(ctx->ev_prep);
@@ -235,6 +236,7 @@
     case LRBMS_OPT_SOLVE_VALU: ctx->opt_solve_valu = value; break;
     case LRBMS_OPT_ESTIMATE_VALU: ctx->opt_estimate_valu = value; break;
     case LRBMS_OPT_PREP_LDS: ctx->opt_prep_lds = value; break;
+    case LRBMS_OPT_SIDE_TABLES: ctx->opt_side_tables = value; break;
     default: return lrbms_fail(ctx, LRBMS_E_INVALID, "set_option: unknown option");
   }
   return LRBMS_OK;
@@ -369,7 +371,7 @@
     ctx->diag_explicit = false;
   }
   ctx->subset_n = 0;
-  ctx->wab_src = nullptr;
+  forget_assembled(ctx);
   ctx->pass_ran = false;
   ctx->S = S;
   ctx->S_ext = S_ext;
@@ -434,6 +436,13 @@
   LRBMS_REQUIRE_MESH(ctx); CHECK_Q_N(ctx, Q, 1); CHECK_PTR(ctx, theta_bar); CHECK_PTR(ctx, lam); CHECK_PTR(ctx, lam_df); CHECK_PTR(ctx, lbar);
   CHECK_PTR(ctx, lhat); CHECK_PTR(ctx, P_diag); CHECK_PTR(ctx, ebar); CHECK_PTR(ctx, caa); CHECK_PTR(ctx, Aab); CHECK_PTR(ctx, Bbb);
   return launch_assemble_products(ctx, Q, theta_bar, lam, lam_df, lbar, lhat, P_diag, ebar, caa, Aab, Bbb, (hipStream_t)stream);
+}
+
+int32_t lrbms_assembled_arrays(lrbms_ctx* ctx, int32_t kind, const double** out, int32_t cap) {
+  if (!ctx || kind < 0 || kind >= lrbms_ctx::SRC_COUNT || cap < 0 || (cap > 0 && !out)) return -1;
+  const std::vector<lrbms_ctx::AsmRec>& known = ctx->asm_known[kind];
+  for (int32_t i = 0; i < cap && i < (int32_t)known.size(); ++i) out[i] = known[(size_t)i].p;
+  return (int32_t)known.size();
 }
 
 int lrbms_assemble_flux(lrbms_ctx* ctx, int32_t Q, const double* lam, double* F, void* stream) {
diff --git a/pylrbms_amd/csrc/fused.hip b/pylrbms_amd/csrc/fused.hip
--- a/pylrbms_amd/csrc/fused.hip
+++ b/pylrbms_amd/csrc/fused.hip
@@ -3382,11 +3382,48 @@
 constexpr int NCF_ROWS = 8;
 
 struct ThinNcfArgs {
-  const double *V, *ebar, *AvgSelf, *AvgSide;
+  const double *V, *AvgSelf, *AvgSide;
   const int* nbr;
   double* Fnc;
   int N, S;
+  const double *ktab = nullptr, *mtab = nullptr;
 };
+
+__device__ inline void ncf_side_tables(const Tmpl& t, const double* __restrict__ ebar, int s, int side, int tid, int nthreads,
+                                       double* ksc, double* __restrict__ mab) {
+  const int nvs = nvs_of(t), ne = t.touch_count[side];
+  const int nside = (side == 0 || side == 3) ? t.nvx : t.nvy;
+  const double* ebs = ebar + (long)s * t.nT;
+  const int* telem = t.touch_elem + side * t.ntouch;
+  const int* side_mask = t.touch_mask + side * t.ntouch;
+  const int* ptab = t.touch_pos + side * t.ntouch * 12;
+  const int* rlist = t.touch_rlist + side * nvs * (NCF_ROWS + 1);
+  for (int i = tid; i < 9 * t.ntouch; i += nthreads) {
+    const int T = telem[i < 9 * ne ? i / 9 : 0];
+    ksc[i] = i < 9 * ne ? ebs[T] * t.stiff[9 * T + i % 9] : 0.0;
+  }
+  __syncthreads();
+  for (int it = tid; it < nvs * 4 * nvs; it += nthreads) {
+    const int pos = it / (4 * nvs), rem = it - pos * 4 * nvs, sb = rem / nvs, pos2 = rem - sb * nvs;
+    double m = 0.0;
+    const int ax = side == 0 || side == 3 ? pos : (side == 1 ? 0 : t.nvx - 1), ay = side == 1 || side == 2 ? pos : (side == 0 ? 0 : t.nvy - 1);
+    const int bx = sb == 0 || sb == 3 ? pos2 : (sb == 1 ? 0 : t.nvx - 1), by = sb == 1 || sb == 2 ? pos2 : (sb == 0 ? 0 : t.nvy - 1);
+    const bool near = ax - bx <= 1 && bx - ax <= 1 && ay - by <= 1 && by - ay <= 1;
+    if (pos < nside && near) {
+      const int bit = 1 << sb;
+      const int* rl = rlist + pos * (NCF_ROWS + 1);
+      const int nr = rl[0] >= 0 ? rl[0] : 3 * ne;
+      for (int i = 0; i < nr; ++i) {
+        const int r = rl[0] >= 0 ? rl[1 + i] : i, p = r / 3, k = r - 3 * p;
+        if (!(side_mask[p] & bit) || ptab[r * 4 + side] != pos) continue;
+#pragma unroll
+        for (int k2 = 0; k2 < 3; ++k2)
+          if (ptab[(3 * p + k2) * 4 + sb] == pos2) m += ksc[9 * p + 3 * k + k2];
+      }
+    }
+    mab[it] = m;
+  }
+}
 
 __device__ __forceinline__ void thin_ncf_body(const Tmpl& t, const ThinNcfArgs& a, int side, int s) {
   extern __shared__ double lds[];
@@ -3407,19 +3444,19 @@
   int* ptab = vtab + 3 * t.ntouch;
   int* side_mask = ptab + 12 * t.ntouch;
   int* rlist = side_mask + t.ntouch;
-  const double* ebs = a.ebar + (long)s * t.nT;
-  for (int i = tid; i < ne; i += 256) {
-    ttab[i] = t.touch_elem[side * t.ntouch + i];
-    side_mask[i] = t.touch_mask[side * t.ntouch + i];
-  }
+  const double* kt = a.ktab + ((long)s * 4 + side) * 9 * t.ntouch;
+  const double* mt = a.mtab + ((long)s * 4 + side) * 4 * nvs * nvs;
+  constexpr int MT = 2;
+  double mv[MT];
+#pragma unroll
+  for (int u = 0; u < MT; ++u) mv[u] = mt[u * 256 + tid < 4 * nvs * nvs ? u * 256 + tid : 0];
+  (void)side_mask;
+  for (int i = tid; i < ne; i += 256) ttab[i] = t.touch_elem[side * t.ntouch + i];
   static_assert(NCF_ROWS == 8, "layout of t.touch_rlist");
   for (int i = tid; i < nvs * (NCF_ROWS + 1); i += 256) rlist[i] = t.touch_rlist[side * nvs * (NCF_ROWS + 1) + i];
   for (int i = tid; i < 3 * ne; i += 256) vtab[i] = t.touch_vtx[side * t.ntouch * 3 + i];
   for (int i = tid; i < 12 * ne; i += 256) ptab[i] = t.touch_pos[side * t.ntouch * 12 + i];
-  for (int i = tid; i < 9 * ne; i += 256) {
-    const int T = t.touch_elem[side * t.ntouch + i / 9];
-    Ksc[i] = ebs[T] * t.stiff[9 * T + i % 9];
-  }
+  for (int i = tid; i < 9 * ne; i += 256) Ksc[i] = kt[i];
   THIN_STAMP(2, 1);
   __syncthreads();
   THIN_STAMP(2, 2);
@@ -3491,25 +3528,9 @@
       Fs[(long)pos * LD + 2 * N + 4 * nvs + j] = carries ? Ac[((long)s * 4 + corner) * N + j] : 0.0;
     }
   }
-  for (int it = tid; it < nvs * 4 * nvs; it += 256) {
-    const int pos = it / (4 * nvs), rem = it - pos * 4 * nvs, sb = rem / nvs, pos2 = rem - sb * nvs;
-    double m = 0.0;
-    const int ax = side == 0 || side == 3 ? pos : (side == 1 ? 0 : t.nvx - 1), ay = side == 1 || side == 2 ? pos : (side == 0 ? 0 : t.nvy - 1);
-    const int bx = sb == 0 || sb == 3 ? pos2 : (sb == 1 ? 0 : t.nvx - 1), by = sb == 1 || sb == 2 ? pos2 : (sb == 0 ? 0 : t.nvy - 1);
-    const bool near = ax - bx <= 1 && bx - ax <= 1 && ay - by <= 1 && by - ay <= 1;
-    if (pos < nside && near) {
-      const int bit = 1 << sb;
-      const int* rl = rlist + pos * (NCF_ROWS + 1);
-      const int nr = rl[0] >= 0 ? rl[0] : 3 * ne;
-      for (int i = 0; i < nr; ++i) {
-        const int r = rl[0] >= 0 ? rl[1 + i] : i, p = r / 3, k = r - 3 * p;
-        if (!(side_mask[p] & bit) || ptab[r * 4 + side] != pos) continue;
-#pragma unroll
-        for (int k2 = 0; k2 < 3; ++k2)
-          if (ptab[(3 * p + k2) * 4 + sb] == pos2) m += Ksc[9 * p + 3 * k + k2];
-      }
-    }
-    Fs[(long)pos * LD + 2 * N + rem] = m;
+  for (int it = tid, u = 0; it < nvs * 4 * nvs; it += 256, ++u) {
+    const int pos = it / (4 * nvs), rem = it - pos * 4 * nvs;
+    Fs[(long)pos * LD + 2 * N + rem] = u < MT ? (u == 0 ? mv[0] : mv[1]) : mt[it];
   }
   THIN_STAMP(2, 5);
 }
@@ -3523,11 +3544,55 @@
 }
 
 struct ThinRtArgs {
-  const double *V, *Rself, *Rside, *Bbb, *Aab, *b;
+  const double *V, *Rself, *Rside;
   const int* nbr;
   double *Fside, *r_fd;
   int Q, N, S;
+  const double* rec = nullptr;
 };
+
+constexpr int RTREC_LD = 28;
+__device__ inline void rt_side_record(const Tmpl& t, const int* __restrict__ nbr, const double* __restrict__ Bbb, const double* __restrict__ Aab,
+                                      const double* __restrict__ b, int Q, int S, int s, int side, int p, double* __restrict__ rec) {
+  const int* nbr_s = nbr + s * 5;
+  const int4* ti4 = reinterpret_cast<const int4*>(t.sface_i + (side * t.ncf + p) * 12);
+  const int4 i0 = ti4[0], i1 = ti4[1], i2 = ti4[2];
+  const double* td = t.sface_d + (side * t.ncf + p) * 4;
+  const double len[3] = {td[0], td[1], td[2]}, area = td[3];
+  const int T = i0.x, fp = i0.y;
+  const int rt[3] = {i0.z, i0.w, i1.x}, sg[3] = {i1.y, i1.z, i1.w}, bs[3] = {i2.x, i2.y, i2.z};
+  const double* be = b + (long)s * t.n + 3 * T;
+  const double* B = Bbb + ((long)s * t.nT + T) * 9 + fp * 3;
+  const double b0 = be[0], b1 = be[1], b2 = be[2], B0 = B[0], B1 = B[1], B2 = B[2];
+  int* ri = reinterpret_cast<int*>(rec);
+  ri[0] = T;
+  ri[1] = fp;
+  double fco[4];
+#pragma unroll
+  for (int g = 0; g < 3; ++g) {
+    ri[2 + g] = rt[g];
+    const int sign = (bs[g] >= 0 && nbr_s[side_to_slot(bs[g] >= 0 ? bs[g] : 0)] < 0) ? 1 : sg[g];
+    fco[g] = sign * len[g] / area;
+  }
+  ri[5] = ri[6] = ri[7] = 0;
+  fco[3] = area;
+  const double cp = fp == 0 ? fco[0] : fp == 1 ? fco[1] : fco[2];
+  const double sc2 = (b0 + b1 + b2) * cp;
+#pragma unroll
+  for (int g = 0; g < 4; ++g) rec[4 + g] = fco[g];
+  rec[8] = sc2;
+  rec[9] = B0;
+  rec[10] = B1;
+  rec[11] = B2;
+  rec[12] = fp == 0 ? B0 : fp == 1 ? B1 : B2;
+  rec[13] = area * cp * cp;
+  rec[14] = sc2;
+  rec[15] = 0.0;
+#pragma unroll
+  for (int q = 0; q < 4; ++q)
+#pragma unroll
+    for (int k = 0; k < 3; ++k) rec[16 + q * 3 + k] = q < Q ? Aab[(((long)q * S + s) * t.nT + T) * 9 + k * 3 + fp] : 0.0;
+}
 
 __host__ __device__ inline int fside_ld(int Q, int N) { return 4 * Q * N + 4; }
 
@@ -3538,7 +3603,7 @@
 __device__ __forceinline__ void thin_rt_body(const Tmpl& t, const ThinRtArgs& a, int side, int s) {
   extern __shared__ double lds[];
   const int slot = side_to_slot(side), tid = threadIdx.x;
-  const int Q = a.Q, N = a.N, QN = Q * N, C = 5 * QN, S = a.S, LD = fside_ld(Q, N);
+  const int Q = a.Q, N = a.N, QN = Q * N, C = 5 * QN, LD = fside_ld(Q, N);
   double* Fs = a.Fside + ((long)s * 4 + side) * t.ncf * LD;
   const int s2 = a.nbr[s * 5 + slot];
   const int np = s2 < 0 ? 0 : t.side_count[side];
@@ -3554,7 +3619,6 @@
   double* Aq = Bl + 3 * np;
   double* Rl = Aq + 3 * Q * np + ((np * (8 + 3 * Q)) & 1);
   int* fidx = reinterpret_cast<int*>(Rl + np * QN);
-  const int* nbr_s = a.nbr + s * 5;
   const double* Rs = a.Rself + (long)s * t.nrt * QN;
   const double* Rsd = a.Rside + ((long)s * 4 + side) * t.ncf * QN;
   constexpr int RT_IT = 3;
@@ -3563,47 +3627,36 @@
   for (int u = 0; u < RT_IT; ++u) rr[u] = Rsd[u * 256 + tid < np * QN ? u * 256 + tid : 0];
   if (tid < np) {
     const int p = tid;
-    const int4* ti4 = reinterpret_cast<const int4*>(t.sface_i + (side * t.ncf + p) * 12);
-    const int4 i0 = ti4[0], i1 = ti4[1], i2 = ti4[2];
-    const double* td = t.sface_d + (side * t.ncf + p) * 4;
-    const double len[3] = {td[0], td[1], td[2]}, area = td[3];
-    const int T = i0.x, fp = i0.y;
-    const int rt[3] = {i0.z, i0.w, i1.x}, sg[3] = {i1.y, i1.z, i1.w}, bs[3] = {i2.x, i2.y, i2.z};
-    const double* be = a.b + (long)s * t.n + 3 * T;
-    const double* B = a.Bbb + ((long)s * t.nT + T) * 9 + fp * 3;
-    const double b0 = be[0], b1 = be[1], b2 = be[2], B0 = B[0], B1 = B[1], B2 = B[2];
-    double Aqv[4][3];
-#pragma unroll
-    for (int q = 0; q < 4; ++q)
-      if (q < Q) {
-        const double* A = a.Aab + (((long)q * S + s) * t.nT + T) * 9;
-#pragma unroll
-        for (int k = 0; k < 3; ++k) Aqv[q][k] = A[k * 3 + fp];
-      }
-    fidx[p * 5] = T;
-    fidx[p * 5 + 1] = fp;
-#pragma unroll
-    for (int g = 0; g < 3; ++g) {
-      fidx[p * 5 + 2 + g] = rt[g];
-      const int sign = (bs[g] >= 0 && nbr_s[side_to_slot(bs[g] >= 0 ? bs[g] : 0)] < 0) ? 1 : sg[g];
-      fco[p * 4 + g] = sign * len[g] / area;
-    }
-    fco[p * 4 + 3] = area;
-    const double cp = fco[p * 4 + fp];
-    sc2[p] = (b0 + b1 + b2) * cp;
+    const d2* r2 = reinterpret_cast<const d2*>(a.rec + (((long)s * 4 + side) * t.ncf + p) * RTREC_LD);
+    const int4* ri4 = reinterpret_cast<const int4*>(r2);
+    const int4 i0 = ri4[0], i1 = ri4[1];
+    d2 rc[8], ra[6];
+#pragma unroll
+    for (int k = 2; k < 8; ++k) rc[k] = r2[k];
+#pragma unroll
+    for (int k = 0; k < 6; ++k)
+      if (2 * k < 3 * Q) ra[k] = r2[8 + k];
+    fidx[p * 5] = i0.x;
+    fidx[p * 5 + 1] = i0.y;
+    fidx[p * 5 + 2] = i0.z;
+    fidx[p * 5 + 3] = i0.w;
+    fidx[p * 5 + 4] = i1.x;
+    fco[p * 4] = rc[2][0];
+    fco[p * 4 + 1] = rc[2][1];
+    fco[p * 4 + 2] = rc[3][0];
+    fco[p * 4 + 3] = rc[3][1];
+    sc2[p] = rc[4][0];
+    Bl[p * 3] = rc[4][1];
+    Bl[p * 3 + 1] = rc[5][0];
+    Bl[p * 3 + 2] = rc[5][1];
     double* row = Fs + (long)p * LD + 4 * QN;
-    row[0] = fp == 0 ? B0 : fp == 1 ? B1 : B2;
-    row[1] = area * cp * cp;
-    row[2] = sc2[p];
-    row[3] = 0.0;
-    Bl[p * 3] = B0;
-    Bl[p * 3 + 1] = B1;
-    Bl[p * 3 + 2] = B2;
-#pragma unroll
-    for (int q = 0; q < 4; ++q)
-      if (q < Q)
-#pragma unroll
-        for (int k = 0; k < 3; ++k) Aq[(p * Q + q) * 3 + k] = Aqv[q][k];
+    row[0] = rc[6][0];
+    row[1] = rc[6][1];
+    row[2] = rc[7][0];
+    row[3] = rc[7][1];
+#pragma unroll
+    for (int k = 0; k < 12; ++k)
+      if (k < 3 * Q) Aq[p * Q * 3 + k] = ra[k >> 1][k & 1];
   }
 #pragma unroll
   for (int u = 0; u < RT_IT; ++u)
@@ -3944,6 +3997,7 @@
   const double *ebar, *AvgSelf, *AvgSide, *A_cpl;
   double *G_nc, *B_sys;
   double* Fnc;
+  const double *ktab, *mtab;
 };
 template <int NTX>
 __global__ __launch_bounds__(512) __attribute__((amdgpu_waves_per_eu(NTX <= 3 ? 5 : 4, 8))) void k_thin(Tmpl t, ThinRtArgs a, ThinNcArgs c) {
@@ -3954,7 +4008,7 @@
   }
   if (threadIdx.x >= 256) return;
   if (blockIdx.z == 0) {
-    const ThinNcfArgs f{a.V, c.ebar, c.AvgSelf, c.AvgSide, a.nbr, c.Fnc, a.N, a.S};
+    const ThinNcfArgs f{a.V, c.AvgSelf, c.AvgSide, a.nbr, c.Fnc, a.N, a.S, c.ktab, c.mtab};
     thin_ncf_body(t, f, side, s);
     return;
   }
@@ -4178,6 +4232,80 @@
   hipLaunchKernelGGL(k_wab, dim3(grid_for(total)), dim3(256), 0, st, ctx->t, total, Aab, Wab);
   LRBMS_LAUNCH_CHECK(ctx);
   return LRBMS_OK;
+}
+
+struct SideTabs {
+  double *rec, *ktab, *mtab;
+};
+static long side_tabs_size(const Tmpl& t, int S) {
+  const long nvs = t.nvx > t.nvy ? t.nvx : t.nvy;
+  return (long)S * (4L * t.ncf * RTREC_LD + 36L * t.ntouch + 16L * nvs * nvs);
+}
+static SideTabs side_tabs_of(const Tmpl& t, int S, double* base) {
+  SideTabs x;
+  x.rec = base;
+  x.ktab = x.rec + (long)S * 4 * t.ncf * RTREC_LD;
+  x.mtab = x.ktab + (long)S * 36 * t.ntouch;
+  return x;
+}
+namespace {
+__global__ __launch_bounds__(256) void k_side_tables(Tmpl t, int S, int Q, const int* __restrict__ nbr, const double* __restrict__ Bbb,
+                                                     const double* __restrict__ Aab, const double* __restrict__ b,
+                                                     const double* __restrict__ ebar, SideTabs x) {
+  const int s = blockIdx.x, side = blockIdx.y, tid = threadIdx.x, nvs = nvs_of(t);
+  for (int p = tid; p < t.ncf; p += 256) {
+    double* rec = x.rec + (((long)s * 4 + side) * t.ncf + p) * RTREC_LD;
+    if (p < t.side_count[side]) rt_side_record(t, nbr, Bbb, Aab, b, Q, S, s, side, p, rec);
+    else
+      for (int i = 0; i < RTREC_LD; ++i) rec[i] = 0.0;
+  }
+  ncf_side_tables(t, ebar, s, side, tid, 256, x.ktab + ((long)s * 4 + side) * 9 * t.ntouch, x.mtab + ((long)s * 4 + side) * 4 * nvs * nvs);
+}
+}
+
+static int side_tables_ensure(lrbms_ctx* ctx, int Q, const double* Bbb, const double* Aab, const double* b, const double* ebar,
+                              hipStream_t st, SideTabs* out) {
+  const Tmpl& t = ctx->t;
+  const long need = side_tabs_size(t, ctx->S);
+  if (ctx->stab_cap < need) {
+    if (ctx->stab) LRBMS_HIP_CHECK(ctx, hipFree(ctx->stab));
+    ctx->stab = nullptr;
+    ctx->stab_cap = 0;
+    LRBMS_HIP_CHECK(ctx, hipMalloc(&ctx->stab, sizeof(double) * (size_t)need));
+    ctx->stab_cap = need;
+    for (int k = 0; k < lrbms_ctx::SRC_COUNT; ++k) ctx->stab_ptr[k] = nullptr;
+  }
+  const SideTabs x = side_tabs_of(t, ctx->S, ctx->stab);
+  if (out) *out = x;
+  const double* src[lrbms_ctx::SRC_COUNT] = {Bbb, Aab, b, ebar};
+  bool kept = ctx->opt_side_tables != 0 && ctx->stab_Q == Q;
+  for (int k = 0; k < lrbms_ctx::SRC_COUNT; ++k) {
+    const long gen = asm_gen_of(ctx, k, src[k]);
+    kept = kept && gen >= 0 && ctx->stab_ptr[k] == src[k] && ctx->stab_gen[k] == gen;
+  }
+  if (kept) return LRBMS_OK;
+  {
+    KScope ks(ctx, "k_side_tables", st);
+    hipLaunchKernelGGL(k_side_tables, dim3(ctx->S, 4), dim3(256), 0, st, t, ctx->S, Q, ctx->nbr, Bbb, Aab, b, ebar, x);
+  }
+  LRBMS_LAUNCH_CHECK(ctx);
+  ctx->stab_Q = Q;
+  for (int k = 0; k < lrbms_ctx::SRC_COUNT; ++k) {
+    ctx->stab_ptr[k] = src[k];
+    ctx->stab_gen[k] = asm_gen_of(ctx, k, src[k]);
+  }
+  return LRBMS_OK;
+}
+
+int side_tables_after_assembly(lrbms_ctx* ctx, bool from_rhs, hipStream_t st) {
+  for (int k = 0; k < lrbms_ctx::SRC_COUNT; ++k)
+    if (ctx->asm_ptr[k] == nullptr) return LRBMS_OK;
+  if (ctx->opt_side_tables == 0 || ctx->asm_Q < 1 || ctx->asm_Q > 4) return LRBMS_OK;
+  const double* tb = ctx->stab_ptr[lrbms_ctx::SRC_B];
+  if (from_rhs && tb != nullptr && tb != ctx->asm_ptr[lrbms_ctx::SRC_B] && asm_gen_of(ctx, lrbms_ctx::SRC_B, tb) >= 0) return LRBMS_OK;
+  const double* b = tb != nullptr && asm_gen_of(ctx, lrbms_ctx::SRC_B, tb) >= 0 ? tb : ctx->asm_ptr[lrbms_ctx::SRC_B];
+  return side_tables_ensure(ctx, ctx->asm_Q, ctx->asm_ptr[lrbms_ctx::SRC_BBB], ctx->asm_ptr[lrbms_ctx::SRC_AAB], b,
+                            ctx->asm_ptr[lrbms_ctx::SRC_EBAR], st, nullptr);
 }
 
 static bool f1w_usable(lrbms_ctx* ctx, int Q, int N) { return Q == 2 && N % 2 == 0; }
@@ -4324,7 +4452,8 @@
     for (int i = 0; i < 11; ++i) probe.push_back({i < 2 ? G_SYS : i == 2 ? G_ENERGY : i == 3 ? G_MASS : i < 7 ? G_AA : G_AB, i == 6 ? 1 : 0, i == 5 || i == 6 ? 1 : 0});
     f1w_ok = Q == 2 && f1w_layout(probe, N, Q);
     if (f1w_ok) {
-      if (ctx->wab != nullptr && ctx->wab_src == Aab && ctx->wab_Q == Q) {
+      if (ctx->opt_side_tables != 0 && ctx->wab != nullptr && ctx->wab_src == Aab && ctx->wab_Q == Q &&
+          ctx->wab_gen == asm_gen_of(ctx, lrbms_ctx::SRC_AAB, Aab)) {
         Wab = ctx->wab;
       } else {
         double* wloc = AvgSide + (long)S * 4 * nvs * N + (long)S * 4 * t.ncf * fside_ld(Q, N);
@@ -4333,6 +4462,9 @@
       }
     }
   }
+  SideTabs tabs{};
+  if (do_b)
+    if (int rc = side_tables_ensure(ctx, Q, Bbb, Aab, b, ebar, st, &tabs)) return rc;
   if (do_prep) {
     if (prep_from_lds) {
       KScope ks(ctx, "k_prep_lds", st);
@@ -4534,8 +4666,8 @@
     if (int rc = side_prep(ctx->aux[0])) return rc;
   if (do_b && merge_thin) {
     const int ntx = (N + 15) / 16;
-    ThinRtArgs a{V, Rself, Rside, Bbb, Aab, b, ctx->nbr, Fside, r_fd, Q, N, S};
-    ThinNcArgs c{ebar, AvgSelf, AvgSide, A_cpl, G_nc, B_sys, Fnc};
+    ThinRtArgs a{V, Rself, Rside, ctx->nbr, Fside, r_fd, Q, N, S, tabs.rec};
+    ThinNcArgs c{ebar, AvgSelf, AvgSide, A_cpl, G_nc, B_sys, Fnc, tabs.ktab, tabs.mtab};
     size_t lds = factored ? thin_ncf_lds_bytes(t, N) : thin_nc_lds_bytes(t, ntx);
     lds = std::max(lds, thin_rt_lds_bytes(t, Q, N));
     lds = std::max(lds, coupling_lds_bytes(t, ntx, Q));
@@ -4552,7 +4684,7 @@
     hipLaunchKernelGGL(k_thin3<NTX>, dim3(4, Sg, 3), dim3(256), lds, s_rt, t, a, f, A_cpl, B_sys);                            \
   } while (0)
     if (factored) {
-      const ThinNcfArgs f{V, ebar, AvgSelf, AvgSide, ctx->nbr, Fnc, N, S};
+      const ThinNcfArgs f{V, AvgSelf, AvgSide, ctx->nbr, Fnc, N, S, tabs.ktab, tabs.mtab};
       KScope ks(ctx, "k_thin3", s_rt);
       switch (ntx) {
         case 1: LRBMS_THIN3(1); break;
@@ -4588,7 +4720,7 @@
     }
     const int ntx = (N + 15) / 16;
     if (factored) {
-      const ThinNcfArgs f{V, ebar, AvgSelf, AvgSide, ctx->nbr, Fnc, N, S};
+      const ThinNcfArgs f{V, AvgSelf, AvgSide, ctx->nbr, Fnc, N, S, tabs.ktab, tabs.mtab};
       const size_t ldsf = thin_ncf_lds_bytes(t, N);
       if (ldsf > 64 * 1024)
         LRBMS_HIP_CHECK(ctx, hipFuncSetAttribute((const void*)k_thin_ncf, hipFuncAttributeMaxDynamicSharedMemorySize, (int)ldsf));
@@ -4614,7 +4746,7 @@
 #undef LRBMS_THIN_NC
     }
     LRBMS_LAUNCH_CHECK(ctx);
-    ThinRtArgs a{V, Rself, Rside, Bbb, Aab, b, ctx->nbr, Fside, r_fd, Q, N, S};
+    ThinRtArgs a{V, Rself, Rside, ctx->nbr, Fside, r_fd, Q, N, S, tabs.rec};
     const size_t lds2 = thin_rt_lds_bytes(t, Q, N);
     {
       KScope ks(ctx, "k_thin_rt", s_rt);
diff --git a/pylrbms_amd/csrc/lrbms_dev.h b/pylrbms_amd/csrc/lrbms_dev.h
--- a/pylrbms_amd/csrc/lrbms_dev.h
+++ b/pylrbms_amd/csrc/lrbms_dev.h
@@ -57,6 +57,23 @@
   long wab_cap = 0;
   const double* wab_src = nullptr;
   int wab_Q = 0;
+  long wab_gen = -1;
+  enum { SRC_BBB = 0, SRC_AAB, SRC_B, SRC_EBAR, SRC_COUNT };
+  static constexpr int asm_known_max(int kind) { return kind == SRC_B ? 32 : 4; }
+  struct AsmRec {
+    const double* p;
+    long gen;
+  };
+  std::vector<AsmRec> asm_known[SRC_COUNT];
+  long asm_counter = 0;
+  const double* asm_ptr[SRC_COUNT] = {nullptr, nullptr, nullptr, nullptr};
+  int asm_Q = 0;
+  double* stab = nullptr;
+  long stab_cap = 0;
+  const double* stab_ptr[SRC_COUNT] = {nullptr, nullptr, nullptr, nullptr};
+  long stab_gen[SRC_COUNT] = {0, 0, 0, 0};
+  int stab_Q = 0;
+  int opt_side_tables = 1;
   bool pass_ran = false;
   bool diag_explicit = false;
   int* subset = nullptr;
@@ -76,6 +93,34 @@
 
 int build_template_tables(lrbms_ctx* ctx);
 int launch_wab(lrbms_ctx* ctx, int Q, const double* Aab, double* Wab, hipStream_t st);
+inline void note_assembled(lrbms_ctx* ctx, int kind, const double* p) {
+  std::vector<lrbms_ctx::AsmRec>& known = ctx->asm_known[kind];
+  for (size_t i = 0; i < known.size(); ++i)
+    if (known[i].p == p) {
+      known.erase(known.begin() + (long)i);
+      break;
+    }
+  for (size_t i = 0; (int)known.size() >= lrbms_ctx::asm_known_max(kind) && i < known.size();) {
+    if (known[i].p == ctx->stab_ptr[kind]) ++i;
+    else known.erase(known.begin() + (long)i);
+  }
+  known.push_back({p, ++ctx->asm_counter});
+  ctx->asm_ptr[kind] = p;
+}
+inline long asm_gen_of(const lrbms_ctx* ctx, int kind, const double* p) {
+  for (const lrbms_ctx::AsmRec& r : ctx->asm_known[kind])
+    if (r.p == p) return r.gen;
+  return -1;
+}
+inline void forget_assembled(lrbms_ctx* ctx) {
+  for (int k = 0; k < lrbms_ctx::SRC_COUNT; ++k) {
+    ctx->asm_known[k].clear();
+    ctx->asm_ptr[k] = nullptr;
+    ctx->stab_ptr[k] = nullptr;
+  }
+  ctx->wab_src = nullptr;
+}
+int side_tables_after_assembly(lrbms_ctx* ctx, bool from_rhs, hipStream_t st);
 long f1_mfma_per_subdomain(lrbms_ctx* ctx, int Q, int N);
 int coarse_begin(lrbms_ctx* ctx, double** A0_out, hipStream_t st);
 int coarse_finish(lrbms_ctx* ctx, const double** A0inv_out, hipStream_t st);
diff --git a/pylrbms_amd/sources.py b/pylrbms_amd/sources.py
--- a/pylrbms_amd/sources.py
+++ b/pylrbms_amd/sources.py
@@ -70,6 +70,9 @@
     sp = eng.quadrature
     xf, cl, kl = volume_record_points(eng.grid, eng.local, (sp.rhs, sp.f2))
     f_smp_K = eng.ctx.from_numpy(np.ascontiguousarray(np.stack([sample_function(fn, xf, cl, kl) for fn in funcs])))
-    b_K = torch.stack([eng.ctx.assemble_rhs(f_smp_K[j].contiguous(), eng.lhat)[0] for j in range(len(funcs))]).contiguous()
+    c = eng.ctx
+    b_K, f2, ceps = c.empty(len(funcs), eng.S, eng.t.n), c.empty(eng.S), c.empty(eng.S)
+    for j in range(len(funcs)):
+        c.assemble_rhs(f_smp_K[j].contiguous(), eng.lhat, out=(b_K[j], f2, ceps))
     F2 = eng.ctx.assemble_source_gram(f_smp_K)
     return {'functions': funcs, 'coefficients': coeffs, 'K': len(funcs), 'f_smp_K': f_smp_K, 'b_K': b_K, 'F2': F2}
```

New measurement: 1.751 million subdomains/s (median of 6 runs). 1.8% higher.
